# bepu/bepuphysics2

Measured on NVIDIA H100. Metric: constraint-iterations/sec (solver+integrator), higher is better.
Workload: dtype f32

## Files before the change

### bepuphysics2_b200/csrc/bepu_contacts.cuh

```cuda
#pragma once
#include "bepu_device_math.cuh"

namespace BEPU_NS {

constexpr int kLanes = 32;

struct GlobalRows { const float* ptr; };
struct GlobalAcc { float* ptr; };
struct StagedRows { uint32_t addr, bar, parity; };
struct StagedAcc { uint32_t addr; float* ptr; };
BEPU_DI float lds_f32(uint32_t addr) {
    float v;
    asm("ld.shared.f32 %0, [%1];" : "=f"(v) : "r"(addr));
    return v;
}
BEPU_DI void rows_ready(GlobalRows) {}
BEPU_DI void rows_ready(StagedRows p) {
    asm volatile(
        "{\n"
        ".reg .pred p;\n"
        "MBAR_WAIT:\n"
        "mbarrier.try_wait.parity.shared::cta.b64 p, [%0], %1;\n"
        "@p bra MBAR_DONE;\n"
        "bra MBAR_WAIT;\n"
        "MBAR_DONE:\n"
        "}\n" ::"r"(p.bar), "r"(p.parity)
        : "memory");
}
BEPU_DI float ldrow(const float* p, int r) { return __ldcg(p + r * kLanes); }
BEPU_DI float ldrow(GlobalRows p, int r) { return __ldcg(p.ptr + r * kLanes); }
BEPU_DI float ldrow(StagedRows p, int r) { return lds_f32(p.addr + r * (kLanes * 4)); }
template <class PR> BEPU_DI V3 ldrow3(PR p, int r) { return {ldrow(p, r), ldrow(p, r + 1), ldrow(p, r + 2)}; }
template <class PR> BEPU_DI Q4 ldrow4(PR p, int r) { return {ldrow(p, r), ldrow(p, r + 1), ldrow(p, r + 2), ldrow(p, r + 3)}; }
BEPU_DI float ldacc(GlobalAcc a, int r) { return a.ptr[r * kLanes]; }
BEPU_DI void stacc(GlobalAcc a, int r, float v) { a.ptr[r * kLanes] = v; }
BEPU_DI float ldacc(StagedAcc a, int r) { return lds_f32(a.addr + r * (kLanes * 4)); }
BEPU_DI void stacc(StagedAcc a, int r, float v) { __stcs(a.ptr + r * kLanes, v); }

BEPU_DI void penetration_apply(const Inertia& iA, const Inertia& iB, V3 normal, V3 angularA, V3 angularB, float impulse, Velocity& vA, Velocity& vB) {
    V3 dLinA = normal * (impulse * iA.inv_mass);
    V3 dAngA = transform(angularA * impulse, iA.t);
    V3 dLinB = normal * (impulse * iB.inv_mass);
    V3 dAngB = transform(angularB * impulse, iB.t);
    vA.lin = vA.lin + dLinA;
    vA.ang = vA.ang + dAngA;
    vB.lin = vB.lin - dLinB;
    vB.ang = vB.ang + dAngB;
}
BEPU_DI void penetration_warm_start(const Inertia& iA, const Inertia& iB, V3 normal, V3 offsetA, V3 offsetB, float accumulated, Velocity& vA, Velocity& vB) {
    penetration_apply(iA, iB, normal, cross(offsetA, normal), cross(normal, offsetB), accumulated, vA, vB);
}
BEPU_DI void penetration_solve(const Inertia& iA, const Inertia& iB, V3 normal, V3 offsetA, V3 offsetB, float depth, const Springiness& sp, float maxRecovery,
                               float inverseDt, float& accumulated, Velocity& vA, Velocity& vB) {
    V3 angularA = cross(offsetA, normal);
    V3 angularB = cross(normal, offsetB);
    float angularA0 = vector_sandwich(angularA, iA.t);
    float angularB0 = vector_sandwich(angularB, iB.t);
    float linear = iA.inv_mass + iB.inv_mass;
    float effectiveMass = sp.effective_mass_cfm_scale / (linear + angularA0 + angularB0);
    float biasVelocity = fmin_ps(depth * inverseDt, fmin_ps(depth * sp.position_error_to_velocity, maxRecovery));
    float csvaLinear = dot(vA.lin, normal);
    float csvaAngular = dot(vA.ang, angularA);
    float negatedCSVBLinear = dot(vB.lin, normal);
    float csvbAngular = dot(vB.ang, angularB);
    float negatedCSI = accumulated * sp.softness_impulse_scale + (csvaLinear - negatedCSVBLinear + csvaAngular + csvbAngular - biasVelocity) * effectiveMass;
    float previous = accumulated;
    accumulated = fmax_ps(0.0f, accumulated - negatedCSI);
    penetration_apply(iA, iB, normal, angularA, angularB, accumulated - previous, vA, vB);
}
BEPU_DI float updated_depth(float dt, V3 contactOffsetA, V3 offsetB, V3 normal, const Velocity& vA, const Velocity& vB, float depth) {
    V3 contactVelocityA = cross(vA.ang, contactOffsetA) + vA.lin;
    V3 contactOffsetB = contactOffsetA - offsetB;
    V3 contactVelocityB = cross(vB.ang, contactOffsetB) + vB.lin;
    float estimatedDepthChangeVelocity = dot(normal, contactVelocityA - contactVelocityB);
    return depth - estimatedDepthChangeVelocity * dt;
}

BEPU_DI void penetration1_apply(const Inertia& iA, V3 normal, V3 angularA, float impulse, Velocity& vA) {
    V3 dLinA = normal * (impulse * iA.inv_mass);
    V3 dAngA = transform(angularA * impulse, iA.t);
    vA.lin = vA.lin + dLinA;
    vA.ang = vA.ang + dAngA;
}
BEPU_DI void penetration1_solve(const Inertia& iA, V3 normal, V3 offsetA, float depth, const Springiness& sp, float maxRecovery, float inverseDt, float& accumulated,
                                Velocity& vA) {
    V3 angularA = cross(offsetA, normal);
    float angularA0 = vector_sandwich(angularA, iA.t);
    float effectiveMass = sp.effective_mass_cfm_scale / (iA.inv_mass + angularA0);
    float biasVelocity = fmin_ps(depth * inverseDt, fmin_ps(depth * sp.position_error_to_velocity, maxRecovery));
    float csvaLinear = dot(vA.lin, normal);
    float csvaAngular = dot(vA.ang, angularA);
    float negatedCSI = accumulated * sp.softness_impulse_scale + (csvaLinear + csvaAngular - biasVelocity) * effectiveMass;
    float previous = accumulated;
    accumulated = fmax_ps(0.0f, accumulated - negatedCSI);
    penetration1_apply(iA, normal, angularA, accumulated - previous, vA);
}
BEPU_DI float updated_depth1(float dt, V3 contactOffset, V3 normal, const Velocity& v, float depth) {
    V3 contactVelocity = cross(v.ang, contactOffset) + v.lin;
    return depth - dot(normal, contactVelocity) * dt;
}

struct TangentJacobians { M23 linearA, angularA, angularB; };
BEPU_DI TangentJacobians tangent_jacobians(V3 tX, V3 tY, V3 offsetA, V3 offsetB) {
    TangentJacobians j;
    j.linearA = {tX, tY};
    j.angularA = {cross(offsetA, tX), cross(offsetA, tY)};
    j.angularB = {cross(tX, offsetB), cross(tY, offsetB)};
    return j;
}
BEPU_DI void tangent_apply(const TangentJacobians& j, const Inertia& iA, const Inertia& iB, V2 impulse, Velocity& vA, Velocity& vB) {
    V3 linearImpulseA = transform(impulse, j.linearA);
    V3 angularImpulseA = transform(impulse, j.angularA);
    V3 angularImpulseB = transform(impulse, j.angularB);
    vA.lin = vA.lin + linearImpulseA * iA.inv_mass;
    vA.ang = vA.ang + transform(angularImpulseA, iA.t);
    vB.lin = vB.lin - linearImpulseA * iB.inv_mass;
    vB.ang = vB.ang + transform(angularImpulseB, iB.t);
}
BEPU_DI void tangent_solve(V3 tX, V3 tY, V3 offsetA, V3 offsetB, const Inertia& iA, const Inertia& iB, float maximumImpulse, V2& accumulated, Velocity& vA, Velocity& vB) {
    TangentJacobians j = tangent_jacobians(tX, tY, offsetA, offsetB);
    Sym2 linear = sandwich_scale(j.linearA, iA.inv_mass) + sandwich_scale(j.linearA, iB.inv_mass);
    Sym2 angular = matrix_sandwich(j.angularA, iA.t) + matrix_sandwich(j.angularB, iB.t);
    Sym2 effectiveMass = invert(linear + angular);
    V2 csvaLinear = transform_by_transpose(vA.lin, j.linearA);
    V2 csvaAngular = transform_by_transpose(vA.ang, j.angularA);
    V2 csvbLinear = transform_by_transpose(vB.lin, j.linearA);
    V2 csvbAngular = transform_by_transpose(vB.ang, j.angularB);
    V2 csv = (csvbLinear - csvaLinear) - (csvaAngular + csvbAngular);
    V2 csi = transform(csv, effectiveMass);
    V2 previous = accumulated;
    accumulated = accumulated + csi;
    float magnitude = length(accumulated);
    float scl = fmin_ps(1.0f, maximumImpulse / fmax_ps(1e-16f, magnitude));
    accumulated = accumulated * scl;
    tangent_apply(j, iA, iB, accumulated - previous, vA, vB);
}
BEPU_DI void tangent1_apply(const M23& linearA, const M23& angularA, const Inertia& iA, V2 impulse, Velocity& vA) {
    V3 linearImpulseA = transform(impulse, linearA);
    V3 angularImpulseA = transform(impulse, angularA);
    vA.lin = vA.lin + linearImpulseA * iA.inv_mass;
    vA.ang = vA.ang + transform(angularImpulseA, iA.t);
}
BEPU_DI void tangent1_solve(V3 tX, V3 tY, V3 offsetA, const Inertia& iA, float maximumImpulse, V2& accumulated, Velocity& vA) {
    M23 linearA{tX, tY};
    M23 angularA{cross(offsetA, tX), cross(offsetA, tY)};
    Sym2 effectiveMass = invert(sandwich_scale(linearA, iA.inv_mass) + matrix_sandwich(angularA, iA.t));
    V2 csv = transform_by_transpose(vA.lin, linearA) + transform_by_transpose(vA.ang, angularA);
    V2 negativeCSI = transform(csv, effectiveMass);
    V2 previous = accumulated;
    accumulated = accumulated - negativeCSI;
    float magnitude = length(accumulated);
    float scl = fmin_ps(1.0f, maximumImpulse / fmax_ps(1e-16f, magnitude));
    accumulated = accumulated * scl;
    tangent1_apply(linearA, angularA, iA, accumulated - previous, vA);
}

BEPU_DI void twist_apply(V3 axis, const Inertia& iA, const Inertia& iB, float impulse, Velocity& vA, Velocity& vB) {
    V3 worldImpulseA = axis * impulse;
    vA.ang = vA.ang + transform(worldImpulseA, iA.t);
    vB.ang = vB.ang - transform(worldImpulseA, iB.t);
}
BEPU_DI void twist_solve(V3 axis, const Inertia& iA, const Inertia& iB, float maximumImpulse, float& accumulated, Velocity& vA, Velocity& vB) {
    float inverseEffectiveMass = vector_sandwich(axis, iA.t) + vector_sandwich(axis, iB.t);
    float effectiveMass = (0.0f == inverseEffectiveMass) ? 0.0f : 1.0f / inverseEffectiveMass;
    float negatedCSI = (dot(vA.ang, axis) - dot(vB.ang, axis)) * effectiveMass;
    float previous = accumulated;
    accumulated = fmin_ps(maximumImpulse, fmax_ps(-maximumImpulse, accumulated - negatedCSI));
    twist_apply(axis, iA, iB, accumulated - previous, vA, vB);
}
BEPU_DI void twist1_apply(V3 axis, const Inertia& iA, float impulse, Velocity& vA) { vA.ang = vA.ang + transform(axis * impulse, iA.t); }
BEPU_DI void twist1_solve(V3 axis, const Inertia& iA, float maximumImpulse, float& accumulated, Velocity& vA) {
    float angularA = vector_sandwich(axis, iA.t);
    float effectiveMass = (0.0f == angularA) ? 0.0f : 1.0f / angularA;
    float negativeCSI = dot(vA.ang, axis) * effectiveMass;
    float previous = accumulated;
    accumulated = fmin_ps(maximumImpulse, fmax_ps(-maximumImpulse, accumulated - negativeCSI));
    twist1_apply(axis, iA, accumulated - previous, vA);
}

template <int N, bool TwoBody> struct ConvexLayout {
    static constexpr int kOffsetB = 4 * N;
    static constexpr int kNormal = TwoBody ? 4 * N + 3 : 4 * N;
    static constexpr int kFriction = kNormal + 3;
    static constexpr int kAngularFrequency = kNormal + 4;
    static constexpr int kTwiceDampingRatio = kNormal + 5;
    static constexpr int kMaxRecovery = kNormal + 6;
    static constexpr int kPrestepRows = kNormal + 7;
    static constexpr int kImpulseRows = N + 3;
};

template <int N> BEPU_DI V3 friction_center(const V3 (&offs)[N], const float (&depths)[N]) {
    float w[N];
#pragma unroll
    for (int i = 0; i < N; ++i) w[i] = depths[i] < 0.0f ? 0.0f : 1.0f;
    float weightSum = w[0];
#pragma unroll
    for (int i = 1; i < N; ++i) weightSum = weightSum + w[i];
    bool useFallback = weightSum == 0.0f;
    weightSum = useFallback ? (float)N : weightSum;
    float inverseWeightSum = 1.0f / weightSum;
    V3 c[N];
#pragma unroll
    for (int i = 0; i < N; ++i) c[i] = offs[i] * (useFallback ? inverseWeightSum : w[i] * inverseWeightSum);
    if constexpr (N == 2) return c[0] + c[1];
    else if constexpr (N == 3) return (c[0] + c[1]) + c[2];
    else return (c[0] + c[1]) + (c[2] + c[3]);
}

template <int N> struct ConvexTwoBody {
    typedef ConvexLayout<N, true> L;
    static constexpr int kBodies = 2;
    static constexpr int kPrestepRows = L::kPrestepRows;
    static constexpr int kImpulseRows = L::kImpulseRows;
    static constexpr bool kIncremental = true;
    static constexpr bool kNeedsPose = false;

    template <class PR, class AR> BEPU_DI static void warm_start(const Inertia& iA, const Inertia& iB, PR p, AR a, Velocity& vA, Velocity& vB) {
        V3 normal = ldrow3(p, L::kNormal), offsetB = ldrow3(p, L::kOffsetB);
        V3 x, z;
        build_orthonormal_basis(normal, x, z);
        V3 offs[N];
        float depths[N];
#pragma unroll
        for (int i = 0; i < N; ++i) { offs[i] = ldrow3(p, 4 * i); depths[i] = ldrow(p, 4 * i + 3); }
        V3 centerA;
        if constexpr (N == 1) centerA = offs[0]; else centerA = friction_center<N>(offs, depths);
        V3 centerB = centerA - offsetB;
        tangent_apply(tangent_jacobians(x, z, centerA, centerB), iA, iB, V2{ldacc(a, 0), ldacc(a, 1)}, vA, vB);
#pragma unroll 1
        for (int i = 0; i < N; ++i) {
            V3 offset = ldrow3(p, 4 * i);
            penetration_warm_start(iA, iB, normal, offset, offset - offsetB, ldacc(a, 2 + i), vA, vB);
        }
        twist_apply(normal, iA, iB, ldacc(a, N + 2), vA, vB);
    }
    template <class PR, class AR> BEPU_DI static void solve(const Inertia& iA, const Inertia& iB, float dt, float inverseDt, PR p, AR a, Velocity& vA, Velocity& vB) {
        V3 normal = ldrow3(p, L::kNormal), offsetB = ldrow3(p, L::kOffsetB);
        float friction = ldrow(p, L::kFriction), maxRecovery = ldrow(p, L::kMaxRecovery);
        Springiness sp = compute_springiness(ldrow(p, L::kAngularFrequency), ldrow(p, L::kTwiceDampingRatio), dt);
        if constexpr (N > 1) {
            V3 offs[N];
            float depths[N];
#pragma unroll
            for (int i = 0; i < N; ++i) { offs[i] = ldrow3(p, 4 * i); depths[i] = ldrow(p, 4 * i + 3); }
            const V3 centerA = friction_center<N>(offs, depths);
            float penSum = 0.0f, twistSum = 0.0f;
#pragma unroll 1
            for (int i = 0; i < N; ++i) {
                V3 offset = ldrow3(p, 4 * i);
                float pen = ldacc(a, 2 + i);
                penetration_solve(iA, iB, normal, offset, offset - offsetB, ldrow(p, 4 * i + 3), sp, maxRecovery, inverseDt, pen, vA, vB);
                stacc(a, 2 + i, pen);
                const float lever = pen * distance(centerA, offset);
                penSum = i == 0 ? pen : penSum + pen;
                twistSum = i == 0 ? lever : twistSum + lever;
            }
            V3 x, z;
            build_orthonormal_basis(normal, x, z);
            V2 tangent{ldacc(a, 0), ldacc(a, 1)};
            float twist = ldacc(a, N + 2);
            const float premultiplied = (1.0f / N) * friction;
            tangent_solve(x, z, centerA, centerA - offsetB, iA, iB, premultiplied * penSum, tangent, vA, vB);
            twist_solve(normal, iA, iB, premultiplied * twistSum, twist, vA, vB);
            stacc(a, 0, tangent.x);
            stacc(a, 1, tangent.y);
            stacc(a, N + 2, twist);
        } else
        {
        V3 offs[N];
        float depths[N], pen[N];
#pragma unroll
        for (int i = 0; i < N; ++i) { offs[i] = ldrow3(p, 4 * i); depths[i] = ldrow(p, 4 * i + 3); pen[i] = ldacc(a, 2 + i); }
#pragma unroll
        for (int i = 0; i < N; ++i) penetration_solve(iA, iB, normal, offs[i], offs[i] - offsetB, depths[i], sp, maxRecovery, inverseDt, pen[i], vA, vB);
        V3 x, z;
        build_orthonormal_basis(normal, x, z);
        V2 tangent{ldacc(a, 0), ldacc(a, 1)};
        float twist = ldacc(a, N + 2);
        if constexpr (N == 1) {
            float maximumTangentImpulse = friction * pen[0];
            tangent_solve(x, z, offs[0], offs[0] - offsetB, iA, iB, maximumTangentImpulse, tangent, vA, vB);
            float maximumTwistImpulse = friction * pen[0] * fmax_ps(0.0f, depths[0]);
            twist_solve(normal, iA, iB, maximumTwistImpulse, twist, vA, vB);
        } else {
            float premultiplied = (1.0f / N) * friction;
            float penSum = pen[0];
#pragma unroll
            for (int i = 1; i < N; ++i) penSum = penSum + pen[i];
            V3 centerA = friction_center<N>(offs, depths);
            tangent_solve(x, z, centerA, centerA - offsetB, iA, iB, premultiplied * penSum, tangent, vA, vB);
            float twistSum = pen[0] * distance(centerA, offs[0]);
#pragma unroll
            for (int i = 1; i < N; ++i) twistSum = twistSum + pen[i] * distance(centerA, offs[i]);
            twist_solve(normal, iA, iB, premultiplied * twistSum, twist, vA, vB);
        }
        stacc(a, 0, tangent.x);
        stacc(a, 1, tangent.y);
#pragma unroll
        for (int i = 0; i < N; ++i) stacc(a, 2 + i, pen[i]);
        stacc(a, N + 2, twist);
        }
    }
    BEPU_DI static void incremental_update(float dt, const Velocity& vA, const Velocity& vB, float* p) {
        V3 normal = ldrow3(p, L::kNormal), offsetB = ldrow3(p, L::kOffsetB);
#pragma unroll
        for (int i = 0; i < N; ++i) p[(4 * i + 3) * kLanes] = updated_depth(dt, ldrow3(p, 4 * i), offsetB, normal, vA, vB, ldrow(p, 4 * i + 3));
    }
};

template <int N> struct ConvexOneBody {
    typedef ConvexLayout<N, false> L;
    static constexpr int kBodies = 1;
    static constexpr int kPrestepRows = L::kPrestepRows;
    static constexpr int kImpulseRows = L::kImpulseRows;
    static constexpr bool kIncremental = true;
    static constexpr bool kNeedsPose = false;

    template <class PR, class AR> BEPU_DI static void warm_start(const Inertia& iA, PR p, AR a, Velocity& vA) {
        V3 normal = ldrow3(p, L::kNormal);
        V3 x, z;
        build_orthonormal_basis(normal, x, z);
        V3 offs[N];
        float depths[N];
#pragma unroll
        for (int i = 0; i < N; ++i) { offs[i] = ldrow3(p, 4 * i); depths[i] = ldrow(p, 4 * i + 3); }
        V3 centerA;
        if constexpr (N == 1) centerA = offs[0]; else centerA = friction_center<N>(offs, depths);
        tangent1_apply(M23{x, z}, M23{cross(centerA, x), cross(centerA, z)}, iA, V2{ldacc(a, 0), ldacc(a, 1)}, vA);
#pragma unroll 1
        for (int i = 0; i < N; ++i) penetration1_apply(iA, normal, cross(ldrow3(p, 4 * i), normal), ldacc(a, 2 + i), vA);
        twist1_apply(normal, iA, ldacc(a, N + 2), vA);
    }
    template <class PR, class AR> BEPU_DI static void solve(const Inertia& iA, float dt, float inverseDt, PR p, AR a, Velocity& vA) {
        V3 normal = ldrow3(p, L::kNormal);
        float friction = ldrow(p, L::kFriction), maxRecovery = ldrow(p, L::kMaxRecovery);
        Springiness sp = compute_springiness(ldrow(p, L::kAngularFrequency), ldrow(p, L::kTwiceDampingRatio), dt);
        if constexpr (N > 1) {
            V3 offs[N];
            float depths[N];
#pragma unroll
            for (int i = 0; i < N; ++i) { offs[i] = ldrow3(p, 4 * i); depths[i] = ldrow(p, 4 * i + 3); }
            const V3 centerA = friction_center<N>(offs, depths);
            float penSum = 0.0f, twistSum = 0.0f;
#pragma unroll 1
            for (int i = 0; i < N; ++i) {
                V3 offset = ldrow3(p, 4 * i);
                float pen = ldacc(a, 2 + i);
                penetration1_solve(iA, normal, offset, ldrow(p, 4 * i + 3), sp, maxRecovery, inverseDt, pen, vA);
                stacc(a, 2 + i, pen);
                const float lever = pen * distance(centerA, offset);
                penSum = i == 0 ? pen : penSum + pen;
                twistSum = i == 0 ? lever : twistSum + lever;
            }
            V3 x, z;
            build_orthonormal_basis(normal, x, z);
            V2 tangent{ldacc(a, 0), ldacc(a, 1)};
            float twist = ldacc(a, N + 2);
            const float premultiplied = (1.0f / N) * friction;
            tangent1_solve(x, z, centerA, iA, premultiplied * penSum, tangent, vA);
            twist1_solve(normal, iA, premultiplied * twistSum, twist, vA);
            stacc(a, 0, tangent.x);
            stacc(a, 1, tangent.y);
            stacc(a, N + 2, twist);
        } else
        {
        V3 offs[N];
        float depths[N], pen[N];
#pragma unroll
        for (int i = 0; i < N; ++i) { offs[i] = ldrow3(p, 4 * i); depths[i] = ldrow(p, 4 * i + 3); pen[i] = ldacc(a, 2 + i); }
#pragma unroll
        for (int i = 0; i < N; ++i) penetration1_solve(iA, normal, offs[i], depths[i], sp, maxRecovery, inverseDt, pen[i], vA);
        V3 x, z;
        build_orthonormal_basis(normal, x, z);
        V2 tangent{ldacc(a, 0), ldacc(a, 1)};
        float twist = ldacc(a, N + 2);
        if constexpr (N == 1) {
            tangent1_solve(x, z, offs[0], iA, friction * pen[0], tangent, vA);
            twist1_solve(normal, iA, friction * pen[0] * fmax_ps(0.0f, depths[0]), twist, vA);
        } else {
            float premultiplied = (1.0f / N) * friction;
            float penSum = pen[0];
#pragma unroll
            for (int i = 1; i < N; ++i) penSum = penSum + pen[i];
            V3 centerA = friction_center<N>(offs, depths);
            tangent1_solve(x, z, centerA, iA, premultiplied * penSum, tangent, vA);
            float twistSum = pen[0] * distance(centerA, offs[0]);
#pragma unroll
            for (int i = 1; i < N; ++i) twistSum = twistSum + pen[i] * distance(centerA, offs[i]);
            twist1_solve(normal, iA, premultiplied * twistSum, twist, vA);
        }
        stacc(a, 0, tangent.x);
        stacc(a, 1, tangent.y);
#pragma unroll
        for (int i = 0; i < N; ++i) stacc(a, 2 + i, pen[i]);
        stacc(a, N + 2, twist);
        }
    }
    BEPU_DI static void incremental_update(float dt, const Velocity& vA, float* p) {
        V3 normal = ldrow3(p, L::kNormal);
#pragma unroll
        for (int i = 0; i < N; ++i) p[(4 * i + 3) * kLanes] = updated_depth1(dt, ldrow3(p, 4 * i), normal, vA, ldrow(p, 4 * i + 3));
    }
};

#define BEPU_CONTACT_LOOP _Pragma("unroll 1")
template <int N, bool TwoBody> struct NonconvexLayout {
    static constexpr int kOffsetB = 4;
    static constexpr int kContacts = TwoBody ? 7 : 4;
    static constexpr int kPrestepRows = kContacts + 7 * N;
    static constexpr int kImpulseRows = 3 * N;
};
template <int N> struct NonconvexTwoBody {
    typedef NonconvexLayout<N, true> L;
    static constexpr int kBodies = 2;
    static constexpr int kPrestepRows = L::kPrestepRows;
    static constexpr int kImpulseRows = L::kImpulseRows;
    static constexpr bool kIncremental = true;
    static constexpr bool kNeedsPose = false;
    template <class PR, class AR> BEPU_DI static void warm_start(const Inertia& iA, const Inertia& iB, PR p, AR a, Velocity& vA, Velocity& vB) {
        V3 offsetB = ldrow3(p, L::kOffsetB);
BEPU_CONTACT_LOOP
        for (int i = 0; i < N; ++i) {
            const int c = L::kContacts + 7 * i;
            V3 offset = ldrow3(p, c), normal = ldrow3(p, c + 4);
            V3 x, z;
            build_orthonormal_basis(normal, x, z);
            V3 contactOffsetB = offset - offsetB;
            tangent_apply(tangent_jacobians(x, z, offset, contactOffsetB), iA, iB, V2{ldacc(a, 3 * i), ldacc(a, 3 * i + 1)}, vA, vB);
            penetration_warm_start(iA, iB, normal, offset, contactOffsetB, ldacc(a, 3 * i + 2), vA, vB);
        }
    }
    template <class PR, class AR> BEPU_DI static void solve(const Inertia& iA, const Inertia& iB, float dt, float inverseDt, PR p, AR a, Velocity& vA, Velocity& vB) {
        V3 offsetB = ldrow3(p, L::kOffsetB);
        float friction = ldrow(p, 0), maxRecovery = ldrow(p, 3);
        Springiness sp = compute_springiness(ldrow(p, 1), ldrow(p, 2), dt);
BEPU_CONTACT_LOOP
        for (int i = 0; i < N; ++i) {
            const int c = L::kContacts + 7 * i;
            V3 offset = ldrow3(p, c), normal = ldrow3(p, c + 4);
            float depth = ldrow(p, c + 3);
            V2 tangent{ldacc(a, 3 * i), ldacc(a, 3 * i + 1)};
            float pen = ldacc(a, 3 * i + 2);
            V3 contactOffsetB = offset - offsetB;
            penetration_solve(iA, iB, normal, offset, contactOffsetB, depth, sp, maxRecovery, inverseDt, pen, vA, vB);
            V3 x, z;
            build_orthonormal_basis(normal, x, z);
            tangent_solve(x, z, offset, contactOffsetB, iA, iB, friction * pen, tangent, vA, vB);
            stacc(a, 3 * i, tangent.x);
            stacc(a, 3 * i + 1, tangent.y);
            stacc(a, 3 * i + 2, pen);
        }
    }
    BEPU_DI static void incremental_update(float dt, const Velocity& vA, const Velocity& vB, float* p) {
        V3 offsetB = ldrow3(p, L::kOffsetB);
#pragma unroll
        for (int i = 0; i < N; ++i) {
            const int c = L::kContacts + 7 * i;
            p[(c + 3) * kLanes] = updated_depth(dt, ldrow3(p, c), offsetB, ldrow3(p, c + 4), vA, vB, ldrow(p, c + 3));
        }
    }
};
template <int N> struct NonconvexOneBody {
    typedef NonconvexLayout<N, false> L;
    static constexpr int kBodies = 1;
    static constexpr int kPrestepRows = L::kPrestepRows;
    static constexpr int kImpulseRows = L::kImpulseRows;
    static constexpr bool kIncremental = true;
    static constexpr bool kNeedsPose = false;
    template <class PR, class AR> BEPU_DI static void warm_start(const Inertia& iA, PR p, AR a, Velocity& vA) {
BEPU_CONTACT_LOOP
        for (int i = 0; i < N; ++i) {
            const int c = L::kContacts + 7 * i;
            V3 offset = ldrow3(p, c), normal = ldrow3(p, c + 4);
            V3 x, z;
            build_orthonormal_basis(normal, x, z);
            tangent1_apply(M23{x, z}, M23{cross(offset, x), cross(offset, z)}, iA, V2{ldacc(a, 3 * i), ldacc(a, 3 * i + 1)}, vA);
            penetration1_apply(iA, normal, cross(offset, normal), ldacc(a, 3 * i + 2), vA);
        }
    }
    template <class PR, class AR> BEPU_DI static void solve(const Inertia& iA, float dt, float inverseDt, PR p, AR a, Velocity& vA) {
        float friction = ldrow(p, 0), maxRecovery = ldrow(p, 3);
        Springiness sp = compute_springiness(ldrow(p, 1), ldrow(p, 2), dt);
BEPU_CONTACT_LOOP
        for (int i = 0; i < N; ++i) {
            const int c = L::kContacts + 7 * i;
            V3 offset = ldrow3(p, c), normal = ldrow3(p, c + 4);
            float depth = ldrow(p, c + 3);
            V2 tangent{ldacc(a, 3 * i), ldacc(a, 3 * i + 1)};
            float pen = ldacc(a, 3 * i + 2);
            penetration1_solve(iA, normal, offset, depth, sp, maxRecovery, inverseDt, pen, vA);
            V3 x, z;
            build_orthonormal_basis(normal, x, z);
            tangent1_solve(x, z, offset, iA, friction * pen, tangent, vA);
            stacc(a, 3 * i, tangent.x);
            stacc(a, 3 * i + 1, tangent.y);
            stacc(a, 3 * i + 2, pen);
        }
    }
    BEPU_DI static void incremental_update(float dt, const Velocity& vA, float* p) {
#pragma unroll
        for (int i = 0; i < N; ++i) {
            const int c = L::kContacts + 7 * i;
            p[(c + 3) * kLanes] = updated_depth1(dt, ldrow3(p, c), ldrow3(p, c + 4), vA, ldrow(p, c + 3));
        }
    }
};

}
```

### bepuphysics2_b200/csrc/bepu_solver_kernels.cuh

```cuda
#pragma once
#include "bepu_contacts.cuh"
#include "bepu_joints_more.cuh"
#include "bepu_integration.cuh"
#include "bepu_device_types.h"

namespace BEPU_NS {

using namespace bepucuda;

struct F8 { float a, b, c, d, e, f, g, h; };
#define BEPU_BODY_LD "ld.global.L1::no_allocate.L2::cache_hint.v4.f32"
#define BEPU_BODY_ST "st.global.L1::no_allocate.L2::cache_hint.v4.f32"
BEPU_DI uint64_t l2_evict_last_policy() {
    uint64_t policy;
    asm("createpolicy.fractional.L2::evict_last.b64 %0, 1.0;" : "=l"(policy));
    return policy;
}
BEPU_DI F8 ld256(const float4* p) {
    F8 r;
    asm volatile(BEPU_BODY_LD " {%0,%1,%2,%3}, [%8], %9;\n\t" BEPU_BODY_LD " {%4,%5,%6,%7}, [%8+16], %9;"
                 : "=f"(r.a), "=f"(r.b), "=f"(r.c), "=f"(r.d), "=f"(r.e), "=f"(r.f), "=f"(r.g), "=f"(r.h)
                 : "l"(p), "l"(l2_evict_last_policy())
                 : "memory");
    return r;
}
BEPU_DI void st256(float4* p, float a, float b, float c, float d, float e, float f, float g, float h) {
    asm volatile(BEPU_BODY_ST " [%0], {%1,%2,%3,%4}, %9;\n\t" BEPU_BODY_ST " [%0+16], {%5,%6,%7,%8}, %9;" ::"l"(p), "f"(a), "f"(b), "f"(c), "f"(d), "f"(e), "f"(f), "f"(g), "f"(h),
                 "l"(l2_evict_last_policy())
                 : "memory");
}
BEPU_DI void load_velocity(const float4* vel, uint32_t i, Velocity& v) {
    const F8 r = ld256(vel + 2 * (size_t)i);
    v.lin = {r.a, r.b, r.c};
    v.ang = {r.e, r.f, r.g};
}
BEPU_DI void store_velocity(float4* vel, uint32_t i, const Velocity& v) { st256(vel + 2 * (size_t)i, v.lin.x, v.lin.y, v.lin.z, 0.0f, v.ang.x, v.ang.y, v.ang.z, 0.0f); }
BEPU_DI void load_inertia(const float4* in, uint32_t i, Inertia& r) {
    const F8 x = ld256(in + 2 * (size_t)i);
    r.t = {x.a, x.b, x.c, x.d, x.e, x.f};
    r.inv_mass = x.g;
}
BEPU_DI void store_inertia(float4* in, uint32_t i, const Inertia& r) { st256(in + 2 * (size_t)i, r.t.xx, r.t.yx, r.t.yy, r.t.zx, r.t.zy, r.t.zz, r.inv_mass, 0.0f); }
BEPU_DI void load_pose(const float4* pose, uint32_t i, V3& pos, Q4& q) {
    const F8 x = ld256(pose + 2 * (size_t)i);
    q = {x.a, x.b, x.c, x.d};
    pos = {x.e, x.f, x.g};
}
BEPU_DI void store_pose(float4* pose, uint32_t i, V3 pos, Q4 q) { st256(pose + 2 * (size_t)i, q.x, q.y, q.z, q.w, pos.x, pos.y, pos.z, 0.0f); }

template <int STAGE, bool NeedsPose>
BEPU_DI void warm_start_body(uint32_t enc, const BodyBuffers& B, const FrameParams& fp, BodyState& b, Velocity& v) {
    const uint32_t idx = enc & kRefIndexMask;
    if (enc & kRefIntegrateBit) {
        Inertia local;
        load_inertia(B.inertia_local, idx, local);
        load_pose(B.pose, idx, b.pos, b.q);
        b.inertia.inv_mass = local.inv_mass;
        if (STAGE == kStageWarmStart) {
            b.pos = b.pos + v.lin * fp.dt;
            Q4 previousOrientation = b.q;
            b.q = integrate_orientation(b.q, v.ang, fp.dt * 0.5f);
            b.inertia.t = rotate_inverse_inertia(local.t, b.q);
            if (fp.angular_mode == 1) integrate_angular_conserve_momentum(previousOrientation, local.t, b.inertia.t, v.ang);
            else if (fp.angular_mode == 2) integrate_angular_gyroscopic(b.q, local.t, v.ang, fp.dt);
            store_pose(B.pose, idx, b.pos, b.q);
        } else {
            b.inertia.t = rotate_inverse_inertia(local.t, b.q);
            if (fp.angular_mode == 1) {
                Q4 previousOrientation = integrate_orientation(b.q, v.ang, fp.dt * -0.5f);
                integrate_angular_conserve_momentum(previousOrientation, local.t, b.inertia.t, v.ang);
            } else if (fp.angular_mode == 2) {
                integrate_angular_gyroscopic(b.q, local.t, v.ang, fp.dt);
            }
        }
        callback_integrate_velocity(v, fp.gravity_dt[0], fp.gravity_dt[1], fp.gravity_dt[2], fp.linear_damping_dt, fp.angular_damping_dt);
        store_inertia(B.inertia_world, idx, b.inertia);
    } else {
        load_inertia(B.inertia_world, idx, b.inertia);
        if (NeedsPose) load_pose(B.pose, idx, b.pos, b.q);
        if (STAGE == kStageWarmStartFirst && fp.angular_mode != 0 && (enc & kRefBundleIntegratesBit) && !(enc & kRefKinematicBit)) {
            Inertia local;
            load_inertia(B.inertia_local, idx, local);
            V3 pos;
            Q4 q;
            load_pose(B.pose, idx, pos, q);
            if (fp.angular_mode == 1) integrate_angular_conserve_momentum(integrate_orientation(q, v.ang, fp.dt * -0.5f), local.t, b.inertia.t, v.ang);
            else integrate_angular_gyroscopic(q, local.t, v.ang, fp.dt);
        }
    }
}
template <int STAGE, bool NeedsPose>
BEPU_DI void gather_for_warm_start(uint32_t enc, const BodyBuffers& B, const FrameParams& fp, BodyState& b, Velocity& v) {
    load_velocity(B.velocity, enc & kRefIndexMask, v);
    warm_start_body<STAGE, NeedsPose>(enc, B, fp, b, v);
}

template <class T, class PR, class AR> BEPU_DI void call_warm_start(const BodyState* b, PR p, AR a, Velocity* v) {
    if constexpr (T::kNeedsPose) T::warm_start(b, p, a, v);
    else if constexpr (T::kBodies == 2) T::warm_start(b[0].inertia, b[1].inertia, p, a, v[0], v[1]);
    else T::warm_start(b[0].inertia, p, a, v[0]);
}
template <class T, class PR, class AR> BEPU_DI void call_solve(const BodyState* b, float dt, float inverseDt, PR p, AR a, Velocity* v) {
    if constexpr (T::kNeedsPose) T::solve(b, dt, inverseDt, p, a, v);
    else if constexpr (T::kBodies == 2) T::solve(b[0].inertia, b[1].inertia, dt, inverseDt, p, a, v[0], v[1]);
    else T::solve(b[0].inertia, dt, inverseDt, p, a, v[0]);
}
template <class T> BEPU_DI void call_incremental(float dt, const Velocity* v, float* p) {
    if constexpr (T::kIncremental) {
        if constexpr (T::kBodies == 2) T::incremental_update(dt, v[0], v[1], p);
        else T::incremental_update(dt, v[0], p);
    }
}

BEPU_DI uint32_t ldg_nc_u32(const void* p) {
    uint32_t v;
    asm volatile("ld.global.nc.u32 %0, [%1];" : "=r"(v) : "l"(p));
    return v;
}
BEPU_DI void push_record(float4* const* arrays, uint32_t mask, uint32_t idx, float a, float b, float c, float d, float e, float f, float g, float h) {
    while (mask) {
        const int q = __ffs((int)mask) - 1;
        mask &= mask - 1u;
        float4* dst = arrays[q] + 2 * (size_t)idx;
        dst[0] = make_float4(a, b, c, d);
        dst[1] = make_float4(e, f, g, h);
    }
}
template <class T, int STAGE, bool kSharded, class PR, class AR>
BEPU_DI void run_lane(const int32_t* refs, PR p, AR a, float* p_rw, uint32_t enc0, uint32_t enc1, const BodyBuffers& B, const FrameParams& fp, const ShardPeers* peers = nullptr,
                      long long peer_delta = 0) {
    constexpr int NB = T::kBodies;
    uint32_t enc[NB];
    enc[0] = enc0;
    if constexpr (NB > 1) enc[1] = enc1;
#pragma unroll
    for (int s = 2; s < NB; ++s) enc[s] = (uint32_t)__ldg(refs + s * kLanes);
    uint32_t push_to[kSharded ? NB : 1];
    if constexpr (kSharded) {
#pragma unroll
        for (int s = 0; s < NB; ++s) push_to[s] = peer_delta != 0 ? ldg_nc_u32(refs + peer_delta + s * kLanes) : 0u;
    }
    if ((int32_t)enc[0] == kRefEmpty) return;
    BodyState b[NB];
    Velocity v[NB];
    if constexpr (STAGE == kStageIncremental) {
#pragma unroll
        for (int s = 0; s < NB; ++s) load_velocity(B.velocity, enc[s] & kRefIndexMask, v[s]);
        call_incremental<T>(fp.dt, v, p_rw);
    } else if constexpr (STAGE == kStageSolve) {
#pragma unroll
        for (int s = 0; s < NB; ++s) {
            const uint32_t idx = enc[s] & kRefIndexMask;
            load_velocity(B.velocity, idx, v[s]);
            load_inertia(B.inertia_world, idx, b[s].inertia);
            if (T::kNeedsPose) load_pose(B.pose, idx, b[s].pos, b[s].q);
        }
        rows_ready(p);
        call_solve<T>(b, fp.dt, fp.inverse_dt, p, a, v);
#pragma unroll
        for (int s = 0; s < NB; ++s)
            if (!(enc[s] & kRefKinematicBit)) {
                store_velocity(B.velocity, enc[s] & kRefIndexMask, v[s]);
                if constexpr (kSharded) {
                    const uint32_t mask = push_to[s];
                    if (mask) push_record(peers->velocity, mask, enc[s] & kRefIndexMask, v[s].lin.x, v[s].lin.y, v[s].lin.z, 0.0f, v[s].ang.x, v[s].ang.y, v[s].ang.z, 0.0f);
                }
            }
    } else {
#pragma unroll
        for (int s = 0; s < NB; ++s) gather_for_warm_start<STAGE, T::kNeedsPose>(enc[s], B, fp, b[s], v[s]);
        rows_ready(p);
        call_warm_start<T>(b, p, a, v);
#pragma unroll
        for (int s = 0; s < NB; ++s)
            if (!(enc[s] & kRefKinematicBit)) {
                const uint32_t idx = enc[s] & kRefIndexMask;
                store_velocity(B.velocity, idx, v[s]);
                if constexpr (kSharded) {
                    const uint32_t mask = push_to[s];
                    if (mask) {
                        push_record(peers->velocity, mask, idx, v[s].lin.x, v[s].lin.y, v[s].lin.z, 0.0f, v[s].ang.x, v[s].ang.y, v[s].ang.z, 0.0f);
                        if (enc[s] & kRefIntegrateBit) {
                            const Inertia& in = b[s].inertia;
                            push_record(peers->inertia_world, mask, idx, in.t.xx, in.t.yx, in.t.yy, in.t.zx, in.t.zy, in.t.zz, in.inv_mass, 0.0f);
                            if (STAGE == kStageWarmStart) push_record(peers->pose, mask, idx, b[s].q.x, b[s].q.y, b[s].q.z, b[s].q.w, b[s].pos.x, b[s].pos.y, b[s].pos.z, 0.0f);
                        }
                    }
                }
            }
    }
}
template <class T, int STAGE, class PR, class AR>
BEPU_DI void run_lane(const int32_t* refs, PR p, AR a, float* p_rw, uint32_t enc0, uint32_t enc1, const BodyBuffers& B, const FrameParams& fp) {
    run_lane<T, STAGE, false>(refs, p, a, p_rw, enc0, enc1, B, fp);
}

BEPU_DI int4 ldg_nc_v4(const void* p) {
    int4 v;
    asm volatile("ld.global.nc.v4.s32 {%0,%1,%2,%3}, [%4];" : "=r"(v.x), "=r"(v.y), "=r"(v.z), "=r"(v.w) : "l"(p));
    return v;
}
BEPU_DI WorkRecord load_record(const WorkRecord* r) {
    const int4 lo = ldg_nc_v4(r), hi = ldg_nc_v4(reinterpret_cast<const int4*>(r) + 1);
    WorkRecord w;
    w.refs = reinterpret_cast<int32_t*>((unsigned long long)(unsigned int)lo.x | ((unsigned long long)(unsigned int)lo.y << 32));
    w.prestep = reinterpret_cast<float*>((unsigned long long)(unsigned int)lo.z | ((unsigned long long)(unsigned int)lo.w << 32));
    w.impulses = reinterpret_cast<float*>((unsigned long long)(unsigned int)hi.x | ((unsigned long long)(unsigned int)hi.y << 32));
    w.type_id = hi.z;
    w.live_lanes = hi.w;
    return w;
}

#define BEPU_CONTACT_TYPES(X)                                                                                                     \
    X(0, ConvexOneBody<1>) X(1, ConvexOneBody<2>) X(2, ConvexOneBody<3>) X(3, ConvexOneBody<4>)                                   \
    X(4, ConvexTwoBody<1>) X(5, ConvexTwoBody<2>) X(6, ConvexTwoBody<3>) X(7, ConvexTwoBody<4>)                                   \
    X(8, NonconvexOneBody<2>) X(9, NonconvexOneBody<3>) X(10, NonconvexOneBody<4>)                                                \
    X(15, NonconvexTwoBody<2>) X(16, NonconvexTwoBody<3>) X(17, NonconvexTwoBody<4>)

template <int STAGE, bool kSharded, class PR, class AR>
BEPU_DI void run_bundle_rows(const WorkRecord& rec, int lane, PR p, AR a, uint32_t enc0, uint32_t enc1, const BodyBuffers& B, const FrameParams& fp, const ShardPeers* peers = nullptr,
                             long long peer_delta = 0) {
    const int32_t* refs = rec.refs + lane;
    float* p_rw = rec.prestep + lane;
    switch (rec.type_id) {
#define BEPU_CASE(ID, T) \
    case ID: run_lane<T, STAGE, kSharded>(refs, p, a, p_rw, enc0, enc1, B, fp, peers, peer_delta); break;
        BEPU_CONTACT_TYPES(BEPU_CASE)
        BEPU_JOINT_TYPES(BEPU_CASE)
        BEPU_JOINT_TYPES_MORE(BEPU_CASE)
#undef BEPU_CASE
        default: break;
    }
}
template <int STAGE, class PR, class AR>
BEPU_DI void run_bundle_rows(const WorkRecord& rec, int lane, PR p, AR a, uint32_t enc0, uint32_t enc1, const BodyBuffers& B, const FrameParams& fp) {
    run_bundle_rows<STAGE, false>(rec, lane, p, a, enc0, enc1, B, fp);
}
template <int STAGE>
BEPU_DI void run_bundle(const WorkRecord& rec, int lane, uint32_t enc0, uint32_t enc1, const BodyBuffers& B, const FrameParams& fp) {
    run_bundle_rows<STAGE>(rec, lane, GlobalRows{rec.prestep + lane}, GlobalAcc{rec.impulses + lane}, enc0, enc1, B, fp);
}
template <int STAGE> BEPU_DI void run_bundle(const WorkRecord& rec, int lane, const BodyBuffers& B, const FrameParams& fp) {
    const uint32_t enc0 = ldg_nc_u32(rec.refs + lane), enc1 = ldg_nc_u32(rec.refs + kLanes + lane);
    run_bundle<STAGE>(rec, lane, enc0, enc1, B, fp);
}

struct StageRowCounts { uint8_t prestep[64], impulses[64]; };
__host__ __device__ constexpr StageRowCounts make_stage_row_counts() {
    StageRowCounts c{};
#define BEPU_ROWS(ID, T) c.prestep[ID] = (uint8_t)T::kPrestepRows; c.impulses[ID] = (uint8_t)T::kImpulseRows;
    BEPU_CONTACT_TYPES(BEPU_ROWS)
    BEPU_JOINT_TYPES(BEPU_ROWS)
    BEPU_JOINT_TYPES_MORE(BEPU_ROWS)
#undef BEPU_ROWS
    return c;
}
__constant__ StageRowCounts kStageRowCounts = make_stage_row_counts();
constexpr int kStageSlabRows = 48;
constexpr int kStageSlabBytes = kStageSlabRows * kLanes * 4;

BEPU_DI uint32_t smem_u32(const void* p) { return (uint32_t)__cvta_generic_to_shared(p); }
BEPU_DI void mbar_init(uint32_t bar, uint32_t count) {
    asm volatile("mbarrier.init.shared::cta.b64 [%0], %1;" ::"r"(bar), "r"(count) : "memory");
    asm volatile("fence.mbarrier_init.release.cluster;" ::: "memory");
    asm volatile("fence.proxy.async.shared::cta;" ::: "memory");
}
BEPU_DI void mbar_expect_tx(uint32_t bar, uint32_t bytes) { asm volatile("mbarrier.arrive.expect_tx.shared::cta.b64 _, [%0], %1;" ::"r"(bar), "r"(bytes) : "memory"); }
BEPU_DI uint64_t l2_evict_first_policy() {
    uint64_t policy;
    asm volatile("createpolicy.fractional.L2::evict_first.b64 %0, 1.0;" : "=l"(policy));
    return policy;
}
BEPU_DI void bulk_copy_g2s(uint32_t dst, const void* src, uint32_t bytes, uint32_t bar, uint64_t policy) {
    asm volatile("cp.async.bulk.shared::cluster.global.mbarrier::complete_tx::bytes.L2::cache_hint [%0], [%1], %2, [%3], %4;" ::"r"(dst), "l"(src), "r"(bytes), "r"(bar),
                 "l"(policy)
                 : "memory");
}

#ifndef BEPU_STAGE_BLOCK_THREADS
#define BEPU_STAGE_BLOCK_THREADS 64
#endif
constexpr int kStageBlockThreads = BEPU_STAGE_BLOCK_THREADS;

constexpr int kStagePrefetchRows = 1;
BEPU_DI void shard_announce(const ShardPeers& peers, int lane) {
    if (lane < peers.rank_count && lane != peers.rank)
        asm volatile("red.release.sys.global.add.u64 [%0], 1;" ::"l"(peers.flags[lane] + kShardCounterSlot + peers.rank) : "memory");
}
BEPU_DI void shard_wait(const ShardPeers& peers, int lane, uint32_t solve_index, uint32_t exchange_point, int32_t* error_flag) {
    if (lane < peers.rank_count && lane != peers.rank) {
        const unsigned long long* mine = peers.flags[peers.rank];
        const unsigned long long* targets = mine + kShardTargetSlot + (size_t)lane * kShardMaxExchanges;
        const unsigned long long want = (unsigned long long)solve_index * targets[kShardMaxExchanges - 1] + targets[exchange_point];
        unsigned long long seen;
        unsigned int spins = 0;
        do {
            asm volatile("ld.acquire.sys.global.u64 %0, [%1];" : "=l"(seen) : "l"(mine + kShardCounterSlot + lane) : "memory");
        } while (seen < want && ++spins < 100000000u);
        if (seen < want) atomicExch(error_flag, 5);
    }
    __syncwarp();
}
template <int STAGE, bool kSharded>
BEPU_DI void constraint_stage_body(const WorkRecord* __restrict__ records, const int32_t* __restrict__ ref_rows, int work_count, const BodyBuffers& B, const FrameParams* __restrict__ fpp, int flags, const ShardPeers* peers,
                                   long long peer_delta, const ShardStage* shard = nullptr) {
    constexpr bool kStaged = STAGE != kStageIncremental;
    constexpr int kWarps = kStageBlockThreads / 32;
    __shared__ __align__(128) float slab[kStaged ? kWarps * kStageSlabRows * kLanes : 1];
    __shared__ __align__(8) unsigned long long bars[kWarps];
    const int warp_in_block = threadIdx.x >> 5;
    const int global_warp = (blockIdx.x * kStageBlockThreads + threadIdx.x) >> 5;
    const int lane = threadIdx.x & 31;
    WorkRecord rec{};
    uint32_t enc0 = (uint32_t)kRefEmpty, enc1 = 0;
    const int warp = global_warp;
    const bool active = warp < work_count;
    const uint32_t slab_addr = kStaged ? smem_u32(slab) + warp_in_block * kStageSlabBytes : 0;
    const uint32_t bar = smem_u32(&bars[warp_in_block]);
    const bool early_rows = kStaged && (flags & kStagePrefetchRows);
    uint32_t prestep_bytes = 0, impulse_bytes = 0;
    if (active) {
        rec = load_record(records + warp);
        if constexpr (kStaged) {
            prestep_bytes = kStageRowCounts.prestep[rec.type_id] * (kLanes * 4);
            impulse_bytes = kStageRowCounts.impulses[rec.type_id] * (kLanes * 4);
            if (lane == 0) {
                mbar_init(bar, 1);
                if (early_rows) {
                    const uint64_t policy = l2_evict_first_policy();
                    mbar_expect_tx(bar, prestep_bytes + impulse_bytes);
                    bulk_copy_g2s(slab_addr, rec.prestep, prestep_bytes, bar, policy);
                    bulk_copy_g2s(slab_addr + prestep_bytes, rec.impulses, impulse_bytes, bar, policy);
                }
            }
        }
        enc0 = ldg_nc_u32(ref_rows + (size_t)warp * (2 * kLanes) + lane);
        enc1 = ldg_nc_u32(ref_rows + (size_t)warp * (2 * kLanes) + kLanes + lane);
    }
    const FrameParams fp = *fpp;
    asm volatile("griddepcontrol.wait;" ::: "memory");
    asm volatile("griddepcontrol.launch_dependents;");
    bool boundary = false;
    if constexpr (kSharded) {
        boundary = active && (rec.live_lanes & kRecordBoundaryBit) != 0;
        if (boundary && shard->exchange_index > 0 && !(fp.tune[0] & 1)) shard_wait(*peers, lane, fp.shard_solve_index, shard->exchange_index - 1u, shard->error_flag);
    }
    if (!active) return;
    if constexpr (kStaged) {
        if (!early_rows && lane == 0) {
            const uint64_t policy = l2_evict_first_policy();
            mbar_expect_tx(bar, prestep_bytes + impulse_bytes);
            bulk_copy_g2s(slab_addr, rec.prestep, prestep_bytes, bar, policy);
            bulk_copy_g2s(slab_addr + prestep_bytes, rec.impulses, impulse_bytes, bar, policy);
        }
        __syncwarp();
        run_bundle_rows<STAGE, kSharded>(rec, lane, StagedRows{slab_addr + lane * 4, bar, 0u}, StagedAcc{slab_addr + prestep_bytes + lane * 4, rec.impulses + lane}, enc0, enc1, B, fp,
                                         peers, boundary && !(fp.tune[0] & 4) ? peer_delta : 0);
        if constexpr (kSharded) {
            if (boundary && !(fp.tune[0] & 2)) {
                __syncwarp();
                shard_announce(*peers, lane);
            }
        }
    } else {
        run_bundle<STAGE>(rec, lane, enc0, enc1, B, fp);
    }
}

template <int STAGE, int MINB>
__global__ void __launch_bounds__(kStageBlockThreads, MINB) constraint_stage_kernel(const WorkRecord* __restrict__ records, const int32_t* __restrict__ ref_rows, int work_count, BodyBuffers B, const FrameParams* __restrict__ fpp, int flags) {
    constraint_stage_body<STAGE, false>(records, ref_rows, work_count, B, fpp, flags, nullptr, 0);
}
template <int STAGE, int MINB>
__global__ void __launch_bounds__(kStageBlockThreads, MINB)
constraint_stage_kernel_sharded(const WorkRecord* __restrict__ records, const int32_t* __restrict__ ref_rows, int work_count, BodyBuffers B, const FrameParams* __restrict__ fpp, int flags, const __grid_constant__ ShardPeers peers,
                                long long peer_delta, const __grid_constant__ ShardStage shard) {
    constraint_stage_body<STAGE, true>(records, ref_rows, work_count, B, fpp, flags, &peers, peer_delta, &shard);
}

template <int STAGE> BEPU_DI void run_kinematic(int i, const int32_t* kinematics, const BodyBuffers& B, const FrameParams& fp) {
    const uint32_t idx = (uint32_t)kinematics[i];
    Velocity v;
    load_velocity(B.velocity, idx, v);
    if (STAGE == kStageKinematic) {
        V3 pos;
        Q4 q;
        load_pose(B.pose, idx, pos, q);
        pos = pos + v.lin * fp.dt;
        q = integrate_orientation(q, v.ang, fp.dt * 0.5f);
        store_pose(B.pose, idx, pos, q);
    }
    if (fp.integrate_velocity_for_kinematics) {
        callback_integrate_velocity(v, fp.gravity_dt[0], fp.gravity_dt[1], fp.gravity_dt[2], fp.linear_damping_dt, fp.angular_damping_dt);
        store_velocity(B.velocity, idx, v);
    }
}
template <int STAGE>
__global__ void kinematic_stage_kernel(const int32_t* __restrict__ kinematics, int count, BodyBuffers B, const FrameParams* __restrict__ fpp) {
    const int i = blockIdx.x * blockDim.x + threadIdx.x;
    if (i >= count) return;
    const FrameParams fp = *fpp;
    run_kinematic<STAGE>(i, kinematics, B, fp);
}

BEPU_DI void run_final_pose(int i, const BodyBuffers& B, const FrameParams& fp) {
    V3 pos;
    Q4 q;
    Velocity v;
    load_pose(B.pose, i, pos, q);
    load_velocity(B.velocity, i, v);
    if (B.constrained[i]) {
        q = integrate_orientation(q, v.ang, fp.dt * 0.5f);
        pos = pos + v.lin * fp.dt;
        store_pose(B.pose, i, pos, q);
        return;
    }
    Inertia local;
    load_inertia(B.inertia_local, i, local);
    const bool kinematic = local.inv_mass == 0.0f && local.t.xx == 0.0f && local.t.yx == 0.0f && local.t.yy == 0.0f && local.t.zx == 0.0f && local.t.zy == 0.0f && local.t.zz == 0.0f;
    const bool integrateVelocity = fp.integrate_velocity_for_kinematics || !kinematic;
    const float dt = fp.final_dt, halfDt = fp.final_dt * 0.5f;
    for (int step = 0; step < fp.final_steps; ++step) {
        if (integrateVelocity)
            callback_integrate_velocity(v, fp.final_gravity_dt[0], fp.final_gravity_dt[1], fp.final_gravity_dt[2], fp.final_linear_damping_dt, fp.final_angular_damping_dt);
        pos = pos + v.lin * dt;
        if (fp.angular_mode == 1) {
            Q4 previousOrientation = q;
            q = integrate_orientation(q, v.ang, halfDt);
            integrate_angular_conserve_momentum(previousOrientation, local.t, rotate_inverse_inertia(local.t, q), v.ang);
        } else if (fp.angular_mode == 2) {
            q = integrate_orientation(q, v.ang, halfDt);
            integrate_angular_gyroscopic(q, local.t, v.ang, dt);
        } else {
            q = integrate_orientation(q, v.ang, halfDt);
        }
    }
    store_pose(B.pose, i, pos, q);
    if (integrateVelocity) store_velocity(B.velocity, i, v);
}
static __global__ void final_pose_kernel(BodyBuffers B, const FrameParams* __restrict__ fpp) {
    const int i = blockIdx.x * blockDim.x + threadIdx.x;
    if (i >= B.count) return;
    const FrameParams fp = *fpp;
    run_final_pose(i, B, fp);
}

}
```

### bepuphysics2_b200/csrc/bepucuda_api.cu

```cuda
#include <algorithm>
#include <cmath>
#include <cstdio>
#include <cstdlib>
#include <cstring>
#include <map>
#include <string>
#include <vector>

#include "../../include/bepucuda.h"
#include "bepu_layout_kernels.h"
#include "bepu_coloring.h"
#include "bepu_bounds.h"

using namespace bepucuda;

namespace bepucuda {

static TypeInfo make_contact(int bodies, int prestep, int impulses, int contacts, const char* name) {
    TypeInfo t{};
    t.bodies = bodies; t.prestep_rows = prestep; t.impulse_rows = impulses; t.incremental = 1; t.name = name;
    const int body_rw = 13 + 6;
    t.solve_bytes = 4 * (prestep + 2 * impulses + bodies + bodies * body_rw);
    t.warm_start_bytes = 4 * (prestep + impulses + bodies + bodies * body_rw);
    t.incremental_bytes = 4 * (prestep + contacts + bodies + 6 * bodies);
    return t;
}
static TypeInfo make_joint(int bodies, int prestep, int impulses, int solve_r, int solve_w, int ws_r, int ws_w, const char* name) {
    TypeInfo t{};
    t.bodies = bodies; t.prestep_rows = prestep; t.impulse_rows = impulses; t.incremental = 0; t.name = name;
    t.solve_bytes = 4 * (prestep + 2 * impulses + bodies + solve_r + solve_w);
    t.warm_start_bytes = 4 * (prestep + impulses + bodies + ws_r + ws_w);
    t.incremental_bytes = 0;
    return t;
}
struct Registry {
    TypeInfo types[64];
    bool present[64];
    Registry() {
        std::memset(present, 0, sizeof(present));
        auto add = [&](int id, TypeInfo t) { types[id] = t; present[id] = true; };
        add(0, make_contact(1, 11, 4, 1, "Contact1OneBody")); add(1, make_contact(1, 15, 5, 2, "Contact2OneBody"));
        add(2, make_contact(1, 19, 6, 3, "Contact3OneBody")); add(3, make_contact(1, 23, 7, 4, "Contact4OneBody"));
        add(4, make_contact(2, 14, 4, 1, "Contact1")); add(5, make_contact(2, 18, 5, 2, "Contact2"));
        add(6, make_contact(2, 22, 6, 3, "Contact3")); add(7, make_contact(2, 26, 7, 4, "Contact4"));
        add(8, make_contact(1, 18, 6, 2, "Contact2NonconvexOneBody")); add(9, make_contact(1, 25, 9, 3, "Contact3NonconvexOneBody"));
        add(10, make_contact(1, 32, 12, 4, "Contact4NonconvexOneBody"));
        add(15, make_contact(2, 21, 6, 2, "Contact2Nonconvex")); add(16, make_contact(2, 28, 9, 3, "Contact3Nonconvex"));
        add(17, make_contact(2, 35, 12, 4, "Contact4Nonconvex"));
#define BEPU_REGISTER_JOINTS
#include "bepu_joint_registry.inc"
#undef BEPU_REGISTER_JOINTS
    }
};
static const Registry& registry() {
    static Registry r;
    return r;
}
const TypeInfo* get_type_info(int type_id) {
    if (type_id < 0 || type_id >= 64 || !registry().present[type_id]) return nullptr;
    return &registry().types[type_id];
}

struct DeviceBuffer {
    void* ptr = nullptr;
    size_t capacity = 0;
    cudaError_t reserve(size_t bytes) {
        if (bytes <= capacity) return cudaSuccess;
        if (ptr) cudaFree(ptr);
        ptr = nullptr;
        capacity = 0;
        size_t want = bytes + bytes / 4 + 256;
        cudaError_t e = cudaMalloc(&ptr, want);
        if (e == cudaSuccess) capacity = want;
        return e;
    }
    void release() {
        if (ptr) cudaFree(ptr);
        ptr = nullptr;
        capacity = 0;
    }
    template <class T> T* as() const { return (T*)ptr; }
};

struct ChunkArena {
    struct Chunk { char* base; size_t size, used; };
    std::vector<Chunk> chunks;
    bool pinned_host = false;
    size_t min_chunk = (size_t)64 << 20;
    void reset() { for (auto& c : chunks) c.used = 0; }
    void* alloc(size_t bytes, cudaError_t* err) {
        bytes = (bytes + 255) & ~(size_t)255;
        for (auto& c : chunks)
            if (c.size - c.used >= bytes) {
                void* p = c.base + c.used;
                c.used += bytes;
                return p;
            }
        Chunk c{};
        c.size = std::max(bytes, min_chunk);
        cudaError_t e = pinned_host ? cudaMallocHost((void**)&c.base, c.size) : cudaMalloc((void**)&c.base, c.size);
        if (e != cudaSuccess) { if (err) *err = e; return nullptr; }
        c.used = bytes;
        chunks.push_back(c);
        return chunks.back().base;
    }
    void release() {
        for (auto& c : chunks) { if (pinned_host) cudaFreeHost(c.base); else cudaFree(c.base); }
        chunks.clear();
    }
};

struct SourceTypeBatch {
    int batch_index, type_batch_index, type_id, count;
    int live = 0;
    float* host_impulses;
    int32_t* raw_refs;
    float* raw_prestep;
    float* raw_impulses;
    size_t refs_bytes, prestep_bytes, impulse_bytes;
    std::vector<int32_t> host_refs;
    std::vector<int> device_tbs;
    int32_t* raw_features_old = nullptr;
    int32_t* raw_features_new = nullptr;
    size_t feature_bytes = 0;
    bool resident_impulses = false, redistribute = false;
};

}

struct bepucuda_ctx {
    bepucuda_config cfg{};
    int32_t tune[4] = {0, 0, 0, 0};
    int device = 0;
    cudaStream_t stream = nullptr;
    cudaEvent_t ev_solve_begin = nullptr, ev_solve_end = nullptr, ev_up_begin = nullptr, ev_up_end = nullptr, ev_down_begin = nullptr, ev_down_end = nullptr;
    bool up_open = false, have_solve = false, have_down = false, have_up = false;
    std::string error;
    const SolverLaunchers* launchers = nullptr;

    std::vector<int32_t> iterations{1};
    int fallback_threshold = 64;
    bepucuda_integrator_desc integ{};
    bool integ_set = false;

    int body_count = 0;
    DeviceBuffer raw_bodies, pose, velocity, inertia_local, inertia_world, constrained, first_batch, sync_refcount, sync_mask;
    BodyBuffers B{};

    int W = 8;
    int batch_count = 0;
    bool constraints_open = false, constraints_ready = false, data_dirty = false, descs_dirty = false;
    std::vector<SourceTypeBatch> sources;
    ChunkArena raw_arena, pinned_arena;
    DeviceBuffer record_table, ref_rows, source_bundle_flags, refs32, prestep32, impulses32, tb_table, tdesc_table, work_table, map_table, bodies_per_type, kinematics_dev, program_dev, frame_params_dev, error_dev;
    std::vector<DeviceTypeBatch> tbs;
    std::vector<TransposeDesc> tdescs;
    std::vector<WorkItem> work;
    std::vector<int32_t> bundle_live;
    std::vector<WorkRecord> records;
    std::vector<std::pair<int, int>> batch_work;
    bool exchange_failed = false;
    bepucuda_exchange_fn exchange = nullptr;
    void* exchange_user = nullptr;
    DeviceBuffer exchange_staging;
    bool peer_mode = false;
    ShardPeers peers{};
    DeviceBuffer shard_flags, pushes_dev, peer32, body_masks_dev, boundary_flags_dev;
    uint32_t shard_solve_index = 0;
    std::vector<int> boundary_count;
    std::vector<uint8_t> body_masks;
    size_t refs_words = 0;
    std::vector<void*> opened_ipc;
    std::vector<int32_t> global_first_batch;
    std::vector<uint8_t> global_constrained;
    std::map<int, std::vector<uint32_t>> pushes_by_batch;
    std::vector<std::pair<size_t, int>> push_range;
    uint32_t exchange_counter = 0;
    uint32_t exchanges_per_solve = 0;
    int inc_work_begin = 0, inc_work_count = 0;
    int all_work_count = 0;
    int sync_batch_count = 0, fallback_levels = 0;
    std::vector<int32_t> kinematics;
    std::vector<StageOp> program;
    FrameParams* frame_params_host = nullptr;

    cudaGraph_t graph = nullptr;
    cudaGraphExec_t graph_exec = nullptr;
    bool graph_valid = false;

    bepucuda_timings timings{};
    int64_t h2d_accum = 0;
    struct HostRange { char* host; size_t bytes; char* dev; };
    std::vector<HostRange> host_ranges;
    std::vector<CopyChunk> pending_h2d;
    DeviceBuffer chunk_table;
    struct ChunkStage { void* host = nullptr; size_t capacity = 0; cudaEvent_t done = nullptr; };
    ChunkStage chunk_stage[4];
    int chunk_stage_next = 0;
    cudaEvent_t user_events[16] = {};
    DeviceBuffer body_shapes, body_activities, body_bounds;
    int shape_count = -1;
    DeviceBuffer color_refs, color_priorities, color_body_min, color_body_mask, color_out, color_lists, color_counts;
    std::vector<cudaEvent_t> profile_events;
};

namespace {

int fail(bepucuda_ctx* c, int code, const std::string& msg) {
    if (c) c->error = msg;
    return code;
}
int cuda_fail(bepucuda_ctx* c, cudaError_t e, const char* what) {
    return fail(c, e == cudaErrorMemoryAllocation ? BEPUCUDA_ERR_OUT_OF_MEMORY : BEPUCUDA_ERR_CUDA, std::string(what) + ": " + cudaGetErrorString(e));
}
#define CK(call)                                                  \
    do {                                                          \
        cudaError_t _e = (call);                                  \
        if (_e != cudaSuccess) return cuda_fail(ctx, _e, #call);  \
    } while (0)

void open_upload_window(bepucuda_ctx* ctx) {
    if (!ctx->up_open) {
        cudaEventRecord(ctx->ev_up_begin, ctx->stream);
        ctx->up_open = true;
    }
}

char* map_host(bepucuda_ctx* ctx, const void* ptr, size_t bytes) {
    const char* p = (const char*)ptr;
    for (auto& r : ctx->host_ranges)
        if (p >= r.host && p + bytes <= r.host + r.bytes) return r.dev + (p - r.host);
    return nullptr;
}
void queue_chunks(std::vector<CopyChunk>& list, void* dst, const void* src, size_t bytes) {
    const size_t kChunk = (size_t)64 << 10;
    for (size_t off = 0; off < bytes; off += kChunk) list.push_back({(char*)dst + off, (const char*)src + off, std::min(kChunk, bytes - off)});
}
int flush_chunks(bepucuda_ctx* ctx, std::vector<CopyChunk>& list) {
    if (list.empty()) return BEPUCUDA_OK;
    const size_t bytes = list.size() * sizeof(CopyChunk);
    CK(ctx->chunk_table.reserve(bytes));
    auto& st = ctx->chunk_stage[ctx->chunk_stage_next];
    ctx->chunk_stage_next = (ctx->chunk_stage_next + 1) & 3;
    if (!st.done) CK(cudaEventCreateWithFlags(&st.done, cudaEventDisableTiming));
    CK(cudaEventSynchronize(st.done));
    if (st.capacity < bytes) {
        if (st.host) cudaFreeHost(st.host);
        st.host = nullptr;
        st.capacity = 0;
        CK(cudaMallocHost(&st.host, bytes * 2));
        st.capacity = bytes * 2;
    }
    std::memcpy(st.host, list.data(), bytes);
    CK(cudaMemcpyAsync(ctx->chunk_table.ptr, st.host, bytes, cudaMemcpyHostToDevice, ctx->stream));
    launch_batched_copy(ctx->chunk_table.as<CopyChunk>(), (int)list.size(), ctx->stream);
    CK(cudaGetLastError());
    CK(cudaEventRecord(st.done, ctx->stream));
    list.clear();
    return BEPUCUDA_OK;
}

int copy_in(bepucuda_ctx* ctx, void* dst, const void* src, size_t bytes) {
    if (bytes == 0) return BEPUCUDA_OK;
    if (char* alias = map_host(ctx, src, bytes)) {
        queue_chunks(ctx->pending_h2d, dst, alias, bytes);
        ctx->h2d_accum += (int64_t)bytes;
        return BEPUCUDA_OK;
    }
    if (bytes < ((size_t)256 << 10)) {
        cudaError_t e = cudaSuccess;
        void* stage = ctx->pinned_arena.alloc(bytes, &e);
        if (!stage) return cuda_fail(ctx, e, "pinned staging");
        std::memcpy(stage, src, bytes);
        CK(cudaMemcpyAsync(dst, stage, bytes, cudaMemcpyHostToDevice, ctx->stream));
    } else {
        CK(cudaMemcpyAsync(dst, src, bytes, cudaMemcpyHostToDevice, ctx->stream));
    }
    ctx->h2d_accum += (int64_t)bytes;
    return BEPUCUDA_OK;
}

void invalidate_graph(bepucuda_ctx* ctx) {
    if (ctx->graph_exec) cudaGraphExecDestroy(ctx->graph_exec);
    if (ctx->graph) cudaGraphDestroy(ctx->graph);
    ctx->graph_exec = nullptr;
    ctx->graph = nullptr;
    ctx->graph_valid = false;
}

void issue_stage_sequence(bepucuda_ctx* ctx, cudaStream_t s, int64_t* launches) {
    const WorkRecord* records = ctx->record_table.as<WorkRecord>();
    const int32_t* ref_rows = ctx->ref_rows.as<int32_t>();
    const FrameParams* fp = ctx->frame_params_dev.as<FrameParams>();
    const int32_t* kin = ctx->kinematics_dev.as<int32_t>();
    int64_t n = 0;
    const bool pdl = ctx->cfg.reserved[1] == 0;
    const StageOp* previous = nullptr;
    uint32_t exchange_index = 0;
    const bool fused_pushes = ctx->peer_mode && !ctx->body_masks.empty();
    for (const StageOp& op : ctx->program) {
        if (ctx->peer_mode && op.pad == -1) {
            launch_shard_exchange(nullptr, 0, 1, ctx->B, ctx->peers, fp, exchange_index++, ctx->error_dev.as<int32_t>(), s);
            ++n;
            continue;
        }
        if (ctx->peer_mode && op.pad >= 2 && op.stage <= kStageSolve) {
            if (op.work_count > 0) {
                bool prefetch = previous != nullptr && previous->stage != kStageIncremental && !(previous->stage <= kStageSolve && previous->work_begin == op.work_begin && previous->work_count > 0);
                const int launch_flags = (pdl ? kLaunchPdl : 0) | (prefetch ? kLaunchPrefetchRows : 0);
                if (fused_pushes) {
                    const ShardStage shard{exchange_index, ctx->error_dev.as<int32_t>()};
                    ctx->launchers->constraint_stage_sharded(op.stage, records + op.work_begin, ref_rows + (size_t)op.work_begin * 64, op.work_count, ctx->B, fp, launch_flags, ctx->peers,
                                                             (long long)(ctx->peer32.as<int32_t>() - ctx->refs32.as<int32_t>()), shard, s);
                    ++exchange_index;
                    ++n;
                    previous = &op;
                    continue;
                }
                ctx->launchers->constraint_stage(op.stage, records + op.work_begin, ref_rows + (size_t)op.work_begin * 64, op.work_count, ctx->B, fp, launch_flags, s);
                ++n;
            }
            if (fused_pushes) { ++exchange_index; continue; }
            const auto& range = ctx->push_range[op.pad - 2];
            launch_shard_exchange(ctx->pushes_dev.as<uint32_t>() + range.first, range.second, op.stage == kStageSolve ? 1 : (op.stage == kStageWarmStart ? 3 : 2), ctx->B, ctx->peers, fp,
                                  exchange_index++, ctx->error_dev.as<int32_t>(), s);
            ++n;
            if (op.work_count > 0) previous = &op;
            continue;
        }
        switch (op.stage) {
            case kStageWarmStartFirst: case kStageWarmStart: case kStageSolve: case kStageIncremental:
                if (op.work_count > 0) {
                    bool prefetch = op.stage != kStageIncremental && previous != nullptr && previous->stage != kStageIncremental;
                    if (prefetch && previous->stage <= kStageSolve && previous->work_begin == op.work_begin) prefetch = false;
                    if (ctx->exchange) {
                        ctx->launchers->constraint_stage(op.stage, records + op.work_begin, ref_rows + (size_t)op.work_begin * 64, op.work_count, ctx->B, fp, 0, s);
                        ++n;
                        if (op.stage != kStageIncremental) {
                            const int planes = op.stage == kStageSolve ? 1 : (op.stage == kStageWarmStart ? 3 : 2);
                            const size_t words = (size_t)ctx->body_count * 8 * planes;
                            cudaMemsetAsync(ctx->exchange_staging.ptr, 0, words * 4, s);
                            launch_collect_stage(ctx->tb_table.as<DeviceTypeBatch>(), ctx->work_table.as<WorkItem>() + op.work_begin, op.work_count, ctx->bodies_per_type.as<int32_t>(), op.stage,
                                                 ctx->B, ctx->exchange_staging.as<int32_t>(), s);
                            if (ctx->exchange(ctx->exchange_user, ctx->exchange_staging.ptr, (int64_t)words, 0, (void*)s) != 0) ctx->exchange_failed = true;
                            launch_apply_stage(ctx->exchange_staging.as<int32_t>(), planes, ctx->B, s);
                            n += 2;
                        }
                        previous = &op;
                        break;
                    }
                    ctx->launchers->constraint_stage(op.stage, records + op.work_begin, ref_rows + (size_t)op.work_begin * 64, op.work_count, ctx->B, fp, (pdl ? kLaunchPdl : 0) | (prefetch ? kLaunchPrefetchRows : 0), s);
                    previous = &op;
                    ++n;
                }
                break;
            case kStageKinematicFirst: case kStageKinematic:
                if (op.work_count > 0) { ctx->launchers->kinematic_stage(op.stage, kin, op.work_count, ctx->B, fp, s); previous = &op; ++n; }
                break;
            case kStageFinalPose:
                if (ctx->B.count > 0) { ctx->launchers->final_pose(ctx->B, fp, s); previous = &op; ++n; }
                break;
        }
    }
    if (launches) *launches = n;
    ctx->exchanges_per_solve = exchange_index;
}

void build_program(bepucuda_ctx* ctx) {
    ctx->program.clear();
    const int substeps = (int)ctx->iterations.size();
    const int kin = (int)ctx->kinematics.size();
    for (int s = 0; s < substeps; ++s) {
        if (s > 0) {
            if (ctx->peer_mode) ctx->program.push_back({kStageKinematic, 0, 0, -1});
            if (ctx->inc_work_count > 0) ctx->program.push_back({kStageIncremental, ctx->inc_work_begin, ctx->inc_work_count, 0});
            if (kin > 0) ctx->program.push_back({kStageKinematic, 0, kin, 0});
        } else if (ctx->integ.integrate_velocity_for_kinematics && kin > 0) {
            ctx->program.push_back({kStageKinematicFirst, 0, kin, 0});
        }
        if (ctx->peer_mode) ctx->program.push_back({kStageKinematic, 0, 0, -1});
        for (size_t b = 0; b < ctx->batch_work.size(); ++b) {
            auto& bw = ctx->batch_work[b];
            if (bw.second > 0 || (ctx->peer_mode && (int)b < ctx->sync_batch_count)) ctx->program.push_back({s == 0 ? kStageWarmStartFirst : kStageWarmStart, bw.first, bw.second, ctx->peer_mode ? (int)b + 2 : 0});
        }
        for (int it = 0; it < ctx->iterations[s]; ++it)
            for (size_t b = 0; b < ctx->batch_work.size(); ++b) {
                auto& bw = ctx->batch_work[b];
                if (bw.second > 0 || (ctx->peer_mode && (int)b < ctx->sync_batch_count)) ctx->program.push_back({kStageSolve, bw.first, bw.second, ctx->peer_mode ? (int)b + 2 : 0});
            }
    }
    if (ctx->peer_mode) ctx->program.push_back({kStageKinematic, 0, 0, -1});
    ctx->program.push_back({kStageFinalPose, 0, ctx->body_count, 0});
}

int upload_program(bepucuda_ctx* ctx) {
    build_program(ctx);
    if (ctx->peer_mode && !ctx->body_masks.empty() && ctx->boundary_count.size() == ctx->batch_work.size()) {
        std::vector<unsigned long long> targets((size_t)kShardMaxExchanges, 0ull);
        unsigned long long arrived = 0;
        size_t e = 0;
        for (const StageOp& op : ctx->program) {
            if (op.pad != -1 && !(op.pad >= 2 && op.stage <= kStageSolve)) continue;
            if (e + 1 >= (size_t)kShardMaxExchanges) return fail(ctx, BEPUCUDA_ERR_BAD_STATE, "peer sharding: more than 4095 exchange points per solve");
            if (op.pad >= 2 && op.work_count > 0) arrived += (unsigned long long)ctx->boundary_count[(size_t)(op.pad - 2)];
            targets[e++] = arrived;
        }
        targets[(size_t)kShardMaxExchanges - 1] = arrived;
        CK(cudaStreamSynchronize(ctx->stream));
        for (int q = 0; q < ctx->peers.rank_count; ++q)
            if (q != ctx->peers.rank)
                CK(cudaMemcpy(ctx->peers.flags[q] + kShardTargetSlot + (size_t)ctx->peers.rank * kShardMaxExchanges, targets.data(), targets.size() * 8, cudaMemcpyDefault));
        CK(cudaMemset((unsigned long long*)ctx->shard_flags.ptr + kShardCounterSlot, 0, kMaxShardRanks * 8));
        ctx->shard_solve_index = 0;
    }
    CK(ctx->program_dev.reserve(ctx->program.size() * sizeof(StageOp)));
    CK(cudaMemcpyAsync(ctx->program_dev.ptr, ctx->program.data(), ctx->program.size() * sizeof(StageOp), cudaMemcpyHostToDevice, ctx->stream));
    CK(cudaStreamSynchronize(ctx->stream));
    invalidate_graph(ctx);
    int64_t stages = 0;
    for (auto& op : ctx->program) stages += (op.work_count > 0 || op.stage == kStageFinalPose) ? 1 : 0;
    ctx->timings.stage_count = stages;
    return BEPUCUDA_OK;
}

void compute_frame_params(bepucuda_ctx* ctx, float dt, FrameParams* fp) {
    const int substeps = (int)ctx->iterations.size();
    const float substepDt = dt / substeps;
    auto clamp01 = [](float v) { return v < 0.f ? 0.f : (v > 1.f ? 1.f : v); };
    const bepucuda_integrator_desc& d = ctx->integ;
    fp->dt = substepDt;
    fp->inverse_dt = 1.0f / substepDt;
    fp->linear_damping_dt = powf(clamp01(1 - d.linear_damping), substepDt);
    fp->angular_damping_dt = powf(clamp01(1 - d.angular_damping), substepDt);
    for (int i = 0; i < 3; ++i) fp->gravity_dt[i] = d.gravity[i] * substepDt;
    const float finalDt = d.allow_substeps_for_unconstrained ? substepDt : dt;
    fp->final_dt = finalDt;
    fp->final_linear_damping_dt = powf(clamp01(1 - d.linear_damping), finalDt);
    fp->final_angular_damping_dt = powf(clamp01(1 - d.angular_damping), finalDt);
    for (int i = 0; i < 3; ++i) fp->final_gravity_dt[i] = d.gravity[i] * finalDt;
    fp->final_steps = d.allow_substeps_for_unconstrained ? substeps : 1;
    fp->angular_mode = d.angular_integration_mode;
    fp->integrate_velocity_for_kinematics = d.integrate_velocity_for_kinematics;
    for (int i = 0; i < 4; ++i) fp->tune[i] = ctx->tune[i];
}

int refresh_device_rows(bepucuda_ctx* ctx) {
    if (!ctx->data_dirty) return BEPUCUDA_OK;
    { int rc = flush_chunks(ctx, ctx->pending_h2d); if (rc != BEPUCUDA_OK) return rc; }
    bool any_redistribute = false;
    if (ctx->descs_dirty) {
        for (SourceTypeBatch& s : ctx->sources)
            for (int tb : s.device_tbs) {
                TransposeDesc& d = ctx->tdescs[tb];
                d.flags = (s.resident_impulses ? kDescResidentImpulses : 0) | (s.redistribute ? kDescRedistribute : 0);
                d.features_old = s.raw_features_old;
                d.features_new = s.raw_features_new;
                any_redistribute |= s.redistribute;
            }
        CK(cudaMemcpyAsync(ctx->tdesc_table.ptr, ctx->tdescs.data(), ctx->tdescs.size() * sizeof(TransposeDesc), cudaMemcpyHostToDevice, ctx->stream));
    }
    launch_transpose_in_all(ctx->tb_table.as<DeviceTypeBatch>(), ctx->tdesc_table.as<TransposeDesc>(), ctx->work_table.as<WorkItem>(), ctx->all_work_count, ctx->W,
                            kTransposePrestep | kTransposeImpulses, ctx->stream);
    if (any_redistribute) {
        launch_redistribute_impulses(ctx->tb_table.as<DeviceTypeBatch>(), ctx->tdesc_table.as<TransposeDesc>(), ctx->work_table.as<WorkItem>(), ctx->all_work_count, ctx->stream);
        for (SourceTypeBatch& s : ctx->sources)
            if (s.redistribute) {
                std::swap(s.raw_features_old, s.raw_features_new);
                s.redistribute = false;
            }
    } else {
        ctx->descs_dirty = false;
    }
    CK(cudaGetLastError());
    ctx->data_dirty = false;
    return BEPUCUDA_OK;
}

}

extern "C" {

int32_t bepucuda_type_info(int32_t type_id, int32_t* bodies_per_constraint, int32_t* prestep_floats, int32_t* impulse_floats) {
    const TypeInfo* t = get_type_info(type_id);
    if (!t) return BEPUCUDA_ERR_UNSUPPORTED_TYPE;
    if (bodies_per_constraint) *bodies_per_constraint = t->bodies;
    if (prestep_floats) *prestep_floats = t->prestep_rows;
    if (impulse_floats) *impulse_floats = t->impulse_rows;
    return BEPUCUDA_OK;
}

int32_t bepucuda_create(const bepucuda_config* cfg, bepucuda_ctx** out) {
    if (!cfg || !out) return BEPUCUDA_ERR_INVALID_ARGUMENT;
    *out = nullptr;
    int count = 0;
    if (cudaGetDeviceCount(&count) != cudaSuccess || count <= 0) return BEPUCUDA_ERR_NO_DEVICE;
    if (cfg->device_ordinal < 0 || cfg->device_ordinal >= count) return BEPUCUDA_ERR_INVALID_ARGUMENT;
    if (cfg->execution_mode != BEPUCUDA_EXEC_GRAPH && cfg->execution_mode != BEPUCUDA_EXEC_STREAM) return BEPUCUDA_ERR_INVALID_ARGUMENT;
    bepucuda_ctx* ctx = new bepucuda_ctx();
    ctx->cfg = *cfg;
    if (const char* tune = getenv("BEPUCUDA_TUNE")) sscanf(tune, "%d,%d,%d,%d", &ctx->tune[0], &ctx->tune[1], &ctx->tune[2], &ctx->tune[3]);
    ctx->device = cfg->device_ordinal;
    ctx->launchers = cfg->strict_fp ? get_launchers_bepu_strict() : get_launchers_bepu_fast();
    ctx->pinned_arena.pinned_host = true;
    ctx->pinned_arena.min_chunk = (size_t)16 << 20;
    cudaError_t e = cudaSetDevice(ctx->device);
    if (e == cudaSuccess) e = cudaStreamCreateWithFlags(&ctx->stream, cudaStreamNonBlocking);
    cudaEvent_t* evs[] = {&ctx->ev_solve_begin, &ctx->ev_solve_end, &ctx->ev_up_begin, &ctx->ev_up_end, &ctx->ev_down_begin, &ctx->ev_down_end};
    for (auto ev : evs)
        if (e == cudaSuccess) e = cudaEventCreate(ev);
    if (e == cudaSuccess) e = cudaMallocHost((void**)&ctx->frame_params_host, sizeof(FrameParams));
    if (e == cudaSuccess) e = ctx->frame_params_dev.reserve(sizeof(FrameParams));
    if (e == cudaSuccess) e = ctx->error_dev.reserve(8 * sizeof(int32_t));
    if (e != cudaSuccess) {
        bepucuda_destroy(ctx);
        return e == cudaErrorMemoryAllocation ? BEPUCUDA_ERR_OUT_OF_MEMORY : BEPUCUDA_ERR_CUDA;
    }
    ctx->integ.gravity[0] = 0; ctx->integ.gravity[1] = -10; ctx->integ.gravity[2] = 0;
    ctx->integ.linear_damping = 0.03f;
    ctx->integ.angular_damping = 0.03f;
    *out = ctx;
    return BEPUCUDA_OK;
}

int32_t bepucuda_destroy(bepucuda_ctx* ctx) {
    if (!ctx) return BEPUCUDA_OK;
    cudaSetDevice(ctx->device);
    if (ctx->stream) cudaStreamSynchronize(ctx->stream);
    invalidate_graph(ctx);
    for (void* p : ctx->opened_ipc) cudaIpcCloseMemHandle(p);
    DeviceBuffer* bufs[] = {&ctx->shard_flags, &ctx->pushes_dev, &ctx->peer32, &ctx->body_masks_dev, &ctx->boundary_flags_dev, &ctx->raw_bodies, &ctx->pose, &ctx->velocity, &ctx->inertia_local, &ctx->inertia_world, &ctx->constrained, &ctx->first_batch, &ctx->sync_refcount,
                            &ctx->sync_mask, &ctx->chunk_table, &ctx->record_table, &ctx->ref_rows, &ctx->body_shapes, &ctx->body_activities, &ctx->body_bounds, &ctx->color_refs, &ctx->color_priorities, &ctx->color_body_min, &ctx->color_body_mask, &ctx->color_out, &ctx->color_lists, &ctx->color_counts, &ctx->source_bundle_flags, &ctx->refs32, &ctx->prestep32, &ctx->impulses32, &ctx->tb_table, &ctx->tdesc_table, &ctx->work_table, &ctx->map_table,
                            &ctx->bodies_per_type, &ctx->kinematics_dev, &ctx->program_dev, &ctx->frame_params_dev, &ctx->error_dev, &ctx->exchange_staging};
    for (auto b : bufs) b->release();
    ctx->raw_arena.release();
    ctx->pinned_arena.release();
    if (ctx->frame_params_host) cudaFreeHost(ctx->frame_params_host);
    for (auto ev : ctx->user_events)
        if (ev) cudaEventDestroy(ev);
    for (auto& st : ctx->chunk_stage) {
        if (st.host) cudaFreeHost(st.host);
        if (st.done) cudaEventDestroy(st.done);
    }
    for (auto ev : ctx->profile_events) cudaEventDestroy(ev);
    cudaEvent_t evs[] = {ctx->ev_solve_begin, ctx->ev_solve_end, ctx->ev_up_begin, ctx->ev_up_end, ctx->ev_down_begin, ctx->ev_down_end};
    for (auto ev : evs)
        if (ev) cudaEventDestroy(ev);
    if (ctx->stream) cudaStreamDestroy(ctx->stream);
    delete ctx;
    return BEPUCUDA_OK;
}

const char* bepucuda_last_error(bepucuda_ctx* ctx) { return ctx ? ctx->error.c_str() : "null context"; }

int32_t bepucuda_host_register(bepucuda_ctx* ctx, void* ptr, int64_t bytes) {
    if (!ctx || !ptr || bytes <= 0) return fail(ctx, BEPUCUDA_ERR_INVALID_ARGUMENT, "host_register: bad arguments");
    CK(cudaSetDevice(ctx->device));
    CK(cudaHostRegister(ptr, (size_t)bytes, cudaHostRegisterMapped | cudaHostRegisterPortable));
    void* dev = nullptr;
    CK(cudaHostGetDevicePointer(&dev, ptr, 0));
    ctx->host_ranges.push_back({(char*)ptr, (size_t)bytes, (char*)dev});
    return BEPUCUDA_OK;
}
int32_t bepucuda_host_unregister(bepucuda_ctx* ctx, void* ptr) {
    if (!ctx || !ptr) return fail(ctx, BEPUCUDA_ERR_INVALID_ARGUMENT, "host_unregister: bad arguments");
    CK(cudaSetDevice(ctx->device));
    CK(cudaStreamSynchronize(ctx->stream));
    CK(cudaHostUnregister(ptr));
    for (size_t i = 0; i < ctx->host_ranges.size(); ++i)
        if (ctx->host_ranges[i].host == (char*)ptr) { ctx->host_ranges.erase(ctx->host_ranges.begin() + i); break; }
    return BEPUCUDA_OK;
}

int32_t bepucuda_set_solve_description(bepucuda_ctx* ctx, int32_t substep_count, const int32_t* its, int32_t fallback_batch_threshold) {
    if (!ctx || substep_count < 1 || !its || fallback_batch_threshold < 1) return fail(ctx, BEPUCUDA_ERR_INVALID_ARGUMENT, "set_solve_description: bad arguments");
    for (int i = 0; i < substep_count; ++i)
        if (its[i] < 0) return fail(ctx, BEPUCUDA_ERR_INVALID_ARGUMENT, "set_solve_description: negative iteration count");
    std::vector<int32_t> v(its, its + substep_count);
    const bool threshold_changed = fallback_batch_threshold != ctx->fallback_threshold;
    const bool changed = v != ctx->iterations || threshold_changed;
    ctx->iterations = v;
    ctx->fallback_threshold = fallback_batch_threshold;
    if (threshold_changed && ctx->constraints_ready) ctx->constraints_ready = false;
    if (changed && ctx->constraints_ready) {
        CK(cudaSetDevice(ctx->device));
        return upload_program(ctx);
    }
    return BEPUCUDA_OK;
}

int32_t bepucuda_set_integrator(bepucuda_ctx* ctx, const bepucuda_integrator_desc* desc) {
    if (!ctx || !desc) return fail(ctx, BEPUCUDA_ERR_INVALID_ARGUMENT, "set_integrator: bad arguments");
    if (desc->angular_integration_mode < 0 || desc->angular_integration_mode > 2) return fail(ctx, BEPUCUDA_ERR_INVALID_ARGUMENT, "set_integrator: unknown AngularIntegrationMode");
    const bool kin_changed = (desc->integrate_velocity_for_kinematics != 0) != (ctx->integ.integrate_velocity_for_kinematics != 0);
    ctx->integ = *desc;
    ctx->integ_set = true;
    if (kin_changed && ctx->constraints_ready) {
        CK(cudaSetDevice(ctx->device));
        return upload_program(ctx);
    }
    return BEPUCUDA_OK;
}

int32_t bepucuda_upload_bodies(bepucuda_ctx* ctx, const void* body_dynamics, int32_t body_count) {
    if (!ctx || body_count < 0 || (body_count > 0 && !body_dynamics)) return fail(ctx, BEPUCUDA_ERR_INVALID_ARGUMENT, "upload_bodies: bad arguments");
    if ((uint32_t)body_count > kRefIndexMask) return fail(ctx, BEPUCUDA_ERR_INVALID_ARGUMENT, "upload_bodies: too many bodies");
    CK(cudaSetDevice(ctx->device));
    open_upload_window(ctx);
    const size_t n = (size_t)body_count;
    if (body_count != ctx->body_count) {
        if (ctx->constraints_ready) ctx->constraints_ready = false;
        invalidate_graph(ctx);
    }
    CK(ctx->raw_bodies.reserve(n * 128));
    CK(ctx->pose.reserve(n * 32));
    CK(ctx->velocity.reserve(n * 32));
    CK(ctx->inertia_local.reserve(n * 32));
    CK(ctx->inertia_world.reserve(n * 32));
    const size_t old_constrained_cap = ctx->constrained.capacity;
    CK(ctx->constrained.reserve(n + 1));
    if (ctx->constrained.capacity != old_constrained_cap) CK(cudaMemsetAsync(ctx->constrained.ptr, 0, ctx->constrained.capacity, ctx->stream));
    ctx->body_count = body_count;
    BodyBuffers B{};
    B.pose = ctx->pose.as<float4>();
    B.velocity = ctx->velocity.as<float4>();
    B.inertia_local = ctx->inertia_local.as<float4>();
    B.inertia_world = ctx->inertia_world.as<float4>();
    B.constrained = ctx->constrained.as<uint8_t>();
    B.count = body_count;
    if (B.pose != ctx->B.pose || B.velocity != ctx->B.velocity || B.inertia_local != ctx->B.inertia_local || B.inertia_world != ctx->B.inertia_world ||
        B.constrained != ctx->B.constrained || B.count != ctx->B.count)
        invalidate_graph(ctx);
    ctx->B = B;
    if (body_count > 0) {
        CK(cudaMemcpyAsync(ctx->raw_bodies.ptr, body_dynamics, n * 128, cudaMemcpyHostToDevice, ctx->stream));
        ctx->h2d_accum += (int64_t)n * 128;
        launch_split_bodies(ctx->raw_bodies.ptr, body_count, ctx->B, ctx->stream);
        CK(cudaGetLastError());
    }
    return BEPUCUDA_OK;
}

int32_t bepucuda_begin_constraints(bepucuda_ctx* ctx, int32_t source_bundle_width, int32_t batch_count) {
    if (!ctx || source_bundle_width < 1 || source_bundle_width > 64 || batch_count < 0) return fail(ctx, BEPUCUDA_ERR_INVALID_ARGUMENT, "begin_constraints: bad arguments");
    CK(cudaSetDevice(ctx->device));
    CK(cudaStreamSynchronize(ctx->stream));
    open_upload_window(ctx);
    ctx->W = source_bundle_width;
    ctx->batch_count = batch_count;
    ctx->sources.clear();
    ctx->pending_h2d.clear();
    ctx->raw_arena.reset();
    ctx->pinned_arena.reset();
    ctx->constraints_open = true;
    ctx->constraints_ready = false;
    invalidate_graph(ctx);
    return BEPUCUDA_OK;
}

int32_t bepucuda_upload_type_batch(bepucuda_ctx* ctx, int32_t batch_index, int32_t type_batch_index, int32_t type_id, int32_t constraint_count,
                                   const int32_t* body_references, const float* prestep, float* accumulated_impulses) {
    if (!ctx) return BEPUCUDA_ERR_INVALID_ARGUMENT;
    if (!ctx->constraints_open) return fail(ctx, BEPUCUDA_ERR_BAD_STATE, "upload_type_batch outside begin/end_constraints");
    if (batch_index < 0 || batch_index >= ctx->batch_count || type_batch_index < 0 || constraint_count < 0)
        return fail(ctx, BEPUCUDA_ERR_INVALID_ARGUMENT, "upload_type_batch: bad indices");
    const TypeInfo* t = get_type_info(type_id);
    if (!t) return fail(ctx, BEPUCUDA_ERR_UNSUPPORTED_TYPE, "upload_type_batch: unsupported constraint type id " + std::to_string(type_id));
    if (constraint_count == 0) return BEPUCUDA_OK;
    if (!body_references || !prestep || !accumulated_impulses) return fail(ctx, BEPUCUDA_ERR_INVALID_ARGUMENT, "upload_type_batch: null buffer");
    CK(cudaSetDevice(ctx->device));
    const int W = ctx->W;
    const size_t bundles = ((size_t)constraint_count + W - 1) / W;
    SourceTypeBatch s{};
    s.batch_index = batch_index; s.type_batch_index = type_batch_index; s.type_id = type_id; s.count = constraint_count;
    s.host_impulses = accumulated_impulses;
    s.refs_bytes = bundles * t->bodies * W * 4;
    s.prestep_bytes = bundles * t->prestep_rows * W * 4;
    s.impulse_bytes = bundles * t->impulse_rows * W * 4;
    cudaError_t e = cudaSuccess;
    s.raw_refs = (int32_t*)ctx->raw_arena.alloc(s.refs_bytes, &e);
    s.raw_prestep = (float*)ctx->raw_arena.alloc(s.prestep_bytes, &e);
    s.raw_impulses = (float*)ctx->raw_arena.alloc(s.impulse_bytes, &e);
    if (!s.raw_refs || !s.raw_prestep || !s.raw_impulses) return cuda_fail(ctx, e, "raw arena");
    int rc;
    if ((rc = copy_in(ctx, s.raw_refs, body_references, s.refs_bytes)) != BEPUCUDA_OK) return rc;
    if ((rc = copy_in(ctx, s.raw_prestep, prestep, s.prestep_bytes)) != BEPUCUDA_OK) return rc;
    if ((rc = copy_in(ctx, s.raw_impulses, accumulated_impulses, s.impulse_bytes)) != BEPUCUDA_OK) return rc;
    if (batch_index >= ctx->fallback_threshold) s.host_refs.assign(body_references, body_references + s.refs_bytes / 4);
    ctx->sources.push_back(std::move(s));
    return BEPUCUDA_OK;
}

int32_t bepucuda_set_constrained_kinematics(bepucuda_ctx* ctx, const int32_t* body_indices, int32_t count) {
    if (!ctx || count < 0 || (count > 0 && !body_indices)) return fail(ctx, BEPUCUDA_ERR_INVALID_ARGUMENT, "set_constrained_kinematics: bad arguments");
    ctx->kinematics.assign(body_indices, body_indices + count);
    if (ctx->constraints_ready) ctx->constraints_ready = false;
    return BEPUCUDA_OK;
}

int32_t bepucuda_end_constraints(bepucuda_ctx* ctx) {
    if (!ctx) return BEPUCUDA_ERR_INVALID_ARGUMENT;
    if (!ctx->constraints_open) return fail(ctx, BEPUCUDA_ERR_BAD_STATE, "end_constraints without begin_constraints");
    CK(cudaSetDevice(ctx->device));
    const int W = ctx->W;
    std::stable_sort(ctx->sources.begin(), ctx->sources.end(), [](const SourceTypeBatch& a, const SourceTypeBatch& b) {
        return a.batch_index != b.batch_index ? a.batch_index < b.batch_index : a.type_batch_index < b.type_batch_index;
    });

    std::vector<int32_t> source_bundle_base(ctx->sources.size());
    int32_t total_source_bundles = 0;
    for (size_t si = 0; si < ctx->sources.size(); ++si) {
        source_bundle_base[si] = total_source_bundles;
        total_source_bundles += (ctx->sources[si].count + W - 1) / W;
    }

    ctx->tbs.clear();
    ctx->tdescs.clear();
    std::vector<int32_t> maps;
    std::vector<size_t> map_offset;
    std::vector<std::vector<int>> batch_tbs;
    int64_t constraint_count = 0;
    ctx->sync_batch_count = 0;
    ctx->fallback_levels = 0;
    {
        int current_batch = -1;
        for (size_t si = 0; si < ctx->sources.size(); ++si) {
            SourceTypeBatch& s = ctx->sources[si];
            s.device_tbs.clear();
            if (s.batch_index >= ctx->fallback_threshold) continue;
            while ((int)batch_tbs.size() <= s.batch_index) batch_tbs.emplace_back();
            current_batch = s.batch_index;
            const TypeInfo* t = get_type_info(s.type_id);
            DeviceTypeBatch d{};
            d.type_id = s.type_id;
            d.bundle_count = (s.count + 31) / 32;
            d.device_batch = s.batch_index;
            TransposeDesc td{s.raw_refs, s.raw_prestep, s.raw_impulses, nullptr, s.count, t->bodies, t->prestep_rows, t->impulse_rows, source_bundle_base[si], 0, nullptr, nullptr};
            s.device_tbs.push_back((int)ctx->tbs.size());
            batch_tbs[s.batch_index].push_back((int)ctx->tbs.size());
            ctx->tbs.push_back(d);
            ctx->tdescs.push_back(td);
            map_offset.push_back(SIZE_MAX);
            s.live = s.count;
            constraint_count += s.count;
        }
        if (ctx->peer_mode) {
            while ((int)batch_tbs.size() < std::min(ctx->batch_count, ctx->fallback_threshold)) batch_tbs.emplace_back();
            for (const SourceTypeBatch& src : ctx->sources)
                if (src.batch_index >= ctx->fallback_threshold) return fail(ctx, BEPUCUDA_ERR_BAD_STATE, "end_constraints: the sequential fallback batch is not supported across ranks");
        }
        if (ctx->exchange && !ctx->peer_mode) {
            for (const SourceTypeBatch& src : ctx->sources)
                if (src.batch_index >= ctx->fallback_threshold) return fail(ctx, BEPUCUDA_ERR_BAD_STATE, "end_constraints: the sequential fallback batch is not supported with an exchange callback");
        }
        (void)current_batch;
        ctx->sync_batch_count = (int)batch_tbs.size();
    }
    {
        std::vector<int32_t> last_level;
        struct Slot { int level; int source; int constraint; };
        std::vector<Slot> slots;
        bool any = false;
        for (size_t si = 0; si < ctx->sources.size(); ++si) {
            SourceTypeBatch& s = ctx->sources[si];
            if (s.batch_index < ctx->fallback_threshold) continue;
            if (!any) { last_level.assign((size_t)ctx->body_count, 0); any = true; }
            s.live = 0;
            const TypeInfo* t = get_type_info(s.type_id);
            const int nb = t->bodies;
            const int bundles = (s.count + W - 1) / W;
            std::vector<int> lane_level(W);
            for (int k = 0; k < bundles; ++k) {
                for (int l = 0; l < W; ++l) {
                    lane_level[l] = 0;
                    const int c = k * W + l;
                    if (c >= s.count) continue;
                    const int32_t first = s.host_refs[((size_t)k * nb) * W + l];
                    if (first < 0) continue;
                    int lvl = 0;
                    for (int b = 0; b < nb; ++b) {
                        const int32_t enc = s.host_refs[((size_t)k * nb + b) * W + l];
                        if (enc < 0 || ((uint32_t)enc & kRefKinematicBit)) continue;
                        const uint32_t idx = (uint32_t)enc & kRefIndexMask;
                        if ((int)idx >= ctx->body_count) return fail(ctx, BEPUCUDA_ERR_INVALID_ARGUMENT, "end_constraints: body reference out of range");
                        lvl = std::max(lvl, last_level[idx]);
                    }
                    lane_level[l] = lvl + 1;
                }
                for (int l = 0; l < W; ++l) {
                    if (lane_level[l] == 0) continue;
                    for (int b = 0; b < nb; ++b) {
                        const int32_t enc = s.host_refs[((size_t)k * nb + b) * W + l];
                        if (enc < 0 || ((uint32_t)enc & kRefKinematicBit)) continue;
                        last_level[(uint32_t)enc & kRefIndexMask] = lane_level[l];
                    }
                    for (int l2 = 0; l2 < l; ++l2) {
                        if (lane_level[l2] == 0) continue;
                        for (int b = 0; b < nb; ++b) {
                            const int32_t e1 = s.host_refs[((size_t)k * nb + b) * W + l];
                            if (e1 < 0 || ((uint32_t)e1 & kRefKinematicBit)) continue;
                            for (int b2 = 0; b2 < nb; ++b2) {
                                const int32_t e2 = s.host_refs[((size_t)k * nb + b2) * W + l2];
                                if (e2 >= 0 && !((uint32_t)e2 & kRefKinematicBit) && (((uint32_t)e1 ^ (uint32_t)e2) & kRefIndexMask) == 0)
                                    return fail(ctx, BEPUCUDA_ERR_BATCH_INVARIANT, "end_constraints: a fallback bundle references the same dynamic body more than once");
                            }
                        }
                    }
                    slots.push_back({lane_level[l], (int)si, k * W + l});
                    ++s.live;
                    ++constraint_count;
                }
            }
        }
        if (any) {
            std::stable_sort(slots.begin(), slots.end(), [](const Slot& a, const Slot& b) { return a.level != b.level ? a.level < b.level : a.source < b.source; });
            size_t i = 0;
            while (i < slots.size()) {
                const int level = slots[i].level;
                batch_tbs.emplace_back();
                ++ctx->fallback_levels;
                while (i < slots.size() && slots[i].level == level) {
                    const int source = slots[i].source;
                    size_t j = i;
                    while (j < slots.size() && slots[j].level == level && slots[j].source == source) ++j;
                    SourceTypeBatch& s = ctx->sources[source];
                    const TypeInfo* t = get_type_info(s.type_id);
                    const int n = (int)(j - i);
                    DeviceTypeBatch d{};
                    d.type_id = s.type_id;
                    d.bundle_count = (n + 31) / 32;
                    d.device_batch = (int)batch_tbs.size() - 1;
                    map_offset.push_back(maps.size());
                    for (size_t q = i; q < j; ++q) maps.push_back(slots[q].constraint);
                    for (int q = n; q < d.bundle_count * 32; ++q) maps.push_back(-1);
                    TransposeDesc td{s.raw_refs, s.raw_prestep, s.raw_impulses, nullptr, s.count, t->bodies, t->prestep_rows, t->impulse_rows, source_bundle_base[source], 0, nullptr, nullptr};
                    s.device_tbs.push_back((int)ctx->tbs.size());
                    batch_tbs.back().push_back((int)ctx->tbs.size());
                    ctx->tbs.push_back(d);
                    ctx->tdescs.push_back(td);
                    i = j;
                }
            }
        }
    }

    size_t refs_floats = 0, prestep_floats = 0, impulse_floats = 0;
    std::vector<size_t> ro(ctx->tbs.size()), po(ctx->tbs.size()), io(ctx->tbs.size());
    for (size_t i = 0; i < ctx->tbs.size(); ++i) {
        const TypeInfo* t = get_type_info(ctx->tbs[i].type_id);
        ro[i] = refs_floats; po[i] = prestep_floats; io[i] = impulse_floats;
        refs_floats += (size_t)ctx->tbs[i].bundle_count * t->bodies * 32;
        prestep_floats += (size_t)ctx->tbs[i].bundle_count * t->prestep_rows * 32;
        impulse_floats += (size_t)ctx->tbs[i].bundle_count * t->impulse_rows * 32;
    }
    CK(ctx->refs32.reserve(refs_floats * 4 + 1024));
    ctx->refs_words = refs_floats;
    CK(ctx->prestep32.reserve(prestep_floats * 4 + 4));
    CK(ctx->impulses32.reserve(impulse_floats * 4 + 4));
    CK(ctx->map_table.reserve(maps.size() * 4 + 4));
    for (size_t i = 0; i < ctx->tbs.size(); ++i) {
        ctx->tbs[i].refs = ctx->refs32.as<int32_t>() + ro[i];
        ctx->tbs[i].prestep = ctx->prestep32.as<float>() + po[i];
        ctx->tbs[i].impulses = ctx->impulses32.as<float>() + io[i];
        ctx->tdescs[i].map = map_offset[i] == SIZE_MAX ? nullptr : ctx->map_table.as<int32_t>() + map_offset[i];
    }

    ctx->work.clear();
    ctx->bundle_live.clear();
    ctx->batch_work.clear();
    auto live_in_bundle = [&](int tb, int k) {
        if (map_offset[tb] == SIZE_MAX) return std::max(0, std::min(32, ctx->tdescs[tb].src_count - k * 32));
        int n = 0;
        for (int l = 0; l < 32; ++l) n += maps[map_offset[tb] + (size_t)k * 32 + l] >= 0;
        return n;
    };
    for (auto& list : batch_tbs) {
        const int begin = (int)ctx->work.size();
        for (int tb : list)
            for (int k = 0; k < ctx->tbs[tb].bundle_count; ++k) { ctx->work.push_back({tb, k}); ctx->bundle_live.push_back(live_in_bundle(tb, k)); }
        ctx->batch_work.push_back({begin, (int)ctx->work.size() - begin});
    }
    ctx->all_work_count = (int)ctx->work.size();
    ctx->inc_work_begin = (int)ctx->work.size();
    for (size_t tb = 0; tb < ctx->tbs.size(); ++tb)
        if (get_type_info(ctx->tbs[tb].type_id)->incremental)
            for (int k = 0; k < ctx->tbs[tb].bundle_count; ++k) { ctx->work.push_back({(int)tb, k}); ctx->bundle_live.push_back(live_in_bundle((int)tb, k)); }
    ctx->inc_work_count = (int)ctx->work.size() - ctx->inc_work_begin;

    ctx->records.resize(ctx->work.size());
    for (size_t i = 0; i < ctx->work.size(); ++i) {
        const WorkItem& w = ctx->work[i];
        const DeviceTypeBatch& tb = ctx->tbs[w.type_batch];
        const TypeInfo* t = get_type_info(tb.type_id);
        WorkRecord r{};
        r.refs = tb.refs + (size_t)w.bundle * t->bodies * 32;
        r.prestep = tb.prestep + (size_t)w.bundle * t->prestep_rows * 32;
        r.impulses = tb.impulses + (size_t)w.bundle * t->impulse_rows * 32;
        r.type_id = tb.type_id;
        r.live_lanes = ctx->bundle_live[i];
        ctx->records[i] = r;
    }

    int32_t bodies_per_type[64];
    for (int i = 0; i < 64; ++i) bodies_per_type[i] = get_type_info(i) ? get_type_info(i)->bodies : 0;
    CK(ctx->tb_table.reserve(ctx->tbs.size() * sizeof(DeviceTypeBatch) + 16));
    CK(ctx->tdesc_table.reserve(ctx->tdescs.size() * sizeof(TransposeDesc) + 16));
    CK(ctx->work_table.reserve(ctx->work.size() * sizeof(WorkItem) + 16));
    CK(ctx->record_table.reserve(ctx->records.size() * sizeof(WorkRecord) + 64));
    CK(ctx->bodies_per_type.reserve(sizeof(bodies_per_type)));
    CK(ctx->kinematics_dev.reserve(ctx->kinematics.size() * 4 + 4));
    if (!ctx->tbs.empty()) CK(cudaMemcpyAsync(ctx->tb_table.ptr, ctx->tbs.data(), ctx->tbs.size() * sizeof(DeviceTypeBatch), cudaMemcpyHostToDevice, ctx->stream));
    if (!ctx->tdescs.empty()) CK(cudaMemcpyAsync(ctx->tdesc_table.ptr, ctx->tdescs.data(), ctx->tdescs.size() * sizeof(TransposeDesc), cudaMemcpyHostToDevice, ctx->stream));
    if (!ctx->work.empty()) CK(cudaMemcpyAsync(ctx->work_table.ptr, ctx->work.data(), ctx->work.size() * sizeof(WorkItem), cudaMemcpyHostToDevice, ctx->stream));
    if (!ctx->records.empty()) CK(cudaMemcpyAsync(ctx->record_table.ptr, ctx->records.data(), ctx->records.size() * sizeof(WorkRecord), cudaMemcpyHostToDevice, ctx->stream));
    if (!maps.empty()) CK(cudaMemcpyAsync(ctx->map_table.ptr, maps.data(), maps.size() * 4, cudaMemcpyHostToDevice, ctx->stream));
    CK(cudaMemcpyAsync(ctx->bodies_per_type.ptr, bodies_per_type, sizeof(bodies_per_type), cudaMemcpyHostToDevice, ctx->stream));
    if (!ctx->kinematics.empty()) CK(cudaMemcpyAsync(ctx->kinematics_dev.ptr, ctx->kinematics.data(), ctx->kinematics.size() * 4, cudaMemcpyHostToDevice, ctx->stream));

    { int rc = flush_chunks(ctx, ctx->pending_h2d); if (rc != BEPUCUDA_OK) return rc; }
    launch_transpose_in_all(ctx->tb_table.as<DeviceTypeBatch>(), ctx->tdesc_table.as<TransposeDesc>(), ctx->work_table.as<WorkItem>(), ctx->all_work_count, W,
                            kTransposeRefs | kTransposePrestep | kTransposeImpulses, ctx->stream);
    const size_t nb = (size_t)std::max(ctx->body_count, 1);
    CK(ctx->first_batch.reserve(nb * 4));
    CK(ctx->sync_refcount.reserve(nb * 4));
    CK(ctx->sync_mask.reserve(nb * 8));
    launch_fill_i32(ctx->first_batch.as<int32_t>(), nb, 0x7fffffff, ctx->stream);
    CK(cudaMemsetAsync(ctx->sync_refcount.ptr, 0, nb * 4, ctx->stream));
    CK(cudaMemsetAsync(ctx->sync_mask.ptr, 0, nb * 8, ctx->stream));
    CK(cudaMemsetAsync(ctx->constrained.ptr, 0, nb, ctx->stream));
    CK(cudaMemsetAsync(ctx->error_dev.ptr, 0, 32, ctx->stream));
    CK(ctx->source_bundle_flags.reserve((size_t)std::max(total_source_bundles, 1) * 16));
    CK(cudaMemsetAsync(ctx->source_bundle_flags.ptr, 0, (size_t)std::max(total_source_bundles, 1) * 16, ctx->stream));
    launch_ownership_pass1(ctx->tb_table.as<DeviceTypeBatch>(), ctx->work_table.as<WorkItem>(), ctx->all_work_count, ctx->bodies_per_type.as<int32_t>(), ctx->sync_batch_count,
                           ctx->body_count, ctx->first_batch.as<int32_t>(), ctx->sync_refcount.as<int32_t>(), (unsigned long long*)ctx->sync_mask.ptr, ctx->error_dev.as<int32_t>(),
                           ctx->stream);
    if (ctx->peer_mode && nb > 0) {
        if ((int)ctx->global_first_batch.size() != ctx->body_count) return fail(ctx, BEPUCUDA_ERR_BAD_STATE, "end_constraints: bepucuda_shard_set_global was not called for this body count");
        CK(cudaMemcpyAsync(ctx->first_batch.ptr, ctx->global_first_batch.data(), (size_t)ctx->body_count * 4, cudaMemcpyHostToDevice, ctx->stream));
    }
    if (ctx->exchange && !ctx->peer_mode && nb > 0) {
        if (ctx->exchange(ctx->exchange_user, ctx->first_batch.ptr, (int64_t)ctx->body_count, 1, (void*)ctx->stream) != 0)
            return fail(ctx, BEPUCUDA_ERR_CUDA, "end_constraints: the exchange callback failed (first-batch minimum)");
    }
    launch_ownership_rest(ctx->tb_table.as<DeviceTypeBatch>(), ctx->work_table.as<WorkItem>(), ctx->all_work_count, ctx->bodies_per_type.as<int32_t>(), ctx->body_count,
                          ctx->first_batch.as<int32_t>(), ctx->sync_refcount.as<int32_t>(), (const unsigned long long*)ctx->sync_mask.ptr, ctx->constrained.as<uint8_t>(),
                          ctx->kinematics_dev.as<int32_t>(), (int)ctx->kinematics.size(), ctx->error_dev.as<int32_t>(), ctx->tdesc_table.as<TransposeDesc>(), W,
                          ctx->source_bundle_flags.as<int32_t>(), ctx->stream);
    if (ctx->peer_mode && nb > 0) {
        CK(cudaMemcpyAsync(ctx->constrained.ptr, ctx->global_constrained.data(), (size_t)ctx->body_count, cudaMemcpyHostToDevice, ctx->stream));
        std::vector<uint32_t> all;
        ctx->push_range.assign(ctx->sync_batch_count, {0, 0});
        for (int b = 0; b < ctx->sync_batch_count; ++b) {
            auto it = ctx->pushes_by_batch.find(b);
            if (it == ctx->pushes_by_batch.end()) continue;
            ctx->push_range[b] = {all.size(), (int)it->second.size()};
            all.insert(all.end(), it->second.begin(), it->second.end());
        }
        CK(ctx->pushes_dev.reserve(all.size() * 4 + 16));
        if (!all.empty()) CK(cudaMemcpy(ctx->pushes_dev.ptr, all.data(), all.size() * 4, cudaMemcpyHostToDevice));
    }
    if (ctx->exchange && !ctx->peer_mode && nb > 0) {
        CK(ctx->exchange_staging.reserve((size_t)nb * 24 * 4));
        launch_widen_u8(ctx->constrained.as<uint8_t>(), ctx->exchange_staging.as<int32_t>(), (size_t)ctx->body_count, ctx->stream);
        if (ctx->exchange(ctx->exchange_user, ctx->exchange_staging.ptr, (int64_t)ctx->body_count, 0, (void*)ctx->stream) != 0)
            return fail(ctx, BEPUCUDA_ERR_CUDA, "end_constraints: the exchange callback failed (constrained mask)");
        launch_narrow_i32(ctx->exchange_staging.as<int32_t>(), ctx->constrained.as<uint8_t>(), (size_t)ctx->body_count, ctx->stream);
    }
    if (ctx->peer_mode && !ctx->body_masks.empty()) {
        if ((int)ctx->body_masks.size() != ctx->body_count) return fail(ctx, BEPUCUDA_ERR_BAD_STATE, "end_constraints: bepucuda_shard_set_body_masks was called for another body count");
        CK(ctx->peer32.reserve(ctx->refs_words * 4 + 1024));
        CK(ctx->body_masks_dev.reserve((size_t)ctx->body_count + 16));
        CK(cudaMemcpyAsync(ctx->body_masks_dev.ptr, ctx->body_masks.data(), (size_t)ctx->body_count, cudaMemcpyHostToDevice, ctx->stream));
        launch_fill_peer_masks(ctx->refs32.as<int32_t>(), ctx->peer32.as<uint32_t>(), ctx->refs_words, ctx->body_masks_dev.as<uint8_t>(), ctx->peers.rank, ctx->stream);
        const int n_rec = ctx->all_work_count;
        CK(ctx->boundary_flags_dev.reserve((size_t)n_rec + 16));
        launch_boundary_flags(ctx->record_table.as<WorkRecord>(), n_rec, ctx->bodies_per_type.as<int32_t>(), (long long)(ctx->peer32.as<int32_t>() - ctx->refs32.as<int32_t>()),
                              ctx->boundary_flags_dev.as<uint8_t>(), ctx->stream);
        std::vector<uint8_t> is_boundary((size_t)n_rec);
        if (n_rec > 0) CK(cudaMemcpyAsync(is_boundary.data(), ctx->boundary_flags_dev.ptr, (size_t)n_rec, cudaMemcpyDeviceToHost, ctx->stream));
        CK(cudaStreamSynchronize(ctx->stream));
        ctx->boundary_count.assign(ctx->batch_work.size(), 0);
        std::vector<WorkRecord> sorted;
        for (size_t b = 0; b < ctx->batch_work.size(); ++b) {
            const int begin = ctx->batch_work[b].first, count = ctx->batch_work[b].second;
            sorted.clear();
            for (int pass = 0; pass < 2; ++pass)
                for (int i = begin; i < begin + count; ++i)
                    if ((is_boundary[(size_t)i] != 0) == (pass == 0)) {
                        WorkRecord r = ctx->records[(size_t)i];
                        r.live_lanes = (r.live_lanes & ~kRecordBoundaryBit) | (pass == 0 ? kRecordBoundaryBit : 0);
                        sorted.push_back(r);
                        ctx->boundary_count[b] += pass == 0;
                    }
            std::copy(sorted.begin(), sorted.end(), ctx->records.begin() + begin);
        }
        if (n_rec > 0) CK(cudaMemcpyAsync(ctx->record_table.ptr, ctx->records.data(), (size_t)n_rec * sizeof(WorkRecord), cudaMemcpyHostToDevice, ctx->stream));
    }
    CK(ctx->ref_rows.reserve((size_t)std::max<size_t>(ctx->records.size(), 1) * 64 * 4));
    launch_pack_ref_rows(ctx->record_table.as<WorkRecord>(), (int)ctx->records.size(), ctx->ref_rows.as<int32_t>(), ctx->stream);
    CK(cudaGetLastError());
    int32_t err = 0;
    CK(cudaMemcpyAsync(&err, ctx->error_dev.ptr, 4, cudaMemcpyDeviceToHost, ctx->stream));
    CK(cudaStreamSynchronize(ctx->stream));
    if (err == 1) return fail(ctx, BEPUCUDA_ERR_BATCH_INVARIANT, "end_constraints: a synchronized batch references the same dynamic body more than once");
    if (err == 2) return fail(ctx, BEPUCUDA_ERR_INVALID_ARGUMENT, "end_constraints: body reference out of range");

    ctx->timings.constraint_count = constraint_count;
    ctx->timings.device_batch_count = (int)batch_tbs.size();
    ctx->timings.fallback_level_count = ctx->fallback_levels;
    ctx->constraints_open = false;
    ctx->constraints_ready = true;
    ctx->data_dirty = false;
    return upload_program(ctx);
}

int32_t bepucuda_update_type_batch(bepucuda_ctx* ctx, int32_t batch_index, int32_t type_batch_index, const float* prestep, float* accumulated_impulses) {
    if (!ctx || !prestep || !accumulated_impulses) return fail(ctx, BEPUCUDA_ERR_INVALID_ARGUMENT, "update_type_batch: bad arguments");
    if (!ctx->constraints_ready) return fail(ctx, BEPUCUDA_ERR_BAD_STATE, "update_type_batch before end_constraints");
    CK(cudaSetDevice(ctx->device));
    open_upload_window(ctx);
    for (auto& s : ctx->sources)
        if (s.batch_index == batch_index && s.type_batch_index == type_batch_index) {
            char* alias_p = map_host(ctx, prestep, s.prestep_bytes);
            char* alias_i = map_host(ctx, accumulated_impulses, s.impulse_bytes);
            if (alias_p && alias_i) {
                queue_chunks(ctx->pending_h2d, s.raw_prestep, alias_p, s.prestep_bytes);
                queue_chunks(ctx->pending_h2d, s.raw_impulses, alias_i, s.impulse_bytes);
            } else {
                CK(cudaMemcpyAsync(s.raw_prestep, prestep, s.prestep_bytes, cudaMemcpyHostToDevice, ctx->stream));
                CK(cudaMemcpyAsync(s.raw_impulses, accumulated_impulses, s.impulse_bytes, cudaMemcpyHostToDevice, ctx->stream));
            }
            ctx->h2d_accum += (int64_t)(s.prestep_bytes + s.impulse_bytes);
            s.host_impulses = accumulated_impulses;
            if (s.resident_impulses) { s.resident_impulses = false; s.redistribute = false; ctx->descs_dirty = true; }
            ctx->data_dirty = true;
            return BEPUCUDA_OK;
        }
    return fail(ctx, BEPUCUDA_ERR_INVALID_ARGUMENT, "update_type_batch: unknown type batch");
}

static int contact_count_of_type(int type_id) {
    if (type_id >= 0 && type_id <= 7) return (type_id & 3) + 1;
    if (type_id >= 8 && type_id <= 10) return type_id - 6;
    if (type_id >= 15 && type_id <= 17) return type_id - 13;
    return 0;
}
static SourceTypeBatch* find_source(bepucuda_ctx* ctx, int32_t batch_index, int32_t type_batch_index) {
    for (auto& s : ctx->sources)
        if (s.batch_index == batch_index && s.type_batch_index == type_batch_index) return &s;
    return nullptr;
}
static int ensure_feature_arrays(bepucuda_ctx* ctx, SourceTypeBatch& s) {
    if (s.raw_features_old) return BEPUCUDA_OK;
    s.feature_bytes = (size_t)s.count * contact_count_of_type(s.type_id) * sizeof(int32_t);
    cudaError_t e = cudaSuccess;
    s.raw_features_old = (int32_t*)ctx->raw_arena.alloc(s.feature_bytes, &e);
    s.raw_features_new = (int32_t*)ctx->raw_arena.alloc(s.feature_bytes, &e);
    if (!s.raw_features_old || !s.raw_features_new) return cuda_fail(ctx, e, "raw arena (contact feature ids)");
    return BEPUCUDA_OK;
}

int32_t bepucuda_set_contact_features(bepucuda_ctx* ctx, int32_t batch_index, int32_t type_batch_index, const int32_t* feature_ids) {
    if (!ctx || !feature_ids) return fail(ctx, BEPUCUDA_ERR_INVALID_ARGUMENT, "set_contact_features: bad arguments");
    if (!ctx->constraints_open && !ctx->constraints_ready) return fail(ctx, BEPUCUDA_ERR_BAD_STATE, "set_contact_features before the type batch was uploaded");
    SourceTypeBatch* s = find_source(ctx, batch_index, type_batch_index);
    if (!s) return fail(ctx, BEPUCUDA_ERR_INVALID_ARGUMENT, "set_contact_features: unknown type batch");
    if (contact_count_of_type(s->type_id) == 0) return fail(ctx, BEPUCUDA_ERR_INVALID_ARGUMENT, "set_contact_features: not a contact constraint type");
    CK(cudaSetDevice(ctx->device));
    { int rc = ensure_feature_arrays(ctx, *s); if (rc != BEPUCUDA_OK) return rc; }
    return copy_in(ctx, s->raw_features_old, feature_ids, s->feature_bytes);
}

int32_t bepucuda_update_contacts(bepucuda_ctx* ctx, int32_t batch_index, int32_t type_batch_index, const float* prestep, const int32_t* new_feature_ids) {
    if (!ctx || !prestep || !new_feature_ids) return fail(ctx, BEPUCUDA_ERR_INVALID_ARGUMENT, "update_contacts: bad arguments");
    if (!ctx->constraints_ready) return fail(ctx, BEPUCUDA_ERR_BAD_STATE, "update_contacts before end_constraints");
    SourceTypeBatch* s = find_source(ctx, batch_index, type_batch_index);
    if (!s) return fail(ctx, BEPUCUDA_ERR_INVALID_ARGUMENT, "update_contacts: unknown type batch");
    if (!s->raw_features_old) return fail(ctx, BEPUCUDA_ERR_BAD_STATE, "update_contacts: bepucuda_set_contact_features was never called for this type batch");
    if (s->redistribute) return fail(ctx, BEPUCUDA_ERR_BAD_STATE, "update_contacts: called twice for the same type batch without a solve in between");
    CK(cudaSetDevice(ctx->device));
    open_upload_window(ctx);
    const void* srcs[2] = {prestep, new_feature_ids};
    void* dsts[2] = {s->raw_prestep, s->raw_features_new};
    const size_t sizes[2] = {s->prestep_bytes, s->feature_bytes};
    for (int i = 0; i < 2; ++i) {
        if (char* alias = map_host(ctx, srcs[i], sizes[i])) queue_chunks(ctx->pending_h2d, dsts[i], alias, sizes[i]);
        else CK(cudaMemcpyAsync(dsts[i], srcs[i], sizes[i], cudaMemcpyHostToDevice, ctx->stream));
        ctx->h2d_accum += (int64_t)sizes[i];
    }
    s->resident_impulses = true;
    s->redistribute = true;
    ctx->descs_dirty = true;
    ctx->data_dirty = true;
    return BEPUCUDA_OK;
}

int32_t bepucuda_upload_body_motion(bepucuda_ctx* ctx, const void* body_dynamics, int32_t body_count) {
    if (!ctx || !body_dynamics || body_count != ctx->body_count) return fail(ctx, BEPUCUDA_ERR_INVALID_ARGUMENT, "upload_body_motion: bad arguments (the body count must match the last upload_bodies)");
    if (body_count == 0) return BEPUCUDA_OK;
    CK(cudaSetDevice(ctx->device));
    open_upload_window(ctx);
    const size_t n = (size_t)body_count;
    if (char* alias = map_host(ctx, body_dynamics, n * 128)) {
        launch_scatter_body_motion(alias, body_count, ctx->B, ctx->stream);
    } else {
        CK(cudaMemcpy2DAsync(ctx->raw_bodies.ptr, 128, body_dynamics, 128, 64, n, cudaMemcpyHostToDevice, ctx->stream));
        launch_scatter_body_motion(ctx->raw_bodies.ptr, body_count, ctx->B, ctx->stream);
    }
    CK(cudaGetLastError());
    ctx->h2d_accum += (int64_t)n * 64;
    return BEPUCUDA_OK;
}

int32_t bepucuda_download_body_motion(bepucuda_ctx* ctx, void* out, int32_t body_count) {
    if (!ctx || !out || body_count < 0 || body_count > ctx->body_count) return fail(ctx, BEPUCUDA_ERR_INVALID_ARGUMENT, "download_body_motion: bad arguments");
    CK(cudaSetDevice(ctx->device));
    CK(cudaEventRecord(ctx->ev_down_begin, ctx->stream));
    const size_t n = (size_t)body_count;
    if (char* alias = map_host(ctx, out, n * 128)) {
        launch_gather_body_motion(alias, body_count, ctx->B, ctx->stream);
    } else {
        launch_gather_body_motion(ctx->raw_bodies.ptr, body_count, ctx->B, ctx->stream);
        CK(cudaMemcpy2DAsync(out, 128, ctx->raw_bodies.ptr, 128, 64, n, cudaMemcpyDeviceToHost, ctx->stream));
    }
    CK(cudaGetLastError());
    CK(cudaEventRecord(ctx->ev_down_end, ctx->stream));
    CK(cudaStreamSynchronize(ctx->stream));
    ctx->have_down = true;
    ctx->timings.d2h_bytes = (int64_t)n * 64;
    return BEPUCUDA_OK;
}

int32_t bepucuda_solve(bepucuda_ctx* ctx, float dt) {
    if (!ctx || !(dt > 0)) return fail(ctx, BEPUCUDA_ERR_INVALID_ARGUMENT, "solve: bad arguments");
    CK(cudaSetDevice(ctx->device));
    if (!ctx->constraints_ready) {
        if (ctx->constraints_open) return fail(ctx, BEPUCUDA_ERR_BAD_STATE, "solve inside begin/end_constraints");
        if (!ctx->sources.empty()) return fail(ctx, BEPUCUDA_ERR_BAD_STATE, "solve: constraint description is stale; re-run begin/upload/end_constraints");
        int rc = bepucuda_begin_constraints(ctx, ctx->W, 0);
        if (rc == BEPUCUDA_OK) rc = bepucuda_end_constraints(ctx);
        if (rc != BEPUCUDA_OK) return rc;
    }
    { int rc = refresh_device_rows(ctx); if (rc != BEPUCUDA_OK) return rc; }
    if (ctx->up_open) {
        cudaEventRecord(ctx->ev_up_end, ctx->stream);
        ctx->up_open = false;
        ctx->have_up = true;
    }
    ctx->timings.h2d_bytes = ctx->h2d_accum;
    ctx->h2d_accum = 0;
    CK(cudaEventSynchronize(ctx->ev_solve_end));
    compute_frame_params(ctx, dt, ctx->frame_params_host);
    ctx->frame_params_host->exchange_base = ctx->exchange_counter;
    ctx->frame_params_host->shard_solve_index = ctx->shard_solve_index;
    CK(cudaMemcpyAsync(ctx->frame_params_dev.ptr, ctx->frame_params_host, sizeof(FrameParams), cudaMemcpyHostToDevice, ctx->stream));

    if (ctx->peer_mode && ctx->cfg.execution_mode != BEPUCUDA_EXEC_GRAPH && ctx->cfg.execution_mode != BEPUCUDA_EXEC_STREAM)
        return fail(ctx, BEPUCUDA_ERR_BAD_STATE, "solve: peer sharding needs BEPUCUDA_EXEC_GRAPH or BEPUCUDA_EXEC_STREAM");
    if (ctx->exchange && !ctx->peer_mode) {
        if (ctx->cfg.execution_mode != BEPUCUDA_EXEC_STREAM) return fail(ctx, BEPUCUDA_ERR_BAD_STATE, "solve: sharded batches need BEPUCUDA_EXEC_STREAM");
        if (ctx->integ.angular_integration_mode != 0) return fail(ctx, BEPUCUDA_ERR_BAD_STATE, "solve: sharded batches support AngularIntegrationMode.Nonconserving only");
        ctx->exchange_failed = false;
    }
    CK(cudaEventRecord(ctx->ev_solve_begin, ctx->stream));
    int64_t launches = 0;
    if (ctx->cfg.execution_mode == BEPUCUDA_EXEC_GRAPH) {
        if (!ctx->graph_valid) {
            ctx->exchange_failed = false;
            CK(cudaStreamBeginCapture(ctx->stream, cudaStreamCaptureModeThreadLocal));
            int64_t n = 0;
            issue_stage_sequence(ctx, ctx->stream, &n);
            cudaError_t e = cudaStreamEndCapture(ctx->stream, &ctx->graph);
            if (e == cudaSuccess && ctx->exchange_failed) e = cudaErrorUnknown;
            if (e == cudaSuccess) e = cudaGraphInstantiate(&ctx->graph_exec, ctx->graph, 0);
            if (e != cudaSuccess) return cuda_fail(ctx, e, "graph capture");
            ctx->graph_valid = true;
            ctx->timings.kernel_launches = n;
        }
        if (ctx->graph_valid) {
            CK(cudaGraphLaunch(ctx->graph_exec, ctx->stream));
            launches = ctx->timings.kernel_launches;
        }
    }
    if (ctx->cfg.execution_mode == BEPUCUDA_EXEC_STREAM) {
        issue_stage_sequence(ctx, ctx->stream, &launches);
        CK(cudaGetLastError());
        if (ctx->exchange_failed) return fail(ctx, BEPUCUDA_ERR_CUDA, "solve: the exchange callback failed");
    }
    CK(cudaEventRecord(ctx->ev_solve_end, ctx->stream));
    if (ctx->peer_mode) { ctx->exchange_counter += ctx->exchanges_per_solve; ++ctx->shard_solve_index; }
    ctx->have_solve = true;
    ctx->timings.kernel_launches = launches;

    int64_t ci = 0, bytes = 0;
    const int substeps = (int)ctx->iterations.size();
    for (const SourceTypeBatch& s : ctx->sources) {
        const TypeInfo* t = get_type_info(s.type_id);
        const int64_t n = s.live;
        for (int sub = 0; sub < substeps; ++sub) {
            ci += n * ctx->iterations[sub];
            bytes += n * ((int64_t)t->warm_start_bytes + (int64_t)ctx->iterations[sub] * t->solve_bytes + (sub > 0 ? t->incremental_bytes : 0));
        }
    }
    bytes += (int64_t)ctx->body_count * 108;
    ctx->timings.constraint_iterations = ci;
    ctx->timings.algorithmic_bytes = bytes;
    return BEPUCUDA_OK;
}

static int check_device_error_flag(bepucuda_ctx* ctx) {
    if (ctx->peer_mode && ctx->tune[3]) {
        unsigned long long acc[4] = {};
        cudaMemcpy(acc, (unsigned long long*)ctx->shard_flags.ptr + kMaxShardRanks, sizeof(acc), cudaMemcpyDeviceToHost);
        if (acc[3]) fprintf(stderr, "[bepucuda shard rank %d] exchange phases, mean over %llu: push+fence %.2f us, signal %.2f us, wait %.2f us\n", ctx->peers.rank, acc[3],
                            acc[0] / 1e3 / acc[3], acc[1] / 1e3 / acc[3], acc[2] / 1e3 / acc[3]);
    }
    if (ctx->peer_mode) {
        int32_t e = 0;
        CK(cudaMemcpyAsync(&e, ctx->error_dev.ptr, 4, cudaMemcpyDeviceToHost, ctx->stream));
        CK(cudaStreamSynchronize(ctx->stream));
        if (e == 5) return fail(ctx, BEPUCUDA_ERR_CUDA, "sharded solve: a peer rank never reached an exchange point (flag barrier timed out); results are invalid");
    }
    return BEPUCUDA_OK;
}

int32_t bepucuda_synchronize(bepucuda_ctx* ctx) {
    if (!ctx) return BEPUCUDA_ERR_INVALID_ARGUMENT;
    CK(cudaSetDevice(ctx->device));
    CK(cudaStreamSynchronize(ctx->stream));
    return check_device_error_flag(ctx);
}

int32_t bepucuda_download_bodies(bepucuda_ctx* ctx, void* out, int32_t body_count) {
    if (!ctx || !out || body_count < 0 || body_count > ctx->body_count) return fail(ctx, BEPUCUDA_ERR_INVALID_ARGUMENT, "download_bodies: bad arguments");
    CK(cudaSetDevice(ctx->device));
    CK(cudaEventRecord(ctx->ev_down_begin, ctx->stream));
    launch_merge_bodies(ctx->raw_bodies.ptr, body_count, ctx->B, ctx->stream);
    CK(cudaGetLastError());
    CK(cudaMemcpyAsync(out, ctx->raw_bodies.ptr, (size_t)body_count * 128, cudaMemcpyDeviceToHost, ctx->stream));
    CK(cudaEventRecord(ctx->ev_down_end, ctx->stream));
    CK(cudaStreamSynchronize(ctx->stream));
    ctx->have_down = true;
    ctx->timings.d2h_bytes = (int64_t)body_count * 128;
    return BEPUCUDA_OK;
}

int32_t bepucuda_download_impulses(bepucuda_ctx* ctx) {
    if (!ctx) return BEPUCUDA_ERR_INVALID_ARGUMENT;
    if (!ctx->constraints_ready) return fail(ctx, BEPUCUDA_ERR_BAD_STATE, "download_impulses before end_constraints");
    CK(cudaSetDevice(ctx->device));
    launch_transpose_out_all(ctx->tb_table.as<DeviceTypeBatch>(), ctx->tdesc_table.as<TransposeDesc>(), ctx->work_table.as<WorkItem>(), ctx->all_work_count, ctx->W,
                             kTransposeImpulses, ctx->stream);
    CK(cudaGetLastError());
    int64_t bytes = 0;
    std::vector<CopyChunk> d2h;
    for (auto& s : ctx->sources) {
        if (char* alias = map_host(ctx, s.host_impulses, s.impulse_bytes)) queue_chunks(d2h, alias, s.raw_impulses, s.impulse_bytes);
        else CK(cudaMemcpyAsync(s.host_impulses, s.raw_impulses, s.impulse_bytes, cudaMemcpyDeviceToHost, ctx->stream));
        bytes += (int64_t)s.impulse_bytes;
    }
    { int rc = flush_chunks(ctx, d2h); if (rc != BEPUCUDA_OK) return rc; }
    CK(cudaStreamSynchronize(ctx->stream));
    ctx->timings.d2h_bytes += bytes;
    return BEPUCUDA_OK;
}

int32_t bepucuda_download_prestep(bepucuda_ctx* ctx, int32_t batch_index, int32_t type_batch_index, float* prestep_out) {
    if (!ctx || !prestep_out) return fail(ctx, BEPUCUDA_ERR_INVALID_ARGUMENT, "download_prestep: bad arguments");
    if (!ctx->constraints_ready) return fail(ctx, BEPUCUDA_ERR_BAD_STATE, "download_prestep before end_constraints");
    CK(cudaSetDevice(ctx->device));
    for (auto& s : ctx->sources)
        if (s.batch_index == batch_index && s.type_batch_index == type_batch_index) {
            launch_transpose_out_all(ctx->tb_table.as<DeviceTypeBatch>(), ctx->tdesc_table.as<TransposeDesc>(), ctx->work_table.as<WorkItem>(), ctx->all_work_count, ctx->W,
                                     kTransposePrestep, ctx->stream);
            CK(cudaGetLastError());
            CK(cudaMemcpyAsync(prestep_out, s.raw_prestep, s.prestep_bytes, cudaMemcpyDeviceToHost, ctx->stream));
            CK(cudaStreamSynchronize(ctx->stream));
            return BEPUCUDA_OK;
        }
    return fail(ctx, BEPUCUDA_ERR_INVALID_ARGUMENT, "download_prestep: unknown type batch");
}

int32_t bepucuda_get_timings(bepucuda_ctx* ctx, bepucuda_timings* out) {
    if (!ctx || !out) return BEPUCUDA_ERR_INVALID_ARGUMENT;
    CK(cudaSetDevice(ctx->device));
    CK(cudaStreamSynchronize(ctx->stream));
    { int rc = check_device_error_flag(ctx); if (rc != BEPUCUDA_OK) return rc; }
    if (ctx->have_solve) cudaEventElapsedTime(&ctx->timings.solve_ms, ctx->ev_solve_begin, ctx->ev_solve_end);
    if (ctx->have_up && !ctx->up_open) cudaEventElapsedTime(&ctx->timings.upload_ms, ctx->ev_up_begin, ctx->ev_up_end);
    if (ctx->have_down) cudaEventElapsedTime(&ctx->timings.download_ms, ctx->ev_down_begin, ctx->ev_down_end);
    *out = ctx->timings;
    return BEPUCUDA_OK;
}

int32_t bepucuda_event_record(bepucuda_ctx* ctx, int32_t slot) {
    if (!ctx || slot < 0 || slot >= 16) return fail(ctx, BEPUCUDA_ERR_INVALID_ARGUMENT, "event_record: bad slot");
    CK(cudaSetDevice(ctx->device));
    if (!ctx->user_events[slot]) CK(cudaEventCreate(&ctx->user_events[slot]));
    CK(cudaEventRecord(ctx->user_events[slot], ctx->stream));
    return BEPUCUDA_OK;
}
int32_t bepucuda_event_elapsed_ms(bepucuda_ctx* ctx, int32_t a, int32_t b, float* ms) {
    if (!ctx || !ms || a < 0 || a >= 16 || b < 0 || b >= 16 || !ctx->user_events[a] || !ctx->user_events[b]) return fail(ctx, BEPUCUDA_ERR_INVALID_ARGUMENT, "event_elapsed_ms: bad slots");
    CK(cudaSetDevice(ctx->device));
    CK(cudaEventSynchronize(ctx->user_events[b]));
    CK(cudaEventElapsedTime(ms, ctx->user_events[a], ctx->user_events[b]));
    return BEPUCUDA_OK;
}

int32_t bepucuda_profile_stages(bepucuda_ctx* ctx, float dt, bepucuda_stage_profile* out) {
    if (ctx && ctx->exchange) return fail(ctx, BEPUCUDA_ERR_BAD_STATE, "profile_stages: not available with sharded batches");
    if (!ctx || !out || !(dt > 0)) return fail(ctx, BEPUCUDA_ERR_INVALID_ARGUMENT, "profile_stages: bad arguments");
    if (!ctx->constraints_ready) return fail(ctx, BEPUCUDA_ERR_BAD_STATE, "profile_stages before end_constraints");
    CK(cudaSetDevice(ctx->device));
    std::memset(out, 0, sizeof(*out));
    { int rc = refresh_device_rows(ctx); if (rc != BEPUCUDA_OK) return rc; }
    CK(cudaStreamSynchronize(ctx->stream));
    compute_frame_params(ctx, dt, ctx->frame_params_host);
    CK(cudaMemcpyAsync(ctx->frame_params_dev.ptr, ctx->frame_params_host, sizeof(FrameParams), cudaMemcpyHostToDevice, ctx->stream));
    const size_t need = ctx->program.size() * 2;
    while (ctx->profile_events.size() < need) {
        cudaEvent_t ev;
        CK(cudaEventCreate(&ev));
        ctx->profile_events.push_back(ev);
    }
    const WorkRecord* records = ctx->record_table.as<WorkRecord>();
    const int32_t* ref_rows = ctx->ref_rows.as<int32_t>();
    const FrameParams* fp = ctx->frame_params_dev.as<FrameParams>();
    const int32_t* kin = ctx->kinematics_dev.as<int32_t>();
    std::vector<int> launched(ctx->program.size(), 0);
    for (size_t i = 0; i < ctx->program.size(); ++i) {
        const StageOp& op = ctx->program[i];
        const bool has_work = op.stage == kStageFinalPose ? ctx->B.count > 0 : op.work_count > 0;
        if (!has_work) continue;
        CK(cudaEventRecord(ctx->profile_events[2 * i], ctx->stream));
        if (op.stage <= kStageIncremental) ctx->launchers->constraint_stage(op.stage, records + op.work_begin, ref_rows + (size_t)op.work_begin * 64, op.work_count, ctx->B, fp, 0, ctx->stream);
        else if (op.stage <= kStageKinematic) ctx->launchers->kinematic_stage(op.stage, kin, op.work_count, ctx->B, fp, ctx->stream);
        else ctx->launchers->final_pose(ctx->B, fp, ctx->stream);
        CK(cudaEventRecord(ctx->profile_events[2 * i + 1], ctx->stream));
        launched[i] = 1;
    }
    CK(cudaStreamSynchronize(ctx->stream));
    CK(cudaGetLastError());
    for (size_t i = 0; i < ctx->program.size(); ++i) {
        if (!launched[i]) continue;
        float ms = 0;
        CK(cudaEventElapsedTime(&ms, ctx->profile_events[2 * i], ctx->profile_events[2 * i + 1]));
        const StageOp& op = ctx->program[i];
        out->ms[op.stage] += ms;
        out->launches[op.stage] += 1;
        int64_t bytes = 0;
        if (op.stage <= kStageIncremental) {
            for (int w = 0; w < op.work_count; ++w) {
                const WorkItem& wi = ctx->work[op.work_begin + w];
                const TypeInfo* t = get_type_info(ctx->tbs[wi.type_batch].type_id);
                const int per = op.stage == kStageSolve ? t->solve_bytes : op.stage == kStageIncremental ? t->incremental_bytes : t->warm_start_bytes;
                bytes += (int64_t)per * ctx->bundle_live[(size_t)op.work_begin + w];
            }
        } else if (op.stage == kStageFinalPose) {
            bytes = (int64_t)ctx->body_count * 108;
        } else {
            bytes = (int64_t)op.work_count * 108;
        }
        out->algorithmic_bytes[op.stage] += bytes;
    }
    return BEPUCUDA_OK;
}

static_assert(sizeof(bepucuda_body_shape) == sizeof(BodyShape) && sizeof(bepucuda_body_activity) == sizeof(BodyActivityRecord), "ABI structs mirror the device records");

int32_t bepucuda_set_body_shapes(bepucuda_ctx* ctx, const bepucuda_body_shape* shapes, int32_t body_count) {
    if (!ctx || body_count < 0 || (body_count > 0 && !shapes)) return fail(ctx, BEPUCUDA_ERR_INVALID_ARGUMENT, "set_body_shapes: bad arguments");
    CK(cudaSetDevice(ctx->device));
    CK(ctx->body_shapes.reserve((size_t)std::max(body_count, 1) * sizeof(BodyShape)));
    if (body_count > 0) CK(cudaMemcpyAsync(ctx->body_shapes.ptr, shapes, (size_t)body_count * sizeof(BodyShape), cudaMemcpyHostToDevice, ctx->stream));
    CK(cudaStreamSynchronize(ctx->stream));
    ctx->shape_count = body_count;
    return BEPUCUDA_OK;
}

int32_t bepucuda_predict_bounding_boxes(bepucuda_ctx* ctx, float dt, bepucuda_body_activity* activities, float* bounds_out) {
    if (!ctx || !(dt > 0) || !activities || !bounds_out) return fail(ctx, BEPUCUDA_ERR_INVALID_ARGUMENT, "predict_bounding_boxes: bad arguments");
    if (ctx->shape_count != ctx->body_count) return fail(ctx, BEPUCUDA_ERR_BAD_STATE, "predict_bounding_boxes: bepucuda_set_body_shapes was not called for the current body count");
    const int n = ctx->body_count;
    if (n == 0) return BEPUCUDA_OK;
    CK(cudaSetDevice(ctx->device));
    CK(ctx->body_activities.reserve((size_t)n * sizeof(BodyActivityRecord)));
    CK(ctx->body_bounds.reserve((size_t)n * 32));
    CK(cudaMemcpyAsync(ctx->body_activities.ptr, activities, (size_t)n * sizeof(BodyActivityRecord), cudaMemcpyHostToDevice, ctx->stream));
    auto clamp01 = [](float v) { return v < 0.f ? 0.f : (v > 1.f ? 1.f : v); };
    PredictParams p{};
    p.dt = dt;
    for (int i = 0; i < 3; ++i) p.gravity_dt[i] = ctx->integ.gravity[i] * dt;
    p.linear_damping_dt = powf(clamp01(1 - ctx->integ.linear_damping), dt);
    p.angular_damping_dt = powf(clamp01(1 - ctx->integ.angular_damping), dt);
    p.integrate_velocity_for_kinematics = ctx->integ.integrate_velocity_for_kinematics;
    launch_predict_bounding_boxes(ctx->B, ctx->body_shapes.as<BodyShape>(), ctx->body_activities.as<BodyActivityRecord>(), ctx->body_bounds.as<float4>(), p, ctx->stream);
    CK(cudaGetLastError());
    CK(cudaMemcpyAsync(activities, ctx->body_activities.ptr, (size_t)n * sizeof(BodyActivityRecord), cudaMemcpyDeviceToHost, ctx->stream));
    CK(cudaMemcpyAsync(bounds_out, ctx->body_bounds.ptr, (size_t)n * 32, cudaMemcpyDeviceToHost, ctx->stream));
    CK(cudaStreamSynchronize(ctx->stream));
    return BEPUCUDA_OK;
}

uint32_t bepucuda_color_hash(uint32_t constraint_index) { return color_hash(constraint_index); }

int32_t bepucuda_color_constraints(bepucuda_ctx* ctx, int32_t constraint_count, int32_t bodies_per_constraint, const int32_t* encoded_body_references, int32_t body_count,
                                   int32_t fallback_batch_threshold, int32_t order, const uint32_t* priorities, int32_t* batch_indices_out, int32_t* batch_count_out,
                                   int32_t* rounds_out) {
    if (!ctx) return BEPUCUDA_ERR_INVALID_ARGUMENT;
    if (constraint_count < 0 || bodies_per_constraint < 1 || bodies_per_constraint > 4 || body_count < 0 || fallback_batch_threshold < 1 || fallback_batch_threshold > 64)
        return fail(ctx, BEPUCUDA_ERR_INVALID_ARGUMENT, "color_constraints: counts out of range (1..4 body slots, fallback threshold 1..64)");
    if (order < BEPUCUDA_COLOR_INSERTION_ORDER || order > BEPUCUDA_COLOR_BY_PRIORITY || (order == BEPUCUDA_COLOR_BY_PRIORITY && !priorities))
        return fail(ctx, BEPUCUDA_ERR_INVALID_ARGUMENT, "color_constraints: unknown order, or BEPUCUDA_COLOR_BY_PRIORITY without priorities");
    if (constraint_count > 0 && (!encoded_body_references || !batch_indices_out)) return fail(ctx, BEPUCUDA_ERR_INVALID_ARGUMENT, "color_constraints: null buffer");
    if (batch_count_out) *batch_count_out = 0;
    if (rounds_out) *rounds_out = 0;
    if (constraint_count == 0) return BEPUCUDA_OK;
    CK(cudaSetDevice(ctx->device));
    const size_t words = (size_t)constraint_count * bodies_per_constraint;
    for (size_t i = 0; i < words; ++i) {
        const int32_t enc = encoded_body_references[i];
        if (enc >= 0 && (int32_t)((uint32_t)enc & ((1u << 30) - 1u)) >= body_count) return fail(ctx, BEPUCUDA_ERR_INVALID_ARGUMENT, "color_constraints: body reference out of range");
    }
    constexpr int kRoundsPerChunk = 32;
    const size_t nb = (size_t)std::max(body_count, 1), nc = (size_t)constraint_count;
    CK(ctx->color_refs.reserve(words * 4));
    CK(ctx->color_priorities.reserve(nc * 4));
    CK(ctx->color_body_min.reserve(nb * 8));
    CK(ctx->color_body_mask.reserve(nb * 8));
    CK(ctx->color_out.reserve(nc * 4));
    CK(ctx->color_lists.reserve(nc * 8));
    CK(ctx->color_counts.reserve((kRoundsPerChunk + 1) * 4));
    CK(cudaMemcpyAsync(ctx->color_refs.ptr, encoded_body_references, words * 4, cudaMemcpyHostToDevice, ctx->stream));
    if (order == BEPUCUDA_COLOR_BY_PRIORITY) CK(cudaMemcpyAsync(ctx->color_priorities.ptr, priorities, nc * 4, cudaMemcpyHostToDevice, ctx->stream));
    ColoringBuffers cb{};
    cb.refs = ctx->color_refs.as<int32_t>();
    cb.priorities = ctx->color_priorities.as<uint32_t>();
    cb.body_min = ctx->color_body_min.as<unsigned long long>();
    cb.body_mask = ctx->color_body_mask.as<unsigned long long>();
    cb.batch_out = ctx->color_out.as<int32_t>();
    cb.list[0] = ctx->color_lists.as<int32_t>();
    cb.list[1] = ctx->color_lists.as<int32_t>() + nc;
    cb.counts = ctx->color_counts.as<unsigned int>();
    cb.constraint_count = constraint_count;
    cb.bodies_per_constraint = bodies_per_constraint;
    cb.body_count = body_count;
    cb.fallback_threshold = fallback_batch_threshold;
    cb.order = order;
    CK(cudaMemsetAsync(ctx->color_counts.ptr, 0, (kRoundsPerChunk + 1) * 4, ctx->stream));
    launch_color_init(cb, ctx->stream);
    unsigned int counts[kRoundsPerChunk + 1];
    int64_t rounds = 0;
    for (;;) {
        for (int r = 0; r < kRoundsPerChunk; ++r) launch_color_round(cb, r, ctx->stream);
        CK(cudaMemcpyAsync(counts, ctx->color_counts.ptr, sizeof(counts), cudaMemcpyDeviceToHost, ctx->stream));
        CK(cudaStreamSynchronize(ctx->stream));
        CK(cudaGetLastError());
        int used = kRoundsPerChunk;
        for (int r = 0; r < kRoundsPerChunk; ++r)
            if (counts[r + 1] == 0) { used = r + 1; break; }
        rounds += used;
        if (counts[used] == 0) break;
        if (counts[kRoundsPerChunk] >= counts[0]) return fail(ctx, BEPUCUDA_ERR_CUDA, "color_constraints: no progress (internal error)");
        counts[0] = counts[kRoundsPerChunk];
        for (int r = 1; r <= kRoundsPerChunk; ++r) counts[r] = 0;
        CK(cudaMemcpyAsync(ctx->color_counts.ptr, counts, sizeof(counts), cudaMemcpyHostToDevice, ctx->stream));
        CK(cudaStreamSynchronize(ctx->stream));
    }
    CK(cudaMemcpyAsync(batch_indices_out, ctx->color_out.ptr, nc * 4, cudaMemcpyDeviceToHost, ctx->stream));
    CK(cudaStreamSynchronize(ctx->stream));
    int32_t highest = -1;
    for (size_t i = 0; i < nc; ++i) highest = std::max(highest, batch_indices_out[i]);
    if (batch_count_out) *batch_count_out = highest + 1;
    if (rounds_out) *rounds_out = (int32_t)std::min<int64_t>(rounds, 0x7fffffff);
    return BEPUCUDA_OK;
}

int32_t bepucuda_shard_export(bepucuda_ctx* ctx, bepucuda_ipc_handles* out) {
    if (!ctx || !out) return fail(ctx, BEPUCUDA_ERR_INVALID_ARGUMENT, "shard_export: bad arguments");
    if (ctx->body_count <= 0) return fail(ctx, BEPUCUDA_ERR_BAD_STATE, "shard_export before upload_bodies");
    CK(cudaSetDevice(ctx->device));
    CK(ctx->shard_flags.reserve(kShardFlagBlockWords * sizeof(unsigned long long)));
    CK(cudaMemset(ctx->shard_flags.ptr, 0, kShardFlagBlockWords * sizeof(unsigned long long)));
    void* ptrs[4] = {ctx->pose.ptr, ctx->velocity.ptr, ctx->inertia_world.ptr, ctx->shard_flags.ptr};
    for (int i = 0; i < 4; ++i) {
        cudaIpcMemHandle_t h;
        CK(cudaIpcGetMemHandle(&h, ptrs[i]));
        static_assert(sizeof(h) == 64, "cudaIpcMemHandle_t is 64 bytes");
        std::memcpy(out->bytes[i], &h, 64);
    }
    return BEPUCUDA_OK;
}

int32_t bepucuda_shard_import(bepucuda_ctx* ctx, int32_t rank, int32_t rank_count, const bepucuda_ipc_handles* all) {
    if (!ctx || !all || rank_count < 1 || rank_count > kMaxShardRanks || rank < 0 || rank >= rank_count) return fail(ctx, BEPUCUDA_ERR_INVALID_ARGUMENT, "shard_import: bad arguments");
    if (!ctx->shard_flags.ptr) return fail(ctx, BEPUCUDA_ERR_BAD_STATE, "shard_import before shard_export");
    CK(cudaSetDevice(ctx->device));
    ShardPeers p{};
    p.rank = rank;
    p.rank_count = rank_count;
    for (int r = 0; r < rank_count; ++r) {
        void* ptrs[4] = {ctx->pose.ptr, ctx->velocity.ptr, ctx->inertia_world.ptr, ctx->shard_flags.ptr};
        if (r != rank)
            for (int i = 0; i < 4; ++i) {
                cudaIpcMemHandle_t h;
                std::memcpy(&h, all[r].bytes[i], 64);
                CK(cudaIpcOpenMemHandle(&ptrs[i], h, cudaIpcMemLazyEnablePeerAccess));
                ctx->opened_ipc.push_back(ptrs[i]);
            }
        p.pose[r] = (float4*)ptrs[0];
        p.velocity[r] = (float4*)ptrs[1];
        p.inertia_world[r] = (float4*)ptrs[2];
        p.flags[r] = (unsigned long long*)ptrs[3];
    }
    ctx->peers = p;
    ctx->peer_mode = true;
    ctx->exchange_counter = 0;
    if (ctx->constraints_ready) ctx->constraints_ready = false;
    invalidate_graph(ctx);
    return BEPUCUDA_OK;
}

int32_t bepucuda_shard_import_contexts(bepucuda_ctx* ctx, int32_t rank, int32_t rank_count, bepucuda_ctx* const* all) {
    if (!ctx || !all || rank_count < 1 || rank_count > kMaxShardRanks || rank < 0 || rank >= rank_count || all[rank] != ctx)
        return fail(ctx, BEPUCUDA_ERR_INVALID_ARGUMENT, "shard_import_contexts: bad arguments");
    CK(cudaSetDevice(ctx->device));
    ShardPeers p{};
    p.rank = rank;
    p.rank_count = rank_count;
    for (int r = 0; r < rank_count; ++r) {
        bepucuda_ctx* o = all[r];
        if (!o || !o->shard_flags.ptr || o->body_count != ctx->body_count) return fail(ctx, BEPUCUDA_ERR_BAD_STATE, "shard_import_contexts: every context needs the same bodies and a shard_export");
        if (o->device != ctx->device) {
            int can = 0;
            CK(cudaDeviceCanAccessPeer(&can, ctx->device, o->device));
            if (!can) return fail(ctx, BEPUCUDA_ERR_BAD_STATE, "shard_import_contexts: no peer access between the devices");
            cudaError_t e = cudaDeviceEnablePeerAccess(o->device, 0);
            if (e != cudaSuccess && e != cudaErrorPeerAccessAlreadyEnabled) CK(e);
            (void)cudaGetLastError();
        }
        p.pose[r] = o->pose.as<float4>();
        p.velocity[r] = o->velocity.as<float4>();
        p.inertia_world[r] = o->inertia_world.as<float4>();
        p.flags[r] = (unsigned long long*)o->shard_flags.ptr;
    }
    ctx->peers = p;
    ctx->peer_mode = true;
    ctx->exchange_counter = 0;
    if (ctx->constraints_ready) ctx->constraints_ready = false;
    invalidate_graph(ctx);
    return BEPUCUDA_OK;
}

int32_t bepucuda_shard_set_global(bepucuda_ctx* ctx, const int32_t* first_batch, const uint8_t* constrained) {
    if (!ctx || !first_batch || !constrained) return fail(ctx, BEPUCUDA_ERR_INVALID_ARGUMENT, "shard_set_global: bad arguments");
    ctx->global_first_batch.assign(first_batch, first_batch + ctx->body_count);
    ctx->global_constrained.assign(constrained, constrained + ctx->body_count);
    if (ctx->constraints_ready) ctx->constraints_ready = false;
    return BEPUCUDA_OK;
}

int32_t bepucuda_shard_set_body_masks(bepucuda_ctx* ctx, const uint8_t* rank_masks) {
    if (!ctx) return BEPUCUDA_ERR_INVALID_ARGUMENT;
    if (rank_masks) ctx->body_masks.assign(rank_masks, rank_masks + ctx->body_count);
    else ctx->body_masks.clear();
    if (ctx->constraints_ready) ctx->constraints_ready = false;
    return BEPUCUDA_OK;
}

int32_t bepucuda_shard_set_pushes(bepucuda_ctx* ctx, int32_t batch_index, int32_t count, const int32_t* bodies, const int32_t* ranks, const int32_t* owner_flags) {
    if (!ctx || batch_index < 0 || count < 0 || (count > 0 && (!bodies || !ranks || !owner_flags))) return fail(ctx, BEPUCUDA_ERR_INVALID_ARGUMENT, "shard_set_pushes: bad arguments");
    std::vector<uint32_t>& list = ctx->pushes_by_batch[batch_index];
    list.resize((size_t)count);
    for (int i = 0; i < count; ++i) {
        if (bodies[i] < 0 || bodies[i] >= ctx->body_count || ranks[i] < 0 || ranks[i] >= kMaxShardRanks) return fail(ctx, BEPUCUDA_ERR_INVALID_ARGUMENT, "shard_set_pushes: body or rank out of range");
        list[i] = (uint32_t)bodies[i] | ((uint32_t)ranks[i] << 28) | (owner_flags[i] ? kPushOwnerBit : 0u);
    }
    if (ctx->constraints_ready) ctx->constraints_ready = false;
    return BEPUCUDA_OK;
}

int32_t bepucuda_set_boundary_bodies(bepucuda_ctx* ctx, const int32_t* body_indices, int32_t count, bepucuda_exchange_fn exchange, void* user) {
    if (!ctx || count < 0) return fail(ctx, BEPUCUDA_ERR_INVALID_ARGUMENT, "set_boundary_bodies: bad arguments");
    (void)body_indices;
    if (ctx->constraints_open) return fail(ctx, BEPUCUDA_ERR_BAD_STATE, "set_boundary_bodies inside begin/end_constraints");
    if (exchange && ctx->cfg.execution_mode != BEPUCUDA_EXEC_STREAM)
        return fail(ctx, BEPUCUDA_ERR_BAD_STATE, "set_boundary_bodies: sharded batches need a context created with BEPUCUDA_EXEC_STREAM");
    ctx->exchange = exchange;
    ctx->exchange_user = user;
    if (ctx->constraints_ready && !ctx->sources.empty()) ctx->constraints_ready = false;
    return BEPUCUDA_OK;
}

}
```

Baseline: 2.005 billion.

## Split contact solves into projection and velocity phases, project before PDL grid wait

Splits each contact solve into a projection step (effective masses, bias velocities, friction center) that only needs prestep rows and inertia, and a velocity step that needs body velocities. In the non-sharded solve kernel, the projection runs before griddepcontrol.wait when rows were prefetched, so it can overlap the previous kernel's tail. Per-lane projection scratch is kept in unused shared-memory slab rows. This adds shared-memory traffic, register pressure and extra template paths, and it also turns off row prefetch for non-fused sharded solve stages.

Result: faster. 2.181 billion (median of 6 runs) (+8.8%).

```diff
diff --git a/bepuphysics2_b200/csrc/bepu_contacts.cuh b/bepuphysics2_b200/csrc/bepu_contacts.cuh
--- a/bepuphysics2_b200/csrc/bepu_contacts.cuh
+++ b/bepuphysics2_b200/csrc/bepu_contacts.cuh
@@ -50,8 +50,9 @@
 BEPU_DI void penetration_warm_start(const Inertia& iA, const Inertia& iB, V3 normal, V3 offsetA, V3 offsetB, float accumulated, Velocity& vA, Velocity& vB) {
     penetration_apply(iA, iB, normal, cross(offsetA, normal), cross(normal, offsetB), accumulated, vA, vB);
 }
-BEPU_DI void penetration_solve(const Inertia& iA, const Inertia& iB, V3 normal, V3 offsetA, V3 offsetB, float depth, const Springiness& sp, float maxRecovery,
-                               float inverseDt, float& accumulated, Velocity& vA, Velocity& vB) {
+struct PenetrationProjection { float effective_mass, bias_velocity; };
+BEPU_DI PenetrationProjection penetration_project(const Inertia& iA, const Inertia& iB, V3 normal, V3 offsetA, V3 offsetB, float depth, const Springiness& sp, float maxRecovery,
+                                                  float inverseDt) {
     V3 angularA = cross(offsetA, normal);
     V3 angularB = cross(normal, offsetB);
     float angularA0 = vector_sandwich(angularA, iA.t);
@@ -59,11 +60,17 @@
     float linear = iA.inv_mass + iB.inv_mass;
     float effectiveMass = sp.effective_mass_cfm_scale / (linear + angularA0 + angularB0);
     float biasVelocity = fmin_ps(depth * inverseDt, fmin_ps(depth * sp.position_error_to_velocity, maxRecovery));
+    return {effectiveMass, biasVelocity};
+}
+BEPU_DI void penetration_velocity(const Inertia& iA, const Inertia& iB, V3 normal, V3 offsetA, V3 offsetB, PenetrationProjection pr, float softnessImpulseScale, float& accumulated,
+                                  Velocity& vA, Velocity& vB) {
+    V3 angularA = cross(offsetA, normal);
+    V3 angularB = cross(normal, offsetB);
     float csvaLinear = dot(vA.lin, normal);
     float csvaAngular = dot(vA.ang, angularA);
     float negatedCSVBLinear = dot(vB.lin, normal);
     float csvbAngular = dot(vB.ang, angularB);
-    float negatedCSI = accumulated * sp.softness_impulse_scale + (csvaLinear - negatedCSVBLinear + csvaAngular + csvbAngular - biasVelocity) * effectiveMass;
+    float negatedCSI = accumulated * softnessImpulseScale + (csvaLinear - negatedCSVBLinear + csvaAngular + csvbAngular - pr.bias_velocity) * pr.effective_mass;
     float previous = accumulated;
     accumulated = fmax_ps(0.0f, accumulated - negatedCSI);
     penetration_apply(iA, iB, normal, angularA, angularB, accumulated - previous, vA, vB);
@@ -82,15 +89,18 @@
     vA.lin = vA.lin + dLinA;
     vA.ang = vA.ang + dAngA;
 }
-BEPU_DI void penetration1_solve(const Inertia& iA, V3 normal, V3 offsetA, float depth, const Springiness& sp, float maxRecovery, float inverseDt, float& accumulated,
-                                Velocity& vA) {
+BEPU_DI PenetrationProjection penetration1_project(const Inertia& iA, V3 normal, V3 offsetA, float depth, const Springiness& sp, float maxRecovery, float inverseDt) {
     V3 angularA = cross(offsetA, normal);
     float angularA0 = vector_sandwich(angularA, iA.t);
     float effectiveMass = sp.effective_mass_cfm_scale / (iA.inv_mass + angularA0);
     float biasVelocity = fmin_ps(depth * inverseDt, fmin_ps(depth * sp.position_error_to_velocity, maxRecovery));
+    return {effectiveMass, biasVelocity};
+}
+BEPU_DI void penetration1_velocity(const Inertia& iA, V3 normal, V3 offsetA, PenetrationProjection pr, float softnessImpulseScale, float& accumulated, Velocity& vA) {
+    V3 angularA = cross(offsetA, normal);
     float csvaLinear = dot(vA.lin, normal);
     float csvaAngular = dot(vA.ang, angularA);
-    float negatedCSI = accumulated * sp.softness_impulse_scale + (csvaLinear + csvaAngular - biasVelocity) * effectiveMass;
+    float negatedCSI = accumulated * softnessImpulseScale + (csvaLinear + csvaAngular - pr.bias_velocity) * pr.effective_mass;
     float previous = accumulated;
     accumulated = fmax_ps(0.0f, accumulated - negatedCSI);
     penetration1_apply(iA, normal, angularA, accumulated - previous, vA);
@@ -117,11 +127,13 @@
     vB.lin = vB.lin - linearImpulseA * iB.inv_mass;
     vB.ang = vB.ang + transform(angularImpulseB, iB.t);
 }
-BEPU_DI void tangent_solve(V3 tX, V3 tY, V3 offsetA, V3 offsetB, const Inertia& iA, const Inertia& iB, float maximumImpulse, V2& accumulated, Velocity& vA, Velocity& vB) {
-    TangentJacobians j = tangent_jacobians(tX, tY, offsetA, offsetB);
+BEPU_DI Sym2 tangent_project(const TangentJacobians& j, const Inertia& iA, const Inertia& iB) {
     Sym2 linear = sandwich_scale(j.linearA, iA.inv_mass) + sandwich_scale(j.linearA, iB.inv_mass);
     Sym2 angular = matrix_sandwich(j.angularA, iA.t) + matrix_sandwich(j.angularB, iB.t);
-    Sym2 effectiveMass = invert(linear + angular);
+    return invert(linear + angular);
+}
+BEPU_DI void tangent_velocity(const TangentJacobians& j, Sym2 effectiveMass, const Inertia& iA, const Inertia& iB, float maximumImpulse, V2& accumulated, Velocity& vA,
+                              Velocity& vB) {
     V2 csvaLinear = transform_by_transpose(vA.lin, j.linearA);
     V2 csvaAngular = transform_by_transpose(vA.ang, j.angularA);
     V2 csvbLinear = transform_by_transpose(vB.lin, j.linearA);
@@ -141,10 +153,8 @@
     vA.lin = vA.lin + linearImpulseA * iA.inv_mass;
     vA.ang = vA.ang + transform(angularImpulseA, iA.t);
 }
-BEPU_DI void tangent1_solve(V3 tX, V3 tY, V3 offsetA, const Inertia& iA, float maximumImpulse, V2& accumulated, Velocity& vA) {
-    M23 linearA{tX, tY};
-    M23 angularA{cross(offsetA, tX), cross(offsetA, tY)};
-    Sym2 effectiveMass = invert(sandwich_scale(linearA, iA.inv_mass) + matrix_sandwich(angularA, iA.t));
+BEPU_DI Sym2 tangent1_project(const M23& linearA, const M23& angularA, const Inertia& iA) { return invert(sandwich_scale(linearA, iA.inv_mass) + matrix_sandwich(angularA, iA.t)); }
+BEPU_DI void tangent1_velocity(const M23& linearA, const M23& angularA, Sym2 effectiveMass, const Inertia& iA, float maximumImpulse, V2& accumulated, Velocity& vA) {
     V2 csv = transform_by_transpose(vA.lin, linearA) + transform_by_transpose(vA.ang, angularA);
     V2 negativeCSI = transform(csv, effectiveMass);
     V2 previous = accumulated;
@@ -160,23 +170,47 @@
     vA.ang = vA.ang + transform(worldImpulseA, iA.t);
     vB.ang = vB.ang - transform(worldImpulseA, iB.t);
 }
-BEPU_DI void twist_solve(V3 axis, const Inertia& iA, const Inertia& iB, float maximumImpulse, float& accumulated, Velocity& vA, Velocity& vB) {
+BEPU_DI float twist_project(V3 axis, const Inertia& iA, const Inertia& iB) {
     float inverseEffectiveMass = vector_sandwich(axis, iA.t) + vector_sandwich(axis, iB.t);
-    float effectiveMass = (0.0f == inverseEffectiveMass) ? 0.0f : 1.0f / inverseEffectiveMass;
+    return (0.0f == inverseEffectiveMass) ? 0.0f : 1.0f / inverseEffectiveMass;
+}
+BEPU_DI void twist_velocity(V3 axis, float effectiveMass, const Inertia& iA, const Inertia& iB, float maximumImpulse, float& accumulated, Velocity& vA, Velocity& vB) {
     float negatedCSI = (dot(vA.ang, axis) - dot(vB.ang, axis)) * effectiveMass;
     float previous = accumulated;
     accumulated = fmin_ps(maximumImpulse, fmax_ps(-maximumImpulse, accumulated - negatedCSI));
     twist_apply(axis, iA, iB, accumulated - previous, vA, vB);
 }
 BEPU_DI void twist1_apply(V3 axis, const Inertia& iA, float impulse, Velocity& vA) { vA.ang = vA.ang + transform(axis * impulse, iA.t); }
-BEPU_DI void twist1_solve(V3 axis, const Inertia& iA, float maximumImpulse, float& accumulated, Velocity& vA) {
+BEPU_DI float twist1_project(V3 axis, const Inertia& iA) {
     float angularA = vector_sandwich(axis, iA.t);
-    float effectiveMass = (0.0f == angularA) ? 0.0f : 1.0f / angularA;
+    return (0.0f == angularA) ? 0.0f : 1.0f / angularA;
+}
+BEPU_DI void twist1_velocity(V3 axis, float effectiveMass, const Inertia& iA, float maximumImpulse, float& accumulated, Velocity& vA) {
     float negativeCSI = dot(vA.ang, axis) * effectiveMass;
     float previous = accumulated;
     accumulated = fmin_ps(maximumImpulse, fmax_ps(-maximumImpulse, accumulated - negativeCSI));
     twist1_apply(axis, iA, accumulated - previous, vA);
 }
+
+constexpr int kStageSlabRows = 48;
+BEPU_DI void sts_f32(uint32_t addr, float v) { asm volatile("st.shared.f32 [%0], %1;" ::"r"(addr), "f"(v) : "memory"); }
+BEPU_DI float lds_f32_ordered(uint32_t addr) {
+    float v;
+    asm volatile("ld.shared.f32 %0, [%1];" : "=f"(v) : "r"(addr) : "memory");
+    return v;
+}
+template <class PR, int K> struct LaneScratch {
+    float v[K];
+    BEPU_DI void st(int k, float x) { v[k] = x; }
+    BEPU_DI float ld(int k) const { return v[k]; }
+};
+template <int K> struct LaneScratch<StagedRows, K> {
+    uint32_t addr;
+    BEPU_DI void st(int k, float x) { sts_f32(addr + k * (kLanes * 4), x); }
+    BEPU_DI float ld(int k) const { return lds_f32_ordered(addr + k * (kLanes * 4)); }
+};
+template <int K, class PR> BEPU_DI LaneScratch<PR, K> lane_scratch(PR) { return {}; }
+template <int K> BEPU_DI LaneScratch<StagedRows, K> lane_scratch(StagedRows p) { return {p.addr + (kStageSlabRows - K) * (kLanes * 4)}; }
 
 template <int N, bool TwoBody> struct ConvexLayout {
     static constexpr int kOffsetB = 4 * N;
@@ -234,72 +268,69 @@
         }
         twist_apply(normal, iA, iB, ldacc(a, N + 2), vA, vB);
     }
-    template <class PR, class AR> BEPU_DI static void solve(const Inertia& iA, const Inertia& iB, float dt, float inverseDt, PR p, AR a, Velocity& vA, Velocity& vB) {
-        V3 normal = ldrow3(p, L::kNormal), offsetB = ldrow3(p, L::kOffsetB);
-        float friction = ldrow(p, L::kFriction), maxRecovery = ldrow(p, L::kMaxRecovery);
-        Springiness sp = compute_springiness(ldrow(p, L::kAngularFrequency), ldrow(p, L::kTwiceDampingRatio), dt);
-        if constexpr (N > 1) {
-            V3 offs[N];
-            float depths[N];
-#pragma unroll
-            for (int i = 0; i < N; ++i) { offs[i] = ldrow3(p, 4 * i); depths[i] = ldrow(p, 4 * i + 3); }
-            const V3 centerA = friction_center<N>(offs, depths);
-            float penSum = 0.0f, twistSum = 0.0f;
+    static constexpr int kScratch = 3 * N;
+    static_assert(kPrestepRows + kImpulseRows + kScratch <= kStageSlabRows, "projection scratch overlaps the staged rows");
+    template <class PR> struct Projection {
+        V3 normal, offsetB;
+        float softness, friction, twistDepth;
+        V3 x, z, centerA;
+        Sym2 tangentMass;
+        float twistMass;
+        LaneScratch<PR, kScratch> rows;
+    };
+    template <class PR> BEPU_DI static Projection<PR> project(const Inertia& iA, const Inertia& iB, float dt, float inverseDt, PR p) {
+        Projection<PR> r;
+        r.normal = ldrow3(p, L::kNormal);
+        r.offsetB = ldrow3(p, L::kOffsetB);
+        const float friction = ldrow(p, L::kFriction), maxRecovery = ldrow(p, L::kMaxRecovery);
+        const Springiness sp = compute_springiness(ldrow(p, L::kAngularFrequency), ldrow(p, L::kTwiceDampingRatio), dt);
+        r.softness = sp.softness_impulse_scale;
+        r.rows = lane_scratch<kScratch>(p);
+        V3 offs[N];
+        float depths[N];
+#pragma unroll
+        for (int i = 0; i < N; ++i) { offs[i] = ldrow3(p, 4 * i); depths[i] = ldrow(p, 4 * i + 3); }
+        V3 centerA;
+        if constexpr (N == 1) centerA = offs[0]; else centerA = friction_center<N>(offs, depths);
+#pragma unroll
+        for (int i = 0; i < N; ++i) {
+            const PenetrationProjection q = penetration_project(iA, iB, r.normal, offs[i], offs[i] - r.offsetB, depths[i], sp, maxRecovery, inverseDt);
+            r.rows.st(3 * i, q.effective_mass);
+            r.rows.st(3 * i + 1, q.bias_velocity);
+            if constexpr (N > 1) r.rows.st(3 * i + 2, distance(centerA, offs[i]));
+        }
+        build_orthonormal_basis(r.normal, r.x, r.z);
+        r.centerA = centerA;
+        r.tangentMass = tangent_project(tangent_jacobians(r.x, r.z, centerA, centerA - r.offsetB), iA, iB);
+        r.twistMass = twist_project(r.normal, iA, iB);
+        r.friction = N == 1 ? friction : (1.0f / N) * friction;
+        r.twistDepth = fmax_ps(0.0f, depths[0]);
+        return r;
+    }
+    template <class PR, class AR> BEPU_DI static void velocity(const Projection<PR>& r, const Inertia& iA, const Inertia& iB, PR p, AR a, Velocity& vA, Velocity& vB) {
+        float penSum = 0.0f, twistSum = 0.0f;
 #pragma unroll 1
-            for (int i = 0; i < N; ++i) {
-                V3 offset = ldrow3(p, 4 * i);
-                float pen = ldacc(a, 2 + i);
-                penetration_solve(iA, iB, normal, offset, offset - offsetB, ldrow(p, 4 * i + 3), sp, maxRecovery, inverseDt, pen, vA, vB);
-                stacc(a, 2 + i, pen);
-                const float lever = pen * distance(centerA, offset);
-                penSum = i == 0 ? pen : penSum + pen;
+        for (int i = 0; i < N; ++i) {
+            V3 offset = ldrow3(p, 4 * i);
+            float pen = ldacc(a, 2 + i);
+            penetration_velocity(iA, iB, r.normal, offset, offset - r.offsetB, PenetrationProjection{r.rows.ld(3 * i), r.rows.ld(3 * i + 1)}, r.softness, pen, vA, vB);
+            stacc(a, 2 + i, pen);
+            penSum = i == 0 ? pen : penSum + pen;
+            if constexpr (N > 1) {
+                const float lever = pen * r.rows.ld(3 * i + 2);
                 twistSum = i == 0 ? lever : twistSum + lever;
             }
-            V3 x, z;
-            build_orthonormal_basis(normal, x, z);
-            V2 tangent{ldacc(a, 0), ldacc(a, 1)};
-            float twist = ldacc(a, N + 2);
-            const float premultiplied = (1.0f / N) * friction;
-            tangent_solve(x, z, centerA, centerA - offsetB, iA, iB, premultiplied * penSum, tangent, vA, vB);
-            twist_solve(normal, iA, iB, premultiplied * twistSum, twist, vA, vB);
-            stacc(a, 0, tangent.x);
-            stacc(a, 1, tangent.y);
-            stacc(a, N + 2, twist);
-        } else
-        {
-        V3 offs[N];
-        float depths[N], pen[N];
-#pragma unroll
-        for (int i = 0; i < N; ++i) { offs[i] = ldrow3(p, 4 * i); depths[i] = ldrow(p, 4 * i + 3); pen[i] = ldacc(a, 2 + i); }
-#pragma unroll
-        for (int i = 0; i < N; ++i) penetration_solve(iA, iB, normal, offs[i], offs[i] - offsetB, depths[i], sp, maxRecovery, inverseDt, pen[i], vA, vB);
-        V3 x, z;
-        build_orthonormal_basis(normal, x, z);
+        }
         V2 tangent{ldacc(a, 0), ldacc(a, 1)};
         float twist = ldacc(a, N + 2);
-        if constexpr (N == 1) {
-            float maximumTangentImpulse = friction * pen[0];
-            tangent_solve(x, z, offs[0], offs[0] - offsetB, iA, iB, maximumTangentImpulse, tangent, vA, vB);
-            float maximumTwistImpulse = friction * pen[0] * fmax_ps(0.0f, depths[0]);
-            twist_solve(normal, iA, iB, maximumTwistImpulse, twist, vA, vB);
-        } else {
-            float premultiplied = (1.0f / N) * friction;
-            float penSum = pen[0];
-#pragma unroll
-            for (int i = 1; i < N; ++i) penSum = penSum + pen[i];
-            V3 centerA = friction_center<N>(offs, depths);
-            tangent_solve(x, z, centerA, centerA - offsetB, iA, iB, premultiplied * penSum, tangent, vA, vB);
-            float twistSum = pen[0] * distance(centerA, offs[0]);
-#pragma unroll
-            for (int i = 1; i < N; ++i) twistSum = twistSum + pen[i] * distance(centerA, offs[i]);
-            twist_solve(normal, iA, iB, premultiplied * twistSum, twist, vA, vB);
-        }
+        tangent_velocity(tangent_jacobians(r.x, r.z, r.centerA, r.centerA - r.offsetB), r.tangentMass, iA, iB, r.friction * penSum, tangent, vA, vB);
+        twist_velocity(r.normal, r.twistMass, iA, iB, N == 1 ? r.friction * penSum * r.twistDepth : r.friction * twistSum, twist, vA, vB);
         stacc(a, 0, tangent.x);
         stacc(a, 1, tangent.y);
-#pragma unroll
-        for (int i = 0; i < N; ++i) stacc(a, 2 + i, pen[i]);
         stacc(a, N + 2, twist);
-        }
+    }
+    template <class PR, class AR> BEPU_DI static void solve(const Inertia& iA, const Inertia& iB, float dt, float inverseDt, PR p, AR a, Velocity& vA, Velocity& vB) {
+        velocity(project(iA, iB, dt, inverseDt, p), iA, iB, p, a, vA, vB);
     }
     BEPU_DI static void incremental_update(float dt, const Velocity& vA, const Velocity& vB, float* p) {
         V3 normal = ldrow3(p, L::kNormal), offsetB = ldrow3(p, L::kOffsetB);
@@ -331,70 +362,68 @@
         for (int i = 0; i < N; ++i) penetration1_apply(iA, normal, cross(ldrow3(p, 4 * i), normal), ldacc(a, 2 + i), vA);
         twist1_apply(normal, iA, ldacc(a, N + 2), vA);
     }
-    template <class PR, class AR> BEPU_DI static void solve(const Inertia& iA, float dt, float inverseDt, PR p, AR a, Velocity& vA) {
-        V3 normal = ldrow3(p, L::kNormal);
-        float friction = ldrow(p, L::kFriction), maxRecovery = ldrow(p, L::kMaxRecovery);
-        Springiness sp = compute_springiness(ldrow(p, L::kAngularFrequency), ldrow(p, L::kTwiceDampingRatio), dt);
-        if constexpr (N > 1) {
-            V3 offs[N];
-            float depths[N];
-#pragma unroll
-            for (int i = 0; i < N; ++i) { offs[i] = ldrow3(p, 4 * i); depths[i] = ldrow(p, 4 * i + 3); }
-            const V3 centerA = friction_center<N>(offs, depths);
-            float penSum = 0.0f, twistSum = 0.0f;
+    static constexpr int kScratch = 3 * N;
+    static_assert(kPrestepRows + kImpulseRows + kScratch <= kStageSlabRows, "projection scratch overlaps the staged rows");
+    template <class PR> struct Projection {
+        V3 normal;
+        float softness, friction, twistDepth;
+        V3 x, z, centerA;
+        Sym2 tangentMass;
+        float twistMass;
+        LaneScratch<PR, kScratch> rows;
+    };
+    template <class PR> BEPU_DI static Projection<PR> project(const Inertia& iA, float dt, float inverseDt, PR p) {
+        Projection<PR> r;
+        r.normal = ldrow3(p, L::kNormal);
+        const float friction = ldrow(p, L::kFriction), maxRecovery = ldrow(p, L::kMaxRecovery);
+        const Springiness sp = compute_springiness(ldrow(p, L::kAngularFrequency), ldrow(p, L::kTwiceDampingRatio), dt);
+        r.softness = sp.softness_impulse_scale;
+        r.rows = lane_scratch<kScratch>(p);
+        V3 offs[N];
+        float depths[N];
+#pragma unroll
+        for (int i = 0; i < N; ++i) { offs[i] = ldrow3(p, 4 * i); depths[i] = ldrow(p, 4 * i + 3); }
+        V3 centerA;
+        if constexpr (N == 1) centerA = offs[0]; else centerA = friction_center<N>(offs, depths);
+#pragma unroll
+        for (int i = 0; i < N; ++i) {
+            const PenetrationProjection q = penetration1_project(iA, r.normal, offs[i], depths[i], sp, maxRecovery, inverseDt);
+            r.rows.st(3 * i, q.effective_mass);
+            r.rows.st(3 * i + 1, q.bias_velocity);
+            if constexpr (N > 1) r.rows.st(3 * i + 2, distance(centerA, offs[i]));
+        }
+        build_orthonormal_basis(r.normal, r.x, r.z);
+        r.centerA = centerA;
+        r.tangentMass = tangent1_project(M23{r.x, r.z}, M23{cross(centerA, r.x), cross(centerA, r.z)}, iA);
+        r.twistMass = twist1_project(r.normal, iA);
+        r.friction = N == 1 ? friction : (1.0f / N) * friction;
+        r.twistDepth = fmax_ps(0.0f, depths[0]);
+        return r;
+    }
+    template <class PR, class AR> BEPU_DI static void velocity(const Projection<PR>& r, const Inertia& iA, PR p, AR a, Velocity& vA) {
+        float penSum = 0.0f, twistSum = 0.0f;
 #pragma unroll 1
-            for (int i = 0; i < N; ++i) {
-                V3 offset = ldrow3(p, 4 * i);
-                float pen = ldacc(a, 2 + i);
-                penetration1_solve(iA, normal, offset, ldrow(p, 4 * i + 3), sp, maxRecovery, inverseDt, pen, vA);
-                stacc(a, 2 + i, pen);
-                const float lever = pen * distance(centerA, offset);
-                penSum = i == 0 ? pen : penSum + pen;
+        for (int i = 0; i < N; ++i) {
+            V3 offset = ldrow3(p, 4 * i);
+            float pen = ldacc(a, 2 + i);
+            penetration1_velocity(iA, r.normal, offset, PenetrationProjection{r.rows.ld(3 * i), r.rows.ld(3 * i + 1)}, r.softness, pen, vA);
+            stacc(a, 2 + i, pen);
+            penSum = i == 0 ? pen : penSum + pen;
+            if constexpr (N > 1) {
+                const float lever = pen * r.rows.ld(3 * i + 2);
                 twistSum = i == 0 ? lever : twistSum + lever;
             }
-            V3 x, z;
-            build_orthonormal_basis(normal, x, z);
-            V2 tangent{ldacc(a, 0), ldacc(a, 1)};
-            float twist = ldacc(a, N + 2);
-            const float premultiplied = (1.0f / N) * friction;
-            tangent1_solve(x, z, centerA, iA, premultiplied * penSum, tangent, vA);
-            twist1_solve(normal, iA, premultiplied * twistSum, twist, vA);
-            stacc(a, 0, tangent.x);
-            stacc(a, 1, tangent.y);
-            stacc(a, N + 2, twist);
-        } else
-        {
-        V3 offs[N];
-        float depths[N], pen[N];
-#pragma unroll
-        for (int i = 0; i < N; ++i) { offs[i] = ldrow3(p, 4 * i); depths[i] = ldrow(p, 4 * i + 3); pen[i] = ldacc(a, 2 + i); }
-#pragma unroll
-        for (int i = 0; i < N; ++i) penetration1_solve(iA, normal, offs[i], depths[i], sp, maxRecovery, inverseDt, pen[i], vA);
-        V3 x, z;
-        build_orthonormal_basis(normal, x, z);
+        }
         V2 tangent{ldacc(a, 0), ldacc(a, 1)};
         float twist = ldacc(a, N + 2);
-        if constexpr (N == 1) {
-            tangent1_solve(x, z, offs[0], iA, friction * pen[0], tangent, vA);
-            twist1_solve(normal, iA, friction * pen[0] * fmax_ps(0.0f, depths[0]), twist, vA);
-        } else {
-            float premultiplied = (1.0f / N) * friction;
-            float penSum = pen[0];
-#pragma unroll
-            for (int i = 1; i < N; ++i) penSum = penSum + pen[i];
-            V3 centerA = friction_center<N>(offs, depths);
-            tangent1_solve(x, z, centerA, iA, premultiplied * penSum, tangent, vA);
-            float twistSum = pen[0] * distance(centerA, offs[0]);
-#pragma unroll
-            for (int i = 1; i < N; ++i) twistSum = twistSum + pen[i] * distance(centerA, offs[i]);
-            twist1_solve(normal, iA, premultiplied * twistSum, twist, vA);
-        }
+        tangent1_velocity(M23{r.x, r.z}, M23{cross(r.centerA, r.x), cross(r.centerA, r.z)}, r.tangentMass, iA, r.friction * penSum, tangent, vA);
+        twist1_velocity(r.normal, r.twistMass, iA, N == 1 ? r.friction * penSum * r.twistDepth : r.friction * twistSum, twist, vA);
         stacc(a, 0, tangent.x);
         stacc(a, 1, tangent.y);
-#pragma unroll
-        for (int i = 0; i < N; ++i) stacc(a, 2 + i, pen[i]);
         stacc(a, N + 2, twist);
-        }
+    }
+    template <class PR, class AR> BEPU_DI static void solve(const Inertia& iA, float dt, float inverseDt, PR p, AR a, Velocity& vA) {
+        velocity(project(iA, dt, inverseDt, p), iA, p, a, vA);
     }
     BEPU_DI static void incremental_update(float dt, const Velocity& vA, float* p) {
         V3 normal = ldrow3(p, L::kNormal);
@@ -430,10 +459,21 @@
             penetration_warm_start(iA, iB, normal, offset, contactOffsetB, ldacc(a, 3 * i + 2), vA, vB);
         }
     }
-    template <class PR, class AR> BEPU_DI static void solve(const Inertia& iA, const Inertia& iB, float dt, float inverseDt, PR p, AR a, Velocity& vA, Velocity& vB) {
-        V3 offsetB = ldrow3(p, L::kOffsetB);
-        float friction = ldrow(p, 0), maxRecovery = ldrow(p, 3);
-        Springiness sp = compute_springiness(ldrow(p, 1), ldrow(p, 2), dt);
+    template <class PR> struct Projection {
+        V3 offsetB;
+        float friction, maxRecovery, inverseDt;
+        Springiness sp;
+    };
+    template <class PR> BEPU_DI static Projection<PR> project(const Inertia&, const Inertia&, float dt, float inverseDt, PR p) {
+        Projection<PR> r;
+        r.offsetB = ldrow3(p, L::kOffsetB);
+        r.friction = ldrow(p, 0);
+        r.maxRecovery = ldrow(p, 3);
+        r.inverseDt = inverseDt;
+        r.sp = compute_springiness(ldrow(p, 1), ldrow(p, 2), dt);
+        return r;
+    }
+    template <class PR, class AR> BEPU_DI static void velocity(const Projection<PR>& r, const Inertia& iA, const Inertia& iB, PR p, AR a, Velocity& vA, Velocity& vB) {
 BEPU_CONTACT_LOOP
         for (int i = 0; i < N; ++i) {
             const int c = L::kContacts + 7 * i;
@@ -441,15 +481,20 @@
             float depth = ldrow(p, c + 3);
             V2 tangent{ldacc(a, 3 * i), ldacc(a, 3 * i + 1)};
             float pen = ldacc(a, 3 * i + 2);
-            V3 contactOffsetB = offset - offsetB;
-            penetration_solve(iA, iB, normal, offset, contactOffsetB, depth, sp, maxRecovery, inverseDt, pen, vA, vB);
+            V3 contactOffsetB = offset - r.offsetB;
+            penetration_velocity(iA, iB, normal, offset, contactOffsetB, penetration_project(iA, iB, normal, offset, contactOffsetB, depth, r.sp, r.maxRecovery, r.inverseDt),
+                                 r.sp.softness_impulse_scale, pen, vA, vB);
             V3 x, z;
             build_orthonormal_basis(normal, x, z);
-            tangent_solve(x, z, offset, contactOffsetB, iA, iB, friction * pen, tangent, vA, vB);
+            const TangentJacobians j = tangent_jacobians(x, z, offset, contactOffsetB);
+            tangent_velocity(j, tangent_project(j, iA, iB), iA, iB, r.friction * pen, tangent, vA, vB);
             stacc(a, 3 * i, tangent.x);
             stacc(a, 3 * i + 1, tangent.y);
             stacc(a, 3 * i + 2, pen);
         }
+    }
+    template <class PR, class AR> BEPU_DI static void solve(const Inertia& iA, const Inertia& iB, float dt, float inverseDt, PR p, AR a, Velocity& vA, Velocity& vB) {
+        velocity(project(iA, iB, dt, inverseDt, p), iA, iB, p, a, vA, vB);
     }
     BEPU_DI static void incremental_update(float dt, const Velocity& vA, const Velocity& vB, float* p) {
         V3 offsetB = ldrow3(p, L::kOffsetB);
@@ -478,9 +523,19 @@
             penetration1_apply(iA, normal, cross(offset, normal), ldacc(a, 3 * i + 2), vA);
         }
     }
-    template <class PR, class AR> BEPU_DI static void solve(const Inertia& iA, float dt, float inverseDt, PR p, AR a, Velocity& vA) {
-        float friction = ldrow(p, 0), maxRecovery = ldrow(p, 3);
-        Springiness sp = compute_springiness(ldrow(p, 1), ldrow(p, 2), dt);
+    template <class PR> struct Projection {
+        float friction, maxRecovery, inverseDt;
+        Springiness sp;
+    };
+    template <class PR> BEPU_DI static Projection<PR> project(const Inertia&, float dt, float inverseDt, PR p) {
+        Projection<PR> r;
+        r.friction = ldrow(p, 0);
+        r.maxRecovery = ldrow(p, 3);
+        r.inverseDt = inverseDt;
+        r.sp = compute_springiness(ldrow(p, 1), ldrow(p, 2), dt);
+        return r;
+    }
+    template <class PR, class AR> BEPU_DI static void velocity(const Projection<PR>& r, const Inertia& iA, PR p, AR a, Velocity& vA) {
 BEPU_CONTACT_LOOP
         for (int i = 0; i < N; ++i) {
             const int c = L::kContacts + 7 * i;
@@ -488,15 +543,19 @@
             float depth = ldrow(p, c + 3);
             V2 tangent{ldacc(a, 3 * i), ldacc(a, 3 * i + 1)};
             float pen = ldacc(a, 3 * i + 2);
-            penetration1_solve(iA, normal, offset, depth, sp, maxRecovery, inverseDt, pen, vA);
+            penetration1_velocity(iA, normal, offset, penetration1_project(iA, normal, offset, depth, r.sp, r.maxRecovery, r.inverseDt), r.sp.softness_impulse_scale, pen, vA);
             V3 x, z;
             build_orthonormal_basis(normal, x, z);
-            tangent1_solve(x, z, offset, iA, friction * pen, tangent, vA);
+            const M23 linearA{x, z}, angularA{cross(offset, x), cross(offset, z)};
+            tangent1_velocity(linearA, angularA, tangent1_project(linearA, angularA, iA), iA, r.friction * pen, tangent, vA);
             stacc(a, 3 * i, tangent.x);
             stacc(a, 3 * i + 1, tangent.y);
             stacc(a, 3 * i + 2, pen);
         }
     }
+    template <class PR, class AR> BEPU_DI static void solve(const Inertia& iA, float dt, float inverseDt, PR p, AR a, Velocity& vA) {
+        velocity(project(iA, dt, inverseDt, p), iA, p, a, vA);
+    }
     BEPU_DI static void incremental_update(float dt, const Velocity& vA, float* p) {
 #pragma unroll
         for (int i = 0; i < N; ++i) {
diff --git a/bepuphysics2_b200/csrc/bepu_solver_kernels.cuh b/bepuphysics2_b200/csrc/bepu_solver_kernels.cuh
--- a/bepuphysics2_b200/csrc/bepu_solver_kernels.cuh
+++ b/bepuphysics2_b200/csrc/bepu_solver_kernels.cuh
@@ -105,12 +105,34 @@
     else if constexpr (T::kBodies == 2) T::solve(b[0].inertia, b[1].inertia, dt, inverseDt, p, a, v[0], v[1]);
     else T::solve(b[0].inertia, dt, inverseDt, p, a, v[0]);
 }
+template <class...> using void_t = void;
+template <class T, class = void> struct HasProjection { static constexpr bool value = false; };
+template <class T> struct HasProjection<T, void_t<typename T::template Projection<StagedRows>>> { static constexpr bool value = true; };
+template <class T, class PR> BEPU_DI auto call_project(const BodyState* b, float dt, float inverseDt, PR p) {
+    if constexpr (T::kBodies == 2) return T::project(b[0].inertia, b[1].inertia, dt, inverseDt, p);
+    else return T::project(b[0].inertia, dt, inverseDt, p);
+}
+template <class T, class PJ, class PR, class AR> BEPU_DI void call_velocity(const PJ& pr, const BodyState* b, PR p, AR a, Velocity* v) {
+    if constexpr (T::kBodies == 2) T::velocity(pr, b[0].inertia, b[1].inertia, p, a, v[0], v[1]);
+    else T::velocity(pr, b[0].inertia, p, a, v[0]);
+}
 template <class T> BEPU_DI void call_incremental(float dt, const Velocity* v, float* p) {
     if constexpr (T::kIncremental) {
         if constexpr (T::kBodies == 2) T::incremental_update(dt, v[0], v[1], p);
         else T::incremental_update(dt, v[0], p);
     }
 }
+
+struct GridDependency {
+    bool pending;
+    BEPU_DI void wait() {
+        if (pending) {
+            asm volatile("griddepcontrol.wait;" ::: "memory");
+            asm volatile("griddepcontrol.launch_dependents;");
+            pending = false;
+        }
+    }
+};
 
 BEPU_DI uint32_t ldg_nc_u32(const void* p) {
     uint32_t v;
@@ -126,9 +148,11 @@
         dst[1] = make_float4(e, f, g, h);
     }
 }
-template <class T, int STAGE, bool kSharded, class PR, class AR>
-BEPU_DI void run_lane(const int32_t* refs, PR p, AR a, float* p_rw, uint32_t enc0, uint32_t enc1, const BodyBuffers& B, const FrameParams& fp, const ShardPeers* peers = nullptr,
-                      long long peer_delta = 0) {
+template <class T, int STAGE, bool kSharded, bool kEarly, class PR, class AR>
+BEPU_DI void run_lane(const int32_t* refs, PR p, AR a, float* p_rw, uint32_t enc0, uint32_t enc1, const BodyBuffers& B, const FrameParams& fp, GridDependency& dep,
+                      const ShardPeers* peers = nullptr, long long peer_delta = 0) {
+    constexpr bool kProjectEarly = kEarly && STAGE == kStageSolve && HasProjection<T>::value;
+    if constexpr (!kProjectEarly) dep.wait();
     constexpr int NB = T::kBodies;
     uint32_t enc[NB];
     enc[0] = enc0;
@@ -148,15 +172,30 @@
         for (int s = 0; s < NB; ++s) load_velocity(B.velocity, enc[s] & kRefIndexMask, v[s]);
         call_incremental<T>(fp.dt, v, p_rw);
     } else if constexpr (STAGE == kStageSolve) {
-#pragma unroll
-        for (int s = 0; s < NB; ++s) {
-            const uint32_t idx = enc[s] & kRefIndexMask;
-            load_velocity(B.velocity, idx, v[s]);
-            load_inertia(B.inertia_world, idx, b[s].inertia);
-            if (T::kNeedsPose) load_pose(B.pose, idx, b[s].pos, b[s].q);
-        }
-        rows_ready(p);
-        call_solve<T>(b, fp.dt, fp.inverse_dt, p, a, v);
+        bool early = false;
+        if constexpr (kProjectEarly) early = dep.pending;
+        if (early) {
+            if constexpr (kProjectEarly) {
+#pragma unroll
+                for (int s = 0; s < NB; ++s) load_inertia(B.inertia_world, enc[s] & kRefIndexMask, b[s].inertia);
+                rows_ready(p);
+                const auto pr = call_project<T>(b, fp.dt, fp.inverse_dt, p);
+                dep.wait();
+#pragma unroll
+                for (int s = 0; s < NB; ++s) load_velocity(B.velocity, enc[s] & kRefIndexMask, v[s]);
+                call_velocity<T>(pr, b, p, a, v);
+            }
+        } else {
+#pragma unroll
+            for (int s = 0; s < NB; ++s) {
+                const uint32_t idx = enc[s] & kRefIndexMask;
+                load_velocity(B.velocity, idx, v[s]);
+                load_inertia(B.inertia_world, idx, b[s].inertia);
+                if (T::kNeedsPose) load_pose(B.pose, idx, b[s].pos, b[s].q);
+            }
+            rows_ready(p);
+            call_solve<T>(b, fp.dt, fp.inverse_dt, p, a, v);
+        }
 #pragma unroll
         for (int s = 0; s < NB; ++s)
             if (!(enc[s] & kRefKinematicBit)) {
@@ -190,10 +229,6 @@
             }
     }
 }
-template <class T, int STAGE, class PR, class AR>
-BEPU_DI void run_lane(const int32_t* refs, PR p, AR a, float* p_rw, uint32_t enc0, uint32_t enc1, const BodyBuffers& B, const FrameParams& fp) {
-    run_lane<T, STAGE, false>(refs, p, a, p_rw, enc0, enc1, B, fp);
-}
 
 BEPU_DI int4 ldg_nc_v4(const void* p) {
     int4 v;
@@ -217,14 +252,14 @@
     X(8, NonconvexOneBody<2>) X(9, NonconvexOneBody<3>) X(10, NonconvexOneBody<4>)                                                \
     X(15, NonconvexTwoBody<2>) X(16, NonconvexTwoBody<3>) X(17, NonconvexTwoBody<4>)
 
-template <int STAGE, bool kSharded, class PR, class AR>
-BEPU_DI void run_bundle_rows(const WorkRecord& rec, int lane, PR p, AR a, uint32_t enc0, uint32_t enc1, const BodyBuffers& B, const FrameParams& fp, const ShardPeers* peers = nullptr,
-                             long long peer_delta = 0) {
+template <int STAGE, bool kSharded, bool kEarly, class PR, class AR>
+BEPU_DI void run_bundle_rows(const WorkRecord& rec, int lane, PR p, AR a, uint32_t enc0, uint32_t enc1, const BodyBuffers& B, const FrameParams& fp, GridDependency& dep,
+                             const ShardPeers* peers = nullptr, long long peer_delta = 0) {
     const int32_t* refs = rec.refs + lane;
     float* p_rw = rec.prestep + lane;
     switch (rec.type_id) {
 #define BEPU_CASE(ID, T) \
-    case ID: run_lane<T, STAGE, kSharded>(refs, p, a, p_rw, enc0, enc1, B, fp, peers, peer_delta); break;
+    case ID: run_lane<T, STAGE, kSharded, kEarly>(refs, p, a, p_rw, enc0, enc1, B, fp, dep, peers, peer_delta); break;
         BEPU_CONTACT_TYPES(BEPU_CASE)
         BEPU_JOINT_TYPES(BEPU_CASE)
         BEPU_JOINT_TYPES_MORE(BEPU_CASE)
@@ -232,13 +267,10 @@
         default: break;
     }
 }
-template <int STAGE, class PR, class AR>
-BEPU_DI void run_bundle_rows(const WorkRecord& rec, int lane, PR p, AR a, uint32_t enc0, uint32_t enc1, const BodyBuffers& B, const FrameParams& fp) {
-    run_bundle_rows<STAGE, false>(rec, lane, p, a, enc0, enc1, B, fp);
-}
 template <int STAGE>
 BEPU_DI void run_bundle(const WorkRecord& rec, int lane, uint32_t enc0, uint32_t enc1, const BodyBuffers& B, const FrameParams& fp) {
-    run_bundle_rows<STAGE>(rec, lane, GlobalRows{rec.prestep + lane}, GlobalAcc{rec.impulses + lane}, enc0, enc1, B, fp);
+    GridDependency waited{false};
+    run_bundle_rows<STAGE, false, false>(rec, lane, GlobalRows{rec.prestep + lane}, GlobalAcc{rec.impulses + lane}, enc0, enc1, B, fp, waited);
 }
 template <int STAGE> BEPU_DI void run_bundle(const WorkRecord& rec, int lane, const BodyBuffers& B, const FrameParams& fp) {
     const uint32_t enc0 = ldg_nc_u32(rec.refs + lane), enc1 = ldg_nc_u32(rec.refs + kLanes + lane);
@@ -256,7 +288,6 @@
     return c;
 }
 __constant__ StageRowCounts kStageRowCounts = make_stage_row_counts();
-constexpr int kStageSlabRows = 48;
 constexpr int kStageSlabBytes = kStageSlabRows * kLanes * 4;
 
 BEPU_DI uint32_t smem_u32(const void* p) { return (uint32_t)__cvta_generic_to_shared(p); }
@@ -301,7 +332,7 @@
     }
     __syncwarp();
 }
-template <int STAGE, bool kSharded>
+template <int STAGE, bool kSharded, bool kEarly>
 BEPU_DI void constraint_stage_body(const WorkRecord* __restrict__ records, const int32_t* __restrict__ ref_rows, int work_count, const BodyBuffers& B, const FrameParams* __restrict__ fpp, int flags, const ShardPeers* peers,
                                    long long peer_delta, const ShardStage* shard = nullptr) {
     constexpr bool kStaged = STAGE != kStageIncremental;
@@ -338,14 +369,17 @@
         enc1 = ldg_nc_u32(ref_rows + (size_t)warp * (2 * kLanes) + kLanes + lane);
     }
     const FrameParams fp = *fpp;
-    asm volatile("griddepcontrol.wait;" ::: "memory");
-    asm volatile("griddepcontrol.launch_dependents;");
+    GridDependency dep{true};
+    if (!(kEarly && STAGE == kStageSolve && early_rows)) dep.wait();
     bool boundary = false;
     if constexpr (kSharded) {
         boundary = active && (rec.live_lanes & kRecordBoundaryBit) != 0;
         if (boundary && shard->exchange_index > 0 && !(fp.tune[0] & 1)) shard_wait(*peers, lane, fp.shard_solve_index, shard->exchange_index - 1u, shard->error_flag);
     }
-    if (!active) return;
+    if (!active) {
+        dep.wait();
+        return;
+    }
     if constexpr (kStaged) {
         if (!early_rows && lane == 0) {
             const uint64_t policy = l2_evict_first_policy();
@@ -354,8 +388,9 @@
             bulk_copy_g2s(slab_addr + prestep_bytes, rec.impulses, impulse_bytes, bar, policy);
         }
         __syncwarp();
-        run_bundle_rows<STAGE, kSharded>(rec, lane, StagedRows{slab_addr + lane * 4, bar, 0u}, StagedAcc{slab_addr + prestep_bytes + lane * 4, rec.impulses + lane}, enc0, enc1, B, fp,
-                                         peers, boundary && !(fp.tune[0] & 4) ? peer_delta : 0);
+        run_bundle_rows<STAGE, kSharded, kEarly>(rec, lane, StagedRows{slab_addr + lane * 4, bar, 0u}, StagedAcc{slab_addr + prestep_bytes + lane * 4, rec.impulses + lane}, enc0, enc1, B, fp,
+                                         dep, peers, boundary && !(fp.tune[0] & 4) ? peer_delta : 0);
+        dep.wait();
         if constexpr (kSharded) {
             if (boundary && !(fp.tune[0] & 2)) {
                 __syncwarp();
@@ -369,13 +404,13 @@
 
 template <int STAGE, int MINB>
 __global__ void __launch_bounds__(kStageBlockThreads, MINB) constraint_stage_kernel(const WorkRecord* __restrict__ records, const int32_t* __restrict__ ref_rows, int work_count, BodyBuffers B, const FrameParams* __restrict__ fpp, int flags) {
-    constraint_stage_body<STAGE, false>(records, ref_rows, work_count, B, fpp, flags, nullptr, 0);
+    constraint_stage_body<STAGE, false, STAGE == kStageSolve && MINB == 1>(records, ref_rows, work_count, B, fpp, flags, nullptr, 0);
 }
 template <int STAGE, int MINB>
 __global__ void __launch_bounds__(kStageBlockThreads, MINB)
 constraint_stage_kernel_sharded(const WorkRecord* __restrict__ records, const int32_t* __restrict__ ref_rows, int work_count, BodyBuffers B, const FrameParams* __restrict__ fpp, int flags, const __grid_constant__ ShardPeers peers,
                                 long long peer_delta, const __grid_constant__ ShardStage shard) {
-    constraint_stage_body<STAGE, true>(records, ref_rows, work_count, B, fpp, flags, &peers, peer_delta, &shard);
+    constraint_stage_body<STAGE, true, false>(records, ref_rows, work_count, B, fpp, flags, &peers, peer_delta, &shard);
 }
 
 template <int STAGE> BEPU_DI void run_kinematic(int i, const int32_t* kinematics, const BodyBuffers& B, const FrameParams& fp) {
diff --git a/bepuphysics2_b200/csrc/bepucuda_api.cu b/bepuphysics2_b200/csrc/bepucuda_api.cu
--- a/bepuphysics2_b200/csrc/bepucuda_api.cu
+++ b/bepuphysics2_b200/csrc/bepucuda_api.cu
@@ -307,6 +307,7 @@
         if (ctx->peer_mode && op.pad >= 2 && op.stage <= kStageSolve) {
             if (op.work_count > 0) {
                 bool prefetch = previous != nullptr && previous->stage != kStageIncremental && !(previous->stage <= kStageSolve && previous->work_begin == op.work_begin && previous->work_count > 0);
+                if (op.stage == kStageSolve && !fused_pushes) prefetch = false;
                 const int launch_flags = (pdl ? kLaunchPdl : 0) | (prefetch ? kLaunchPrefetchRows : 0);
                 if (fused_pushes) {
                     const ShardStage shard{exchange_index, ctx->error_dev.as<int32_t>()};
```
